# A511-1103/building-detection

Measured on AMD Instinct MI355X. Metric: 512x512 tiles/sec fwd+bwd DeepLabv3+ (v3plus.py) (full train step: fwd+loss+bwd+Adam), higher is better.
Workload: dtype f32; 1 GPU; DeepLabv3+ (v3plus.py) 512x512 bs=16/GPU fp32, train step, single GPU; global_batch=16, train_step=eager launches, side_stream_filter_gradients=True

## Files before the change

building_detection_amd/_lib.py:

```python
from __future__ import annotations

import ctypes as C
import os
import threading

_HERE = os.path.dirname(os.path.abspath(__file__))
LIB_PATH = os.path.join(_HERE, "libsegengine.so")

SG_F32, SG_BF16, SG_I64 = 0, 1, 2
SG_HEAD_F32 = 0x100
SG_COMM_ID_BYTES = 128
SG_EPI_BIAS, SG_EPI_RELU = 1, 2
SG_PRO_UP2, SG_EPI_DOWN2 = 16, 32
SG_X_UP2 = 0x200
SG_ACT_RELU, SG_ACT_SIGMOID = 0, 1
SG_LOSS_CE2, SG_LOSS_FOCAL, SG_LOSS_EDGE_FOCAL = 0, 1, 2
SG_MAX_CLASSES = 32
SG_AUGMENT_MAX_ITEMS = 64
SG_AUG_FLIP_UD, SG_AUG_FLIP_LR, SG_AUG_SWAP_RB, SG_AUG_THRESHOLD = 1, 2, 4, 8
SG_SCENE_MAX_ITEMS = 64
SG_SYM_FLIP_UD, SG_SYM_FLIP_LR, SG_SYM_TRANSPOSE = 1, 2, 4
SG_OPT_ADAM, SG_OPT_SGD = 0, 1
SG_OPT_AMSGRAD, SG_OPT_NESTEROV, SG_OPT_EMA = 1, 2, 4
SG_OPT_CLIP_NONE, SG_OPT_CLIP_VALUE, SG_OPT_CLIP_NORM, SG_OPT_CLIP_GLOBAL = 0, 1, 2, 3
# ... 148 lines not shown
    elif k == SG_CK_X6:
        n += f".BN{la.bn}.v{la.var}" + (".mf16" if la.mf16 else "") + (".npl1" if pl.npl == 1 else "")
    elif k == SG_CK_B16:
        n += f".BN{la.bn}.KS{la.ks}.PD{la.pd}"
    elif k == SG_CK_X6W:
        n += f".S{pl.x6w_S}"
    elif k == SG_CK_B16W:
        n += f".S{pl.b16w_S}"
    elif k == SG_CK_PATCH:
        n += f".C{la.pc}" + ("m" if la.pmulti else "") + f".BN{la.bn}"
    elif k == SG_CK_WIDE:
        n += (".b16" if b16 else ".x6") + f".W{la.bn}"
    n += "".join("." + o for o in operands)
    if la.skip_taps:
        n += ".skip"
    if pl.perm2 and k in (SG_CK_X6, SG_CK_B16):
        n += ".perm2"
    if la.group_m > 1:
        n += f".gm{la.group_m}"
    if la.cb:
        n += f".cb{la.cb}"
    if pl.Ckp != pl.Ck and pl.family == SG_CF_SLAB and pl.fast:
        n += ".vpad"
    if pl.nsub > 1:
        n += f".sub{pl.nb}+{pl.tail_n}"
    return n


class SegPlan(C.Structure):

    _fields_ = [(n, C.c_int) for n in ("V", "TX", "TY", "gx", "S")] + [("part_bytes", C.c_size_t)]


_vp, _i, _i64, _f, _sz = C.c_void_p, C.c_int, C.c_int64, C.c_float, C.c_size_t
_op = C.POINTER(ConvOpts)
_dp = C.POINTER(ConvDesc)
_pp = C.POINTER(C.c_void_p)
_fp = C.POINTER(C.c_float)

_SIGNATURES = {
    "sg_abi_version": (_i, []),
    "sg_last_error": (C.c_char_p, []),
    "sg_set_conv_x6": (_i, [_i]),
    "sg_create": (_i, [_i, _pp]),
    "sg_destroy": (_i, [_vp]),
    "sg_num_cus": (_i, [_vp]),
    "sg_conv2d_fwd": (_i, [_vp, _vp, _i, _dp, _vp, _vp, _vp, _vp, _i, _op]),
    "sg_conv2d_fwd_ws_bytes": (_sz, [_dp]),
    "sg_conv2d_fwd_stats_bytes": (_sz, [_dp]),
    "sg_get_conv_x6": (_i, []),
    "sg_conv2d_planes_job": (_i, [_vp, _i, _dp, _i, C.POINTER(PlanesJob), C.POINTER(C.c_size_t)]),
    "sg_prepare_planes": (_i, [_vp, _vp, _vp, _vp, _vp, _i, _i]),
    "sg_bn_tiles_ws_bytes": (_sz, [_vp, _i, _i]),
    "sg_bn_train_fwd_tiles": (_i, [_vp, _vp, _i, _i64, _i, _vp, _i, _vp, _vp, _vp, _vp, C.c_float, C.c_float, _i, _vp, _sz]),
    "sg_bn_apply": (_i, [_vp, _vp, _i, _i64, _i, _vp, _vp, _vp, _vp, _vp, _vp, _i]),
    "sg_conv2d_dgrad_ws_bytes": (_sz, [_dp]),
    "sg_conv2d_dgrad": (_i, [_vp, _vp, _i, _dp, _vp, _vp, _vp, _vp, _i, _op]),
    "sg_conv2d_wgrad_ws_bytes": (_sz, [_vp, _dp]),
    "sg_conv2d_wgrad": (_i, [_vp, _vp, _i, _dp, _vp, _vp, _vp, _vp, _op]),
    "sg_conv2d_caps": (_i, [_vp, _i, _dp, _i, C.POINTER(ConvCaps)]),
    "sg_conv2d_plan": (_i, [_vp, _i, _dp, _i, _i, _i, C.POINTER(ConvPlan)]),
    "sg_split_planes": (_i, [_vp, _vp, _vp, _i64, _i, _i, _vp]),
    "sg_conv2d_wgrad_planes_ws_bytes": (_sz, [_vp, _dp]),
    "sg_conv2d_wgrad_planes": (_i, [_vp, _vp, _dp, _vp, _vp, _vp, _vp, _sz]),
    "sg_conv2d_wgrad_plan": (_i, [_vp, _i, _dp, _i, _i, C.POINTER(WgradPlan)]),
    "sg_bias_grad_ws_bytes": (_sz, [_vp, _i64, _i]),
    "sg_bias_grad": (_i, [_vp, _vp, _i, _i64, _i, _i, _vp, _vp, _vp, _sz]),
    "sg_dwconv2d_fwd": (_i, [_vp, _vp, _i, _dp, _vp, _vp, _vp, _i, C.POINTER(BnIn)]),
    "sg_dwconv2d_dgrad": (_i, [_vp, _vp, _i, _dp, _vp, _vp, _vp, _vp, _i, _vp, C.POINTER(DwBnSums)]),
    "sg_dwconv2d_dgrad_bnsums_ws_bytes": (_sz, [_vp, _dp]),
    "sg_dwconv2d_wgrad_ws_bytes": (_sz, [_vp, _dp]),
    "sg_dwconv2d_wgrad": (_i, [_vp, _vp, _i, _dp, _vp, _vp, _vp, _i, C.POINTER(BnIn), _vp, _sz]),
    "sg_dwconv2d_plan": (_i, [_vp, _i, _dp, _i, _i, _i, C.POINTER(DwPlan)]),
    "sg_dense_fwd": (_i, [_vp, _vp, _i, _i, _i, _i, _vp, _vp, _vp, _vp, _i]),
    "sg_bn_ws_bytes": (_sz, [_vp, _i64, _i]),
    "sg_bn_train_fwd": (_i, [_vp, _vp, _i, _i64, _i, _vp, _vp, _vp, _vp, _vp, _vp, _vp, _vp, _f, _f, _i, _i, _vp, _sz]),
    "sg_bn_train_bwd": (_i, [_vp, _vp, _i, _i64, _i, _vp, _vp, _vp, _vp, _vp, _vp, _vp, _vp, _vp, _vp, _i, _vp, _sz]),
    "sg_bn_train_bwd_apply": (_i, [_vp, _vp, _i, _i64, _i] + [_vp] * 9 + [_i]),
    "sg_bn_train_bwd_thin_ok": (_i, [_vp, _i, _i64, _i, _i, _i]),
    "sg_bn_train_bwd_thin": (_i, [_vp, _vp, _i, _i64, _i, _i, _i] + [_vp] * 10 + [_i, _vp, _sz]),
    "sg_bn_infer": (_i, [_vp, _vp, _i, _i64, _i, _vp, _vp, _vp, _vp, _vp, _vp, _f, _i]),
    "sg_add2_bn": (_i, [_vp, _vp, _i, _i64, _i] + [_vp] * 11 + [_i, _i, _f, _i, _i]),
    "sg_bn_plan": (_i, [_vp, _i, _i64, _i, _i, _i, C.POINTER(BnPlan)]),
    "sg_seg_plan": (_i, [_vp, _i, _i, _i64, _i, _i, _i, C.POINTER(SegPlan)]),
    "sg_act_fwd": (_i, [_vp, _vp, _i, _i, _i64, _vp, _vp]),
    "sg_act_bwd": (_i, [_vp, _vp, _i, _i, _i64, _vp, _vp, _vp, _i]),
    "sg_add_n": (_i, [_vp, _vp, _i, _i, _pp, _i64, _vp, _i]),
    "sg_copy_channels": (_i, [_vp, _vp, _i, _i64, _i, _vp, _i, _i, _vp, _i, _i, _i]),
    "sg_softmax2_fwd": (_i, [_vp, _vp, _i, _i64, _vp, _vp]),
    "sg_softmax2_bwd": (_i, [_vp, _vp, _i, _i64, _vp, _vp, _vp]),
    "sg_softmax_fwd": (_i, [_vp, _vp, _i, _i64, _i, _vp, _vp]),
    "sg_softmax_bwd": (_i, [_vp, _vp, _i, _i64, _i, _vp, _vp, _vp]),
    "sg_softmax_branch_fwd": (_i, [_vp, _vp, _i, _i, _i, _i, _vp, _vp]),
    "sg_softmax_branch_bwd": (_i, [_vp, _vp, _i, _i, _i, _i, _vp, _vp, _vp]),
    "sg_bcast_mul_fwd": (_i, [_vp, _vp, _i, _i, _i64, _i, _i, _vp, _vp, _vp, _i]),
    "sg_bcast_mul_bwd_ws_bytes": (_sz, [_vp, _i, _i64, _i, _i]),
    "sg_bcast_mul_bwd": (_i, [_vp, _vp, _i, _i, _i64, _i, _i, _vp, _vp, _vp, _vp, _vp, _i, _vp, _sz]),
    "sg_scse_fwd": (_i, [_vp, _vp, _i, _i, _i64, _i, _vp, _vp, _vp, _vp]),
    "sg_scse_bwd_ws_bytes": (_sz, [_vp, _i, _i64, _i]),
    "sg_scse_bwd": (_i, [_vp, _vp, _i, _i, _i64, _i, _vp, _vp, _vp, _vp, _vp, _vp, _vp, _vp, _sz]),
    "sg_scse_bwd_sums": (_i, [_vp, _vp, _i, _i, _i64, _i, _vp, _vp, _vp, _vp, _vp, _vp, _vp, _sz]),
    "sg_scse_bwd_final": (_i, [_vp, _vp, _i, _i, _i64, _i, _vp, _vp, _vp, _vp, _vp, _vp, _vp, _i]),
    "sg_bam_fwd": (_i, [_vp, _vp, _i, _i, _i64, _i, _vp, _vp, _vp, _vp]),
    "sg_bam_bwd_ws_bytes": (_sz, [_vp, _i, _i64, _i]),
    "sg_bam_bwd": (_i, [_vp, _vp, _i, _i, _i64, _i, _vp, _vp, _vp, _vp, _vp, _vp, _vp, _vp, _sz]),
    "sg_maxpool_fwd": (_i, [_vp, _vp, _i, _i, _i, _i, _i, _i, _i, _i, _i, _i, _i, _vp, _vp]),
    "sg_maxpool_bwd": (_i, [_vp, _vp, _i, _i, _i, _i, _i, _i, _i, _i, _i, _i, _i, _vp, _vp, _vp, _vp]),
    "sg_maxpool_fwd_idx": (_i, [_vp, _vp, _i, _i, _i, _i, _i, _i, _i, _i, _i, _i, _i, _vp, _vp, _vp]),
    "sg_maxpool_bwd_idx": (_i, [_vp, _vp, _i, _i, _i, _i, _i, _i, _i, _i, _i, _i, _i, _vp, _vp, _vp]),
    "sg_avgpool_ws_bytes": (_sz, [_vp, _i, _i, _i, _i, _i, _i]),
    "sg_avgpool_fwd": (_i, [_vp, _vp, _i, _i, _i, _i, _i, _i, _i, _vp, _vp, _vp, _sz]),
    "sg_avgpool_bwd": (_i, [_vp, _vp, _i, _i, _i, _i, _i, _i, _i, _vp, _vp, _i]),
    "sg_upsample_nearest_fwd": (_i, [_vp, _vp, _i, _i, _i, _i, _i, _i, _i, _vp, _vp, _i]),
    "sg_upsample_nearest_bwd": (_i, [_vp, _vp, _i, _i, _i, _i, _i, _i, _i, _vp, _i, _vp, _i]),
    "sg_upsample_bilinear_fwd": (_i, [_vp, _vp, _i, _i, _i, _i, _i, _i, _i, _vp, _vp, _i]),
    "sg_upsample_bilinear_bwd": (_i, [_vp, _vp, _i, _i, _i, _i, _i, _i, _i, _vp, _i, _vp, _i]),
    "sg_loss_ws_bytes": (_sz, [_vp, _i64]),
    "sg_loss_fwd": (_i, [_vp, _vp, _i, _i64, _i, _vp, _vp, _vp, _vp, _sz]),
    "sg_loss_bwd": (_i, [_vp, _vp, _i, _i64, _i, _vp, _vp, _vp, _f]),
    "sg_confusion_counts": (_i, [_vp, _vp, _i64, _i, _vp, _vp, _vp]),
    "sg_lossn_ws_bytes": (_sz, [_vp, _i64]),
    "sg_lossn_fwd": (_i, [_vp, _vp, _i, _i64, _i, _i, _fp, _vp, _vp, _vp, _vp, _sz]),
    "sg_lossn_bwd": (_i, [_vp, _vp, _i, _i64, _i, _i, _fp, _vp, _vp, _vp, _f]),
    "sg_confusion_matrix": (_i, [_vp, _vp, _i64, _i, _i, _vp, _vp, _vp]),
    "sg_loss_region_ws_bytes": (_sz, [_vp, C.POINTER(RegionDesc)]),
    "sg_loss_region_fwd": (_i, [_vp, _vp, C.POINTER(RegionDesc), _vp, _vp, _vp, _vp, _vp, _sz]),
    "sg_loss_region_bwd": (_i, [_vp, _vp, C.POINTER(RegionDesc), _vp, _vp, _vp, _vp, _f]),
    "sg_loss_mined_ws_bytes": (_sz, [_vp, C.POINTER(MineDesc)]),
    "sg_loss_mined_fwd": (_i, [_vp, _vp, C.POINTER(MineDesc), _vp, _vp, _vp, _vp, _vp, _sz]),
    "sg_loss_mined_bwd": (_i, [_vp, _vp, C.POINTER(MineDesc), _vp, _vp, _vp, _vp, _f]),
    "sg_adam_step": (_i, [_vp, _vp, _i64, _vp, _vp, _vp, _vp, _f, _f, _f, _f, _f]),
    "sg_adam_step_lr": (_i, [_vp, _vp, _i64, _vp, _vp, _vp, _vp, _vp, _f, _f, _f, _f]),
    "sg_optim_norms_ws_bytes": (_sz, [_i]),
    "sg_optim_grad_norms": (_i, [_vp, _vp, C.POINTER(OptimTable), _vp, _f, _vp, _vp, _sz]),
    "sg_optim_step": (_i, [_vp, _vp, C.POINTER(OptimDesc), C.POINTER(OptimTable), _vp, _vp, _vp, _vp, _vp, _vp, _vp, _f, _f, _vp]),
    "sg_edge_labels": (_i, [_vp, _vp, _i, _i, _i, _i, _vp, _vp]),
    "sg_resize_linear_u8": (_i, [_vp, _vp, _i, _i, _i, _i, _vp, _i, _i, _vp]),
    "sg_augment_u8": (_i, [_vp, _vp, _i, _i, _i, _i, _vp, _i, _vp, _i, _i, _i, _vp]),
    "sg_argmax_accumulate_i8": (_i, [_vp, _vp, _vp, _i, _i, _vp, _i, _i, _i, _i]),
    "sg_argmax_max_u8": (_i, [_vp, _vp, _vp, _i, _i, _i, _vp, _i, _i, _i, _i]),
    "sg_scene_tiles_u8": (_i, [_vp, _vp, _i, _i, _vp, _i, _vp, _i, _vp]),
    "sg_prob_accumulate": (_i, [_vp, _vp, _i, _i, _vp, _i, _vp, _vp, _f, _vp, _vp, _i, _i]),
    "sg_prob_finalize": (_i, [_vp, _vp, _i, _vp, _vp, _i, _i, _vp, _i, _vp]),
    "sg_vote_ge": (_i, [_vp, _vp, _i, _pp, _i64, _i, _vp]),
    "sg_mask_objects_ws_bytes": (_sz, [_i, _i]),
    "sg_mask_objects": (_i, [_vp, _vp, _i, _i, _vp, _i, _vp, _sz, _vp, _vp, _i, _vp, _vp]),
    "sg_mask_split_words": (_i64, [_i, _i, _i, _i, _i, _i]),
    "sg_mask_split": (_i, [_vp, _vp, _i, _i, _vp, _vp, _vp, _vp, _i, _i, _vp, _vp]),
    "sg_objects_label_ws_bytes": (_sz, [_i, _i]),
    "sg_objects_label": (_i, [_vp, _vp, _i, _i, _vp, _i, _vp, _sz, _vp, _vp, _i, _vp]),
    "sg_objects_overlap_ws_bytes": (_sz, [_i64]),
    "sg_objects_overlap": (_i, [_vp, _vp, _i, _i, _vp, _vp, _i64, _vp, _sz, _vp, _vp]),
    "sg_object_distances_ws_bytes": (_sz, [_i, _i, _i]),
    "sg_object_distances": (_i, [_vp, _vp, _i, _i, _i, _vp, _vp, _sz, _vp, _vp]),
    "sg_separation_weights": (_i, [_vp, _vp, _i, _i, _i, _vp, _vp, _f, _f, _vp]),
    "sg_u8_to_f32": (_i, [_vp, _vp, _i64, _vp, _vp, _f, _f]),
    "sg_cast": (_i, [_vp, _vp, _i, _i, _i64, _vp, _vp]),
    "sg_fill_f32": (_i, [_vp, _vp, _vp, _i64, _f]),
    "sg_trace_mark": (_i, [_vp, _vp, _i, _i]),
    "sg_scale_f32": (_i, [_vp, _vp, _vp, _i64, _f]),
    "sg_comm_probe": (_i, [_vp]),
    "sg_comm_unique_id": (_i, [_vp]),
    "sg_comm_init": (_i, [_vp, _i, _i, _i, _pp]),
    "sg_comm_allreduce_sum": (_i, [_vp, _vp, _i, _vp, _i64]),
    "sg_comm_rank": (_i, [_vp]),
    "sg_comm_nranks": (_i, [_vp]),
# ... 58 lines not shown
```

building_detection_amd/csrc/norm.hip:

```cpp
#include "sg_reduce.h"

namespace {

__device__ __forceinline__ float bn_affine(float x, float mean, float invstd, float gamma, float beta) {
  return fmaf((x - mean) * invstd, gamma, beta);
}
template <int MODE, int V>
__device__ __forceinline__ void bn_mask(float (&g)[V], const float (&x)[V], const float (&y)[V], const float (&mean)[V],
                                        const float (&invstd)[V], const float (&gamma)[V], const float (&beta)[V]) {
  if constexpr (MODE == 2) {
#pragma unroll
    for (int i = 0; i < V; ++i) g[i] = bn_affine(x[i], mean[i], invstd[i], gamma[i], beta[i]) > 0.f ? g[i] : 0.f;
  } else if constexpr (MODE == 1) {
#pragma unroll
    for (int i = 0; i < V; ++i) g[i] = y[i] > 0.f ? g[i] : 0.f;
  }
}
__device__ __forceinline__ float bn_dx(float x, float g, float mean, float invstd, float gamma, float dgamma, float dbeta, float inv_n) {
  const float xh = (x - mean) * invstd;
  return gamma * invstd * (g - dbeta * inv_n - xh * dgamma * inv_n);
}

template <typename T>
struct BnStatsOp {
  static constexpr int NOUT = 2;
  const T* __restrict__ x;
  int C;
  int64_t rows;
  float* moving_mean;
  float* moving_var;
  float* save_mean;
  float* save_invstd;
  float momentum, eps;
  int unbiased;

  template <int V>
  __device__ __forceinline__ void accum(int, int64_t r, int c, float (&acc)[2][V]) const {
    float k[V], v[V];
    ldv<V>(x + c, k);
    ldv<V>(x + r * C + c, v);
#pragma unroll
    for (int i = 0; i < V; ++i) {
      const float d = v[i] - k[i];
      acc[0][i] += d;
      acc[1][i] = fmaf(d, d, acc[1][i]);
    }
  }
  __device__ __forceinline__ void finalize(int, int c, const double (&s)[2]) const {
    const double n = (double)rows;
    const double m1 = s[0] / n;
    const double mean = (double)ld1<T>(x + c) + m1;
    double var = s[1] / n - m1 * m1;
    if (var < 0.0) var = 0.0;
    save_mean[c] = (float)mean;
    save_invstd[c] = (float)(1.0 / sqrt(var + (double)eps));
    const double var_u = (unbiased && rows > 1) ? var * (n / (n - 1.0)) : var;
    moving_mean[c] = (float)((double)moving_mean[c] * momentum + mean * (1.0 - (double)momentum));
    moving_var[c] = (float)((double)moving_var[c] * momentum + var_u * (1.0 - (double)momentum));
  }
};

template <int V>
struct BnCtx {
  float mv[V], iv[V], gm[V], bt[V];
};

template <typename T, int MODE>
struct BnBwdOp {
  static constexpr int NOUT = 2;
  const T* __restrict__ x;
  const T* __restrict__ y;
  const T* __restrict__ dy;
  const float* __restrict__ mean;
  const float* __restrict__ invstd;
  const float* __restrict__ gamma;
  const float* __restrict__ beta;
  float* dgamma;
  float* dbeta;
  int C;

  template <int V>
  __device__ __forceinline__ BnCtx<V> begin(int, int c) const {
    BnCtx<V> k;
    ldv<V>(mean + c, k.mv);
    ldv<V>(invstd + c, k.iv);
    if constexpr (MODE == 2) {
      ldv<V>(gamma + c, k.gm);
      ldv<V>(beta + c, k.bt);
    }
    return k;
  }
  template <int V>
  __device__ __forceinline__ void accum(int, int64_t r, int c, float (&acc)[2][V], const BnCtx<V>& k) const {
    float xv[V], gv[V], yv[V];
    ldv<V>(x + r * C + c, xv);
    ldv<V>(dy + r * C + c, gv);
    if constexpr (MODE == 1) ldv<V>(y + r * C + c, yv);
    bn_mask<MODE>(gv, xv, yv, k.mv, k.iv, k.gm, k.bt);
#pragma unroll
    for (int i = 0; i < V; ++i) {
      acc[0][i] += gv[i];
      acc[1][i] = fmaf(gv[i], (xv[i] - k.mv[i]) * k.iv[i], acc[1][i]);
    }
  }
  __device__ __forceinline__ void finalize(int, int c, const double (&s)[2]) const {
    dbeta[c] = (float)s[0];
    dgamma[c] = (float)s[1];
  }
};

template <int V, int CO>
__device__ __forceinline__ void thin_w(const float* __restrict__ w, int c, float (&wv)[V][CO]) {
#pragma unroll
  for (int k = 0; k < V; ++k)
#pragma unroll
    for (int o = 0; o < CO; ++o) wv[k][o] = w[(c + k) * CO + o];
}
template <int V, int CO>
__device__ __forceinline__ void thin_dy(const float* __restrict__ g, const float (&wv)[V][CO], float (&dy)[V]) {
  float gv[CO];
#pragma unroll
  for (int o = 0; o < CO; ++o) gv[o] = g[o];
#pragma unroll
  for (int k = 0; k < V; ++k) {
    float a = 0.f;
#pragma unroll
    for (int o = 0; o < CO; ++o) a = fmaf(gv[o], wv[k][o], a);
    dy[k] = a;
  }
}

template <int V, int CO>
struct BnThinCtx {
  BnCtx<V> k;
  float wv[V][CO];
};

template <int MODE, int CO>
struct BnBwdThinOp {
  static constexpr int NOUT = 2;
  const float* __restrict__ x;
  const float* __restrict__ g;
  const float* __restrict__ w;
  const float* __restrict__ mean;
  const float* __restrict__ invstd;
  const float* __restrict__ gamma;
  const float* __restrict__ beta;
  float* dgamma;
  float* dbeta;
  int C, y_ld;

  template <int V>
  __device__ __forceinline__ BnThinCtx<V, CO> begin(int, int c) const {
    BnThinCtx<V, CO> q;
    ldv<V>(mean + c, q.k.mv);
    ldv<V>(invstd + c, q.k.iv);
    if constexpr (MODE == 2) {
      ldv<V>(gamma + c, q.k.gm);
      ldv<V>(beta + c, q.k.bt);
    }
    thin_w<V, CO>(w, c, q.wv);
    return q;
  }
  template <int V>
  __device__ __forceinline__ void accum(int, int64_t r, int c, float (&acc)[2][V], const BnThinCtx<V, CO>& q) const {
    float xv[V], gv[V], yv[V];
    ldv<V>(x + r * C + c, xv);
    thin_dy<V, CO>(g + r * y_ld, q.wv, gv);
    bn_mask<MODE>(gv, xv, yv, q.k.mv, q.k.iv, q.k.gm, q.k.bt);
#pragma unroll
    for (int i = 0; i < V; ++i) {
      acc[0][i] += gv[i];
      acc[1][i] = fmaf(gv[i], (xv[i] - q.k.mv[i]) * q.k.iv[i], acc[1][i]);
    }
  }
  __device__ __forceinline__ void finalize(int, int c, const double (&s)[2]) const {
    dbeta[c] = (float)s[0];
    dgamma[c] = (float)s[1];
  }
};

template <int V, typename T>
__global__ void bn_apply_kernel(const T* __restrict__ x, const float* __restrict__ mean,
                                const float* __restrict__ invstd, const float* __restrict__ gamma,
                                const float* __restrict__ beta, T* __restrict__ y, int64_t rows, int C, int relu,
                                float eps, int infer, FastDiv fd_cv) {
  const uint32_t cv = C / V;
  const uint32_t total = (uint32_t)(rows * cv);
  const uint32_t stride = gridDim.x * blockDim.x;
  for (uint32_t i = blockIdx.x * blockDim.x + threadIdx.x; i < total; i += stride) {
    const int64_t r = fd_div(i, fd_cv);
    const int c = (int)(i - (uint32_t)r * cv) * V;
    float xv[V], mv[V], iv[V], gv[V], bv[V], o[V];
    ldv<V>(x + r * C + c, xv);
    ldv<V>(mean + c, mv);
    ldv<V>(invstd + c, iv);
    ldv<V>(gamma + c, gv);
    ldv<V>(beta + c, bv);
#pragma unroll
    for (int k = 0; k < V; ++k) {
      const float is = infer ? rsqrtf(iv[k] + eps) : iv[k];
      float t = bn_affine(xv[k], mv[k], is, gv[k], bv[k]);
      if (relu) t = fmaxf(t, 0.f);
      o[k] = t;
    }
    stv<V>(y + r * C + c, o);
  }
}

template <int V, typename T, int MODE>
__global__ void bn_bwd_apply_kernel(const T* __restrict__ x, const T* __restrict__ y,
                                    const T* __restrict__ dy, const float* __restrict__ mean,
                                    const float* __restrict__ invstd, const float* __restrict__ gamma,
                                    const float* __restrict__ beta, const float* __restrict__ dgamma,
                                    const float* __restrict__ dbeta, T* __restrict__ dx, int64_t rows, int C,
                                    FastDiv fd_cv) {
  const uint32_t cv = C / V;
  const uint32_t total = (uint32_t)(rows * cv);
  const uint32_t stride = gridDim.x * blockDim.x;
  const float inv_n = 1.0f / (float)rows;
  for (uint32_t i = blockIdx.x * blockDim.x + threadIdx.x; i < total; i += stride) {
    const int64_t r = fd_div(i, fd_cv);
    const int c = (int)(i - (uint32_t)r * cv) * V;
    float xv[V], gv[V], mv[V], iv[V], gam[V], dg[V], db[V], o[V];
    ldv<V>(x + r * C + c, xv);
    ldv<V>(dy + r * C + c, gv);
    ldv<V>(mean + c, mv);
    ldv<V>(invstd + c, iv);
    ldv<V>(gamma + c, gam);
    ldv<V>(dgamma + c, dg);
    ldv<V>(dbeta + c, db);
    if constexpr (MODE == 2) {
      float bt[V];
      ldv<V>(beta + c, bt);
#pragma unroll
      for (int k = 0; k < V; ++k) gv[k] = bn_affine(xv[k], mv[k], iv[k], gam[k], bt[k]) > 0.f ? gv[k] : 0.f;
    } else if constexpr (MODE == 1) {
      float yv[V];
      ldv<V>(y + r * C + c, yv);
#pragma unroll
      for (int k = 0; k < V; ++k) gv[k] = yv[k] > 0.f ? gv[k] : 0.f;
    }
#pragma unroll
    for (int k = 0; k < V; ++k) {
      const float xh = (xv[k] - mv[k]) * iv[k];
      o[k] = gam[k] * iv[k] * (gv[k] - db[k] * inv_n - xh * dg[k] * inv_n);
    }
    stv<V>(dx + r * C + c, o);
  }
}

template <int V, typename T>
__global__ __launch_bounds__(256) void bn_apply_cols_kernel(const T* __restrict__ x, const float* __restrict__ mean,
                                                            const float* __restrict__ invstd, const float* __restrict__ gamma,
                                                            const float* __restrict__ beta, T* __restrict__ y, int64_t rows,
                                                            int C, int relu, float eps, int infer, int prow, FastDiv fd_cv) {
  const uint32_t i0 = blockIdx.x * 256u + threadIdx.x, cv = (uint32_t)(C / V);
  const uint32_t r0 = fd_div(i0, fd_cv);
  const int c = (int)(i0 - r0 * cv) * V;
  float mv[V], is[V], gv[V], bv[V];
  ldv<V>(mean + c, mv);
  ldv<V>(invstd + c, is);
  ldv<V>(gamma + c, gv);
  ldv<V>(beta + c, bv);
  if (infer) {
#pragma unroll
    for (int k = 0; k < V; ++k) is[k] = rsqrtf(is[k] + eps);
  }
  auto one = [&](const float (&xv)[V], int64_t r) {
    float o[V];
#pragma unroll
    for (int k = 0; k < V; ++k) {
      float t = bn_affine(xv[k], mv[k], is[k], gv[k], bv[k]);
      if (relu) t = fmaxf(t, 0.f);
      o[k] = t;
    }
    stv<V>(y + r * C + c, o);
  };
  const int64_t stride = prow, gstep = (int64_t)gridDim.y * 4 * prow;
  for (int64_t r = (int64_t)blockIdx.y * 4 * prow + r0; r < rows; r += gstep) {
    if (r + 3 * stride < rows) {
      float x0[V], x1[V], x2[V], x3[V];
      ldv<V>(x + r * C + c, x0);
      ldv<V>(x + (r + stride) * C + c, x1);
      ldv<V>(x + (r + 2 * stride) * C + c, x2);
      ldv<V>(x + (r + 3 * stride) * C + c, x3);
      one(x0, r); one(x1, r + stride); one(x2, r + 2 * stride); one(x3, r + 3 * stride);
    } else {
      for (int64_t q = r; q < rows; q += stride) {
        float x0[V];
        ldv<V>(x + q * C + c, x0);
        one(x0, q);
      }
    }
  }
}
constexpr int BN_APPLY_PERIODS = 4;

template <int V, typename T, int MODE>
__global__ __launch_bounds__(256) void bn_bwd_apply_cols_kernel(const T* __restrict__ x, const T* __restrict__ y,
                                                                const T* __restrict__ dy, const float* __restrict__ mean,
                                                                const float* __restrict__ invstd, const float* __restrict__ gamma,
                                                                const float* __restrict__ beta, const float* __restrict__ dgamma,
                                                                const float* __restrict__ dbeta, T* __restrict__ dx, int64_t rows,
                                                                int C, int prow, FastDiv fd_cv) {
  const uint32_t i0 = blockIdx.x * 256u + threadIdx.x, cv = (uint32_t)(C / V);
  const uint32_t r0 = fd_div(i0, fd_cv);
  const int c = (int)(i0 - r0 * cv) * V;
  float mv[V], iv[V], gam[V], dg[V], db[V], bt[V];
  ldv<V>(mean + c, mv);
  ldv<V>(invstd + c, iv);
  ldv<V>(gamma + c, gam);
  ldv<V>(dgamma + c, dg);
  ldv<V>(dbeta + c, db);
  if constexpr (MODE == 2) ldv<V>(beta + c, bt);
  const float inv_n = 1.0f / (float)rows;
  auto one = [&](const float (&xv)[V], float (&gv)[V], const float (&yv)[V], int64_t r) {
    float o[V];
    bn_mask<MODE>(gv, xv, yv, mv, iv, gam, bt);
#pragma unroll
    for (int k = 0; k < V; ++k) o[k] = bn_dx(xv[k], gv[k], mv[k], iv[k], gam[k], dg[k], db[k], inv_n);
    stv<V>(dx + r * C + c, o);
  };
  const int64_t stride = (int64_t)gridDim.y * prow, gstep = 2 * stride;
  for (int64_t r = (int64_t)blockIdx.y * prow + r0; r < rows; r += gstep) {
    if (r + stride < rows) {
      float x0[V], x1[V], g0[V], g1[V], y0[V], y1[V];
      ldv<V>(x + r * C + c, x0);
      ldv<V>(x + (r + stride) * C + c, x1);
      ldv<V>(dy + r * C + c, g0);
      ldv<V>(dy + (r + stride) * C + c, g1);
      if constexpr (MODE == 1) {
        ldv<V>(y + r * C + c, y0);
        ldv<V>(y + (r + stride) * C + c, y1);
      }
      one(x0, g0, y0, r);
      one(x1, g1, y1, r + stride);
    } else {
      float x0[V], g0[V], y0[V];
      ldv<V>(x + r * C + c, x0);
      ldv<V>(dy + r * C + c, g0);
      if constexpr (MODE == 1) ldv<V>(y + r * C + c, y0);
      one(x0, g0, y0, r);
    }
  }
}
constexpr int BN_BWD_PERIODS = 1;

template <int V, int MODE, int CO>
__global__ void bn_bwd_apply_thin_kernel(const BnBwdThinOp<MODE, CO> q, float* __restrict__ dx, int64_t rows, FastDiv fd_cv) {
  const int C = q.C;
  const uint32_t cv = C / V;
  const uint32_t total = (uint32_t)(rows * cv);
  const uint32_t stride = gridDim.x * blockDim.x;
  const float inv_n = 1.0f / (float)rows;
  for (uint32_t i = blockIdx.x * blockDim.x + threadIdx.x; i < total; i += stride) {
    const int64_t r = fd_div(i, fd_cv);
    const int c = (int)(i - (uint32_t)r * cv) * V;
    float xv[V], gv[V], mv[V], iv[V], gam[V], dg[V], db[V], o[V], wv[V][CO];
    ldv<V>(q.x + r * C + c, xv);
    thin_w<V, CO>(q.w, c, wv);
    thin_dy<V, CO>(q.g + r * q.y_ld, wv, gv);
    ldv<V>(q.mean + c, mv);
    ldv<V>(q.invstd + c, iv);
    ldv<V>(q.gamma + c, gam);
    ldv<V>(q.dgamma + c, dg);
    ldv<V>(q.dbeta + c, db);
    if constexpr (MODE == 2) {
      float bt[V];
      ldv<V>(q.beta + c, bt);
#pragma unroll
      for (int k = 0; k < V; ++k) gv[k] = bn_affine(xv[k], mv[k], iv[k], gam[k], bt[k]) > 0.f ? gv[k] : 0.f;
    }
#pragma unroll
    for (int k = 0; k < V; ++k) {
      const float xh = (xv[k] - mv[k]) * iv[k];
      o[k] = gam[k] * iv[k] * (gv[k] - db[k] * inv_n - xh * dg[k] * inv_n);
    }
    stv<V>(dx + r * C + c, o);
  }
}

template <int V, int MODE, int CO>
__global__ __launch_bounds__(256) void bn_bwd_apply_cols_thin_kernel(const BnBwdThinOp<MODE, CO> q, float* __restrict__ dx,
                                                                     int64_t rows, int prow, FastDiv fd_cv) {
  const int C = q.C;
  const uint32_t i0 = blockIdx.x * 256u + threadIdx.x, cv = (uint32_t)(C / V);
  const uint32_t r0 = fd_div(i0, fd_cv);
  const int c = (int)(i0 - r0 * cv) * V;
  float mv[V], iv[V], gam[V], dg[V], db[V], bt[V], wv[V][CO];
  ldv<V>(q.mean + c, mv);
  ldv<V>(q.invstd + c, iv);
  ldv<V>(q.gamma + c, gam);
  ldv<V>(q.dgamma + c, dg);
  ldv<V>(q.dbeta + c, db);
  if constexpr (MODE == 2) ldv<V>(q.beta + c, bt);
  thin_w<V, CO>(q.w, c, wv);
  const float inv_n = 1.0f / (float)rows;
  auto one = [&](const float (&xv)[V], float (&gv)[V], int64_t r) {
    float o[V];
    bn_mask<MODE>(gv, xv, xv, mv, iv, gam, bt);
#pragma unroll
    for (int k = 0; k < V; ++k) o[k] = bn_dx(xv[k], gv[k], mv[k], iv[k], gam[k], dg[k], db[k], inv_n);
    stv<V>(dx + r * C + c, o);
  };
  const int64_t stride = (int64_t)gridDim.y * prow, gstep = 2 * stride;
  for (int64_t r = (int64_t)blockIdx.y * prow + r0; r < rows; r += gstep) {
    if (r + stride < rows) {
      float x0[V], x1[V], g0[V], g1[V];
      ldv<V>(q.x + r * C + c, x0);
      ldv<V>(q.x + (r + stride) * C + c, x1);
      thin_dy<V, CO>(q.g + r * q.y_ld, wv, g0);
      thin_dy<V, CO>(q.g + (r + stride) * q.y_ld, wv, g1);
      one(x0, g0, r);
      one(x1, g1, r + stride);
    } else {
      float x0[V], g0[V];
      ldv<V>(q.x + r * C + c, x0);
      thin_dy<V, CO>(q.g + r * q.y_ld, wv, g0);
      one(x0, g0, r);
    }
  }
}

// ... 26 lines not shown
        for (int k = 0; k < V; ++k) is[o][k] = rsqrtf(is[o][k] + eps);
      }
    } else {
#pragma unroll
      for (int k = 0; k < V; ++k) { mv[o][k] = 0.f; is[o][k] = 1.f; gv[o][k] = 1.f; bv[o][k] = 0.f; }
    }
  }
  auto one = [&](const float (&xa)[V], const float (&xb)[V], int64_t r) {
    float o[V];
#pragma unroll
    for (int k = 0; k < V; ++k) {
      float ta = on[0] ? bn_affine(xa[k], mv[0][k], is[0][k], gv[0][k], bv[0][k]) : xa[k];
      float tb = on[1] ? bn_affine(xb[k], mv[1][k], is[1][k], gv[1][k], bv[1][k]) : xb[k];
      if (q.relu_op[0]) ta = fmaxf(ta, 0.f);
      if (q.relu_op[1]) tb = fmaxf(tb, 0.f);
      float t = ta + tb;
      if (relu) t = fmaxf(t, 0.f);
      o[k] = t;
    }
    stv<V>(y + r * C + c, o);
  };
  const int64_t stride = prow, gstep = (int64_t)gridDim.y * 2 * prow;
  for (int64_t r = (int64_t)blockIdx.y * 2 * prow + r0; r < rows; r += gstep) {
    if (r + stride < rows) {
      float a0[V], a1[V], b0[V], b1[V];
      ldv<V>(a + r * C + c, a0);
      ldv<V>(a + (r + stride) * C + c, a1);
      ldv<V>(b + r * C + c, b0);
      ldv<V>(b + (r + stride) * C + c, b1);
      one(a0, b0, r);
      one(a1, b1, r + stride);
    } else {
      float a0[V], b0[V];
      ldv<V>(a + r * C + c, a0);
      ldv<V>(b + r * C + c, b0);
      one(a0, b0, r);
    }
  }
}
constexpr int BN_ADD2_PERIODS = 2;

struct BnPlan : sg_bn_plan_t { SegPlan seg; int refused; };

inline bool bn_cols_grid(int num_cus, int64_t rows, int cv, int unroll, sg_bn_plan_t& pl) {
  int g = 256, a = cv;
  while (a) { const int t_ = g % a; g = a; a = t_; }
  const int64_t b0 = cv / g;
  if (b0 > 16384) return false;
  pl.prow = 256 / g;
  int64_t k = sg_cdiv((int64_t)8 * num_cus, b0);
  const int64_t maxk = sg_cdiv(rows, (int64_t)unroll * pl.prow);
  if (k > maxk) k = maxk;
  if (k > 65535) k = 65535;
  if (k < 1) k = 1;
  pl.gx = (int)b0; pl.gy = (int)k;
  return true;
}

inline BnPlan plan_bn(int num_cus, int dtype, int64_t rows, int C, int pass, bool aligned) {
  BnPlan pl = {};
  const bool vec = aligned && C % 4 == 0, add2 = pass == SG_BN_ADD2;
  pl.V = (vec && dtype == SG_BF16 && C % 8 == 0) ? 8 : (vec ? 4 : 1);
  const int unroll = add2 ? BN_ADD2_PERIODS : ((pass == SG_BN_BWD || pass == SG_BN_BWD_APPLY) ? BN_BWD_PERIODS : BN_APPLY_PERIODS);
  pl.cols = vec && (add2 || sg_switch<SW_BN_COLS>()) && bn_cols_grid(num_cus, rows, C / pl.V, unroll, pl);
  if (!pl.cols && add2) { pl = {}; pl.refused = SG_EUNSUPPORTED; }
  else if (!pl.cols) { pl.gx = (int)ew_blocks(rows * (C / pl.V), 8192); pl.gy = 1; }
  if (pass == SG_BN_FWD || pass == SG_BN_BWD) {
    pl.seg = seg_plan<2>(num_cus, 1, rows, C, vec, dtype == SG_BF16);
    pl.seg_V = pl.seg.V; pl.seg_TX = pl.seg.TX; pl.seg_TY = pl.seg.TY; pl.seg_gx = pl.seg.gx; pl.seg_S = pl.seg.S;
    pl.fused = seg_fused_alone(pl.seg.S);
    pl.fin_lanes = pl.fused ? 0 : seg_finalize_lanes(pl.seg.S);
    pl.ws_bytes = pl.seg.part_bytes;
  }
  return pl;
}

inline int bn_check(const sg_ctx* ctx, int dtype, int64_t rows, int C, bool chunked, const char* who) {
  SG_CHECK_ARG(ctx && (dtype == SG_F32 || dtype == SG_BF16), "%s: bad ctx/dtype", who);
  SG_CHECK_ARG(rows > 0 && C > 0, "%s: bad argument", who);
  SG_CHECK_ARG(chunked || rows * C < (1ll << 31), "%s: tensor exceeds 2^31 elements", who);
  return 0;
}

inline int bn_refuse(const BnPlan& pl, const char* who, const void* ws, size_t ws_bytes) {
  if (pl.refused) {
    sg_set_error("%s: needs C %% 4 == 0, 16-byte aligned tensors and a column grid; apply the BatchNormalization and add instead", who);
    return pl.refused;
  }
  if (pl.ws_bytes && (!ws || ws_bytes < pl.ws_bytes)) {
    sg_set_error("%s: workspace %zu < %zu", who, ws_bytes, pl.ws_bytes);
    return SG_EWORKSPACE;
  }
  return 0;
}

template <class F>
inline void bn_with_form(const BnPlan& pl, F&& fn) {
  constexpr std::integral_constant<int, 8> v8{}; constexpr std::integral_constant<int, 4> v4{};
  if (pl.V == 8) pl.cols ? fn(v8, std::true_type{}) : fn(v8, std::false_type{});
  else if (pl.V == 4) pl.cols ? fn(v4, std::true_type{}) : fn(v4, std::false_type{});
  else fn(std::integral_constant<int, 1>{}, std::false_type{});
}
template <class F>
inline int bn_with_mode(int relu, const void* beta, F&& fn) {
  if (!relu) return fn(std::integral_constant<int, 0>{});
  return beta ? fn(std::integral_constant<int, 2>{}) : fn(std::integral_constant<int, 1>{});
}

template <typename T>
int launch_bn_apply(hipStream_t st, const BnPlan& pl, const T* x, const float* mean, const float* invstd, const float* gamma,
                    const float* beta, T* y, int64_t rows, int C, int relu, float eps, int infer) {
  const FastDiv fd = make_fastdiv((uint32_t)(C / pl.V));
  const dim3 grid((unsigned)pl.gx, (unsigned)pl.gy);
  bn_with_form(pl, [&](auto v, auto cols) {
    constexpr int V = decltype(v)::value;
    if constexpr (decltype(cols)::value)
      hipLaunchKernelGGL((bn_apply_cols_kernel<V, T>), grid, dim3(256), 0, st, x, mean, invstd, gamma, beta, y, rows, C, relu, eps,
                         infer, pl.prow, fd);
    else
      hipLaunchKernelGGL((bn_apply_kernel<V, T>), grid, dim3(256), 0, st, x, mean, invstd, gamma, beta, y, rows, C, relu, eps, infer, fd);
  });
  SG_LAUNCH_CHECK(pl.cols ? "bn_apply_cols_kernel" : "bn_apply_kernel");
  return 0;
}

template <typename T, int MODE>
int launch_bn_bwd_apply(hipStream_t st, const BnPlan& pl, const BnBwdOp<T, MODE>& q, T* dx, int64_t rows) {
  const FastDiv fd = make_fastdiv((uint32_t)(q.C / pl.V));
  const dim3 grid((unsigned)pl.gx, (unsigned)pl.gy);
  bn_with_form(pl, [&](auto v, auto cols) {
    constexpr int V = decltype(v)::value;
    if constexpr (decltype(cols)::value)
      hipLaunchKernelGGL((bn_bwd_apply_cols_kernel<V, T, MODE>), grid, dim3(256), 0, st, q.x, q.y, q.dy, q.mean, q.invstd, q.gamma,
                         q.beta, q.dgamma, q.dbeta, dx, rows, q.C, pl.prow, fd);
    else
      hipLaunchKernelGGL((bn_bwd_apply_kernel<V, T, MODE>), grid, dim3(256), 0, st, q.x, q.y, q.dy, q.mean, q.invstd, q.gamma, q.beta,
                         q.dgamma, q.dbeta, dx, rows, q.C, fd);
  });
  SG_LAUNCH_CHECK(pl.cols ? "bn_bwd_apply_cols_kernel" : "bn_bwd_apply_kernel");
  return 0;
}

template <int MODE, int CO>
int launch_bn_bwd_apply_thin(hipStream_t st, const BnPlan& pl, const BnBwdThinOp<MODE, CO>& q, float* dx, int64_t rows) {
  const FastDiv fd = make_fastdiv((uint32_t)(q.C / pl.V));
  const dim3 grid((unsigned)pl.gx, (unsigned)pl.gy);
  bn_with_form(pl, [&](auto v, auto cols) {
    constexpr int V = decltype(v)::value;
    if constexpr (V == 8) return;
    else if constexpr (decltype(cols)::value)
      hipLaunchKernelGGL((bn_bwd_apply_cols_thin_kernel<V, MODE, CO>), grid, dim3(256), 0, st, q, dx, rows, pl.prow, fd);
    else
      hipLaunchKernelGGL((bn_bwd_apply_thin_kernel<V, MODE, CO>), grid, dim3(256), 0, st, q, dx, rows, fd);
  });
  SG_LAUNCH_CHECK(pl.cols ? "bn_bwd_apply_cols_thin_kernel" : "bn_bwd_apply_thin_kernel");
  return 0;
}

inline int64_t add2_chunk_rows(int64_t rows, int C) { return rows * C < (1ll << 31) ? rows : (((1ll << 31) - 1) / C) & ~1ll; }

int bn_apply_entry(const char* who, sg_ctx* ctx, void* stream, int dtype, int64_t rows, int C, const void* x, const void* gamma,
                   const void* beta, const void* mean, const void* invstd, void* y, int relu, float eps, int infer) {
  if (int e = bn_check(ctx, dtype, rows, C, false, who)) return e;
  SG_CHECK_ARG(x && gamma && beta && mean && invstd && y, "%s: bad argument", who);
  const BnPlan pl = plan_bn(ctx->num_cus, dtype, rows, C, SG_BN_APPLY, sg_all_aligned16({x, y}));
  SG_DTYPE_SWITCH(dtype, who, {
    return launch_bn_apply<T>((hipStream_t)stream, pl, (const T*)x, (const float*)mean, (const float*)invstd, (const float*)gamma,
                              (const float*)beta, (T*)y, rows, C, relu, eps, infer);
  });
  return 0;
}

}

extern "C" {

int sg_bn_plan(const sg_ctx* ctx, int dtype, int64_t rows, int C, int pass, int aligned, sg_bn_plan_t* out) {
  SG_CHECK_ARG(out, "sg_bn_plan: null out");
  *out = sg_bn_plan_t{};
  SG_CHECK_ARG(pass >= SG_BN_FWD && pass <= SG_BN_ADD2, "sg_bn_plan: bad pass");
  if (int e = bn_check(ctx, dtype, rows, C, pass == SG_BN_ADD2, "sg_bn_plan")) return e;
  if (pass == SG_BN_ADD2) rows = add2_chunk_rows(rows, C);
  SG_CHECK_ARG(rows > 0, "sg_bn_plan: a single row exceeds 2^31 elements");
  const BnPlan pl = plan_bn(ctx->num_cus, dtype, rows, C, pass, aligned != 0);
  if (int e = bn_refuse(pl, "sg_bn_plan", out, pl.ws_bytes)) return e;
  *out = pl;
  return 0;
}

size_t sg_bn_ws_bytes(const sg_ctx* ctx, int64_t rows, int C) {
  if (!ctx) return 0;
  size_t m = 0;
  for (int dtype : {SG_F32, SG_BF16})
    for (bool aligned : {false, true}) m = std::max(m, plan_bn(ctx->num_cus, dtype, rows, C, SG_BN_FWD, aligned).ws_bytes);
  return m + 256;
}

int sg_bn_train_fwd(sg_ctx* ctx, void* stream, int dtype, int64_t rows, int C, const void* x, const void* gamma, const void* beta,
                    void* moving_mean, void* moving_var, void* y, void* save_mean, void* save_invstd, float momentum, float eps,
                    int relu, int unbiased_update, void* ws, size_t ws_bytes) {
  if (int e = bn_check(ctx, dtype, rows, C, false, "sg_bn_train_fwd")) return e;
  SG_CHECK_ARG(x && gamma && beta && moving_mean && moving_var && y && save_mean && save_invstd, "sg_bn_train_fwd: bad argument");
  const BnPlan pl = plan_bn(ctx->num_cus, dtype, rows, C, SG_BN_FWD, sg_all_aligned16({x, y}));
  if (int e = bn_refuse(pl, "sg_bn_train_fwd", ws, ws_bytes)) return e;
  SG_DTYPE_SWITCH(dtype, "sg_bn_train_fwd", {
    const BnStatsOp<T> op = {(const T*)x, C, rows, (float*)moving_mean, (float*)moving_var, (float*)save_mean, (float*)save_invstd,
                             momentum, eps, unbiased_update};
    if (int e = seg_reduce_launch(op, pl.seg, 1, rows, C, (float*)ws, (hipStream_t)stream, "bn_stats")) return e;
    return launch_bn_apply<T>((hipStream_t)stream, pl, op.x, op.save_mean, op.save_invstd, (const float*)gamma, (const float*)beta, (T*)y, rows, C, relu,
                              eps, 0);
  });
  return 0;
}

int sg_bn_train_bwd(sg_ctx* ctx, void* stream, int dtype, int64_t rows, int C, const void* x, const void* y, const void* dy,
                    const void* gamma, const void* beta, const void* save_mean, const void* save_invstd, void* dx, void* dgamma,
                    void* dbeta, int relu, void* ws, size_t ws_bytes) {
  if (int e = bn_check(ctx, dtype, rows, C, false, "sg_bn_train_bwd")) return e;
  SG_CHECK_ARG(x && dy && gamma && save_mean && save_invstd && dx && dgamma && dbeta, "sg_bn_train_bwd: bad argument");
  SG_CHECK_ARG(!relu || y || beta, "sg_bn_train_bwd: relu set but neither y nor beta given");
  const BnPlan pl = plan_bn(ctx->num_cus, dtype, rows, C, SG_BN_BWD, sg_all_aligned16({x, dy, dx, relu ? y : nullptr}));
  if (int e = bn_refuse(pl, "sg_bn_train_bwd", ws, ws_bytes)) return e;
  SG_DTYPE_SWITCH(dtype, "sg_bn_train_bwd", {
    return bn_with_mode(relu, beta, [&](auto m) -> int {
      const BnBwdOp<T, decltype(m)::value> op = {(const T*)x, (const T*)y, (const T*)dy, (const float*)save_mean, (const float*)save_invstd,
                                                 (const float*)gamma, (const float*)beta, (float*)dgamma, (float*)dbeta, C};
      if (int e = seg_reduce_launch(op, pl.seg, 1, rows, C, (float*)ws, (hipStream_t)stream, "bn_bwd_reduce")) return e;
      return launch_bn_bwd_apply((hipStream_t)stream, pl, op, (T*)dx, rows);
    });
  });
  return 0;
}

int sg_bn_train_bwd_apply(sg_ctx* ctx, void* stream, int dtype, int64_t rows, int C, const void* x, const void* dy, const void* gamma,
                          const void* beta, const void* save_mean, const void* save_invstd, const void* dgamma, const void* dbeta,
                          void* dx, int relu) {
  if (int e = bn_check(ctx, dtype, rows, C, false, "sg_bn_train_bwd_apply")) return e;
  SG_CHECK_ARG(x && dy && gamma && save_mean && save_invstd && dx && dgamma && dbeta, "sg_bn_train_bwd_apply: bad argument");
  SG_CHECK_ARG(!relu || beta, "sg_bn_train_bwd_apply: relu needs beta (the mask is recomputed from x)");
  const BnPlan pl = plan_bn(ctx->num_cus, dtype, rows, C, SG_BN_BWD_APPLY, sg_all_aligned16({x, dy, dx}));
  SG_DTYPE_SWITCH(dtype, "sg_bn_train_bwd_apply", {
    return bn_with_mode(relu, beta, [&](auto m) -> int {
      const BnBwdOp<T, decltype(m)::value> op = {(const T*)x, nullptr, (const T*)dy, (const float*)save_mean, (const float*)save_invstd,
                                                 (const float*)gamma, (const float*)beta, (float*)dgamma, (float*)dbeta, C};
      return launch_bn_bwd_apply((hipStream_t)stream, pl, op, (T*)dx, rows);
    });
  });
  return 0;
}

int sg_bn_train_bwd_thin_ok(const sg_ctx* ctx, int dtype, int64_t rows, int C, int CO, int y_ld) {
  return ctx && dtype == SG_F32 && rows > 0 && C > 0 && rows * C < (1ll << 31) && CO >= 1 && CO <= 4 && y_ld >= CO &&
         rows * y_ld < (1ll << 31);
}

int sg_bn_train_bwd_thin(sg_ctx* ctx, void* stream, int dtype, int64_t rows, int C, int CO, int y_ld, const void* x, const void* g,
                         const void* w, const void* gamma, const void* beta, const void* save_mean, const void* save_invstd, void* dx,
                         void* dgamma, void* dbeta, int relu, void* ws, size_t ws_bytes) {
  if (int e = bn_check(ctx, dtype, rows, C, false, "sg_bn_train_bwd_thin")) return e;
  SG_CHECK_ARG(x && g && w && gamma && save_mean && save_invstd && dx && dgamma && dbeta, "sg_bn_train_bwd_thin: bad argument");
  SG_CHECK_ARG(!relu || beta, "sg_bn_train_bwd_thin: relu needs beta (the mask is recomputed from x)");
  if (!sg_bn_train_bwd_thin_ok(ctx, dtype, rows, C, CO, y_ld)) {
    sg_set_error("sg_bn_train_bwd_thin: needs fp32 storage and 1 <= CO <= 4, CO <= y_ld; run the thin dgrad and sg_bn_train_bwd instead");
    return SG_EUNSUPPORTED;
  }
  const BnPlan pl = plan_bn(ctx->num_cus, dtype, rows, C, SG_BN_BWD, sg_all_aligned16({x, dx}));
  if (int e = bn_refuse(pl, "sg_bn_train_bwd_thin", ws, ws_bytes)) return e;
  auto run = [&](auto m, auto co) -> int {
    const BnBwdThinOp<decltype(m)::value, decltype(co)::value> op = {
        (const float*)x, (const float*)g, (const float*)w, (const float*)save_mean, (const float*)save_invstd, (const float*)gamma,
        (const float*)beta, (float*)dgamma, (float*)dbeta, C, y_ld};
    if (int e = seg_reduce_launch(op, pl.seg, 1, rows, C, (float*)ws, (hipStream_t)stream, "bn_bwd_thin_reduce")) return e;
    return launch_bn_bwd_apply_thin((hipStream_t)stream, pl, op, (float*)dx, rows);
  };
  auto with_co = [&](auto m) -> int {
    switch (CO) {
      case 1: return run(m, std::integral_constant<int, 1>{});
      case 2: return run(m, std::integral_constant<int, 2>{});
      case 3: return run(m, std::integral_constant<int, 3>{});
      default: return run(m, std::integral_constant<int, 4>{});
    }
  };
  return relu ? with_co(std::integral_constant<int, 2>{}) : with_co(std::integral_constant<int, 0>{});
}

int sg_bn_apply(sg_ctx* ctx, void* stream, int dtype, int64_t rows, int C, const void* x, const void* gamma,
                const void* beta, const void* mean, const void* invstd, void* y, int relu) {
  return bn_apply_entry("sg_bn_apply", ctx, stream, dtype, rows, C, x, gamma, beta, mean, invstd, y, relu, 0.f, 0);
}

int sg_bn_infer(sg_ctx* ctx, void* stream, int dtype, int64_t rows, int C, const void* x, const void* gamma,
                const void* beta, const void* moving_mean, const void* moving_var, void* y, float eps, int relu) {
  return bn_apply_entry("sg_bn_infer", ctx, stream, dtype, rows, C, x, gamma, beta, moving_mean, moving_var, y, relu, eps, 1);
}

int sg_add2_bn(sg_ctx* ctx, void* stream, int dtype, int64_t rows, int C, const void* a, const void* b, const void* a_mean,
               const void* a_invstd, const void* a_gamma, const void* a_beta, const void* b_mean, const void* b_invstd,
               const void* b_gamma, const void* b_beta, void* y, int relu, int infer, float eps, int a_relu, int b_relu) {
  if (int e = bn_check(ctx, dtype, rows, C, true, "sg_add2_bn")) return e;
  SG_CHECK_ARG(a && b && y, "sg_add2_bn: bad argument");
  SG_CHECK_ARG((a_mean != nullptr) == (a_invstd != nullptr && a_gamma != nullptr && a_beta != nullptr) &&
                   (b_mean != nullptr) == (b_invstd != nullptr && b_gamma != nullptr && b_beta != nullptr),
               "sg_add2_bn: an operand's four BatchNormalization parameters come together or not at all");
  const bool aligned = sg_all_aligned16({a, b, y});
  const int64_t chunk_rows = add2_chunk_rows(rows, C);
  SG_CHECK_ARG(chunk_rows > 0, "sg_add2_bn: a single row exceeds 2^31 elements");
  const Add2BnArgs q = {{(const float*)a_mean, (const float*)b_mean}, {(const float*)a_invstd, (const float*)b_invstd},
                        {(const float*)a_gamma, (const float*)b_gamma}, {(const float*)a_beta, (const float*)b_beta},
                        {(a_mean && a_relu) ? 1 : 0, (b_mean && b_relu) ? 1 : 0}};
  SG_DTYPE_SWITCH(dtype, "sg_add2_bn", {
    for (int64_t r0 = 0; r0 < rows; r0 += chunk_rows) {
      const int64_t nr = rows - r0 < chunk_rows ? rows - r0 : chunk_rows;
      const BnPlan pl = plan_bn(ctx->num_cus, dtype, nr, C, SG_BN_ADD2, aligned);
      if (int e = bn_refuse(pl, "sg_add2_bn", nullptr, 0)) return e;
      bn_with_form(pl, [&](auto v, auto cols) {
        constexpr int V = decltype(v)::value;
        if constexpr (decltype(cols)::value)
          hipLaunchKernelGGL((add2_bn_kernel<V, T>), dim3((unsigned)pl.gx, (unsigned)pl.gy), dim3(256), 0, (hipStream_t)stream,
                             (const T*)a + r0 * C, (const T*)b + r0 * C, q, (T*)y + r0 * C, nr, C, relu, eps, infer, pl.prow,
                             make_fastdiv((uint32_t)(C / V)));
      });
    }
  });
  SG_LAUNCH_CHECK("add2_bn_kernel");
  return 0;
}

}
```

building_detection_amd/fusion.py:

```python
from . import layers as L
from . import switches


def sole_consumer(t, outs):
    while (len(t.consumers) == 1 and isinstance(t.consumers[0], L._ActNode) and t.consumers[0].fused_away
           and id(t.consumers[0].output) not in outs):
        t = t.consumers[0].output
    return t.consumers[0] if len(t.consumers) == 1 and id(t) not in outs else None


def root_of(t, path=None):
    while isinstance(t.node, L._ActNode) and t.node.fused_away and len(t.consumers) == 1:
        if path is not None:
            path.append(t.node)
        t = t.node.inputs[0]
    return t


def _bn4(nodes, outs):
    return [n for n in nodes if isinstance(n, L._BNNode) and len(n.output.shape) == 4 and id(n.output) not in outs]


def bias_and_stats(nodes, outs):
    for n in nodes:
# ... 60 lines not shown
        sc = sole_consumer(n.output, outs)
        _, h, w, c = n.output.shape
        if (n.defer_add is None and isinstance(sc, L._SepConvNode) and sc.stride == 1 and sc.bnsum_src is None
                and w % 4 == 0 and c % 4 == 0):
            n.sums_from, sc.bnsum_src = sc, n


def bn_sums_via_add(nodes, outs):
    if not switches.get("SG_BN_SUMS"):
        return
    for sc in nodes:
        if not isinstance(sc, L._SepConvNode) or sc.bnsum_src is not None or sc.stride != 1:
            continue
        path = []
        root = root_of(sc.inputs[0], path)
        first = path[-1] if path else sc
        a = root.node
        if not isinstance(a, L._AddNode) or a.relu or id(root) in outs or len(root.shape) != 4:
            continue
        if any(cn is not first and cn.index < sc.index for cn in root.consumers):
            continue
        cands = [b for b in a.bn_src if b is not None and b.sums_from is None and b.defer_add is a]
        _, h, w, c = root.shape
        if cands and w % 4 == 0 and c % 4 == 0:
            cands[0].sums_from, sc.bnsum_src = sc, cands[0]


def bn_gather(nodes, outs):
    if not switches.get("SG_BN_DEFER"):
        return
    for n in _bn4(nodes, outs):
        sc = sole_consumer(n.output, outs)
        _, h, w, c = n.output.shape
        if (isinstance(sc, L._SepConvNode) and sc.stride == 1 and not sc.pre_relu and sc.bn_src is None
                and w % 4 == 0 and c % 4 == 0):
            n.defer_to, sc.bn_src = sc, n


def bn_conv(nodes, outs):
    for n in _bn4(nodes, outs):
        c = sole_consumer(n.output, outs)
        if (n.defer_to is not None or n.defer_add is not None or not isinstance(c, L._ConvNode) or c.bn_src is not None
                or c.up_src is not None or c.stride != 1 or c.dilation != 1):
            continue
        cin = n.output.shape[-1]
        thin = c.k == 1 and c.filters <= 4 and cin % 4 == 0 and cin >= 16
        patch = c.k == 3 and c.padding == "same" and cin in (32, 64)
        if thin or patch:
            n.defer_conv, c.bn_src = c, n


def thin_grad(nodes, outs):
    for n in _bn4(nodes, outs):
        c = sole_consumer(n.output, outs)
        cin = n.output.shape[-1]
        if (isinstance(c, L._ConvNode) and c.k == 1 and c.stride == 1 and c.filters <= 4 and c.up_src is None
                and cin % 4 == 0 and cin >= 16):
            c.thin_bn = n


def scse_lowrank(nodes, outs):
    for n in nodes:
        if not isinstance(n, L._ScseCombineNode):
            continue
        x, s = n.inputs[0], n.inputs[1]
        sse, cons = s.node, x.consumers
        gaps = [q for q in cons if isinstance(q, L._AvgPoolNode) and q.global_pool]
        if (isinstance(sse, L._ConvNode) and len(cons) == 3 and len(gaps) == 1 and sse in cons and n in cons and id(x) not in outs
                and x.node is not None and sse.inputs[0] is x and sse.k == 1 and sse.stride == 1 and sse.filters == 1
                and sse.activation is None and sse.bn_src is None and sse.up_src is None and len(s.consumers) == 1
                and x.shape[-1] % 4 == 0 and x.shape[-1] >= 16):
            n.lowrank = (sse, gaps[0])


def bn_backward_in_pw(nodes, outs):
    for n in nodes:
        if isinstance(n, L._BNNode) and n.sums_from is not None and len(n.output.shape) == 4:
            prod = n.inputs[0].node
            if (isinstance(prod, L._SepConvNode) and prod.activation in (None, "linear") and len(n.inputs[0].consumers) == 1
                    and id(n.inputs[0]) not in outs):
                n.bnb_to = prod


RULES = (bias_and_stats, up2_conv, absorb_relu, bn_add, bn_sums, bn_sums_via_add, bn_gather, bn_conv, thin_grad, scse_lowrank,
         bn_backward_in_pw)


def run(nodes, outputs):
    outs = {id(t) for t in outputs}
    for rule in RULES:
        rule(nodes, outs)
```

building_detection_amd/layers.py:

```python
from __future__ import annotations


from typing import List, Optional, Sequence

import numpy as np

from .graph import KTensor, Node
from .ops import conv_out_geometry, same_pad
from . import _lib
from . import fusion
from . import switches


def _pair(v):
    if isinstance(v, (tuple, list)):
        assert len(v) == 2 and v[0] == v[1], f"only square kernels/strides occur on this path: {v}"
        return int(v[0])
    return int(v)


def _act_name(a):
    if a is None or a == "linear":
        return None
    if callable(a):
# ... 382 lines not shown
        super().__init__(name)
        self.units, self.activation = int(units), _act_name(activation)

    def __call__(self, x):
        self._once()
        return _DenseNode(self._name, self.units, self.activation).build(x)


class DeferredGrad:

    def materialise(self, eng):
        raise NotImplementedError

    def taken_by(self, node) -> bool:
        return False


class BnBackwardDeferred(DeferredGrad):

    def __init__(self, x, dy, gamma, beta, mean, invstd, dgamma, dbeta, relu):
        self.x, self.dy, self.gamma, self.beta, self.mean, self.invstd = x, dy, gamma, beta, mean, invstd
        self.dgamma, self.dbeta, self.relu = dgamma, dbeta, relu
        self.dtype, self.shape = dy.dtype, dy.shape

    def materialise(self, eng):
        return eng.bn_train_bwd_apply(self.x, self.dy, self.gamma, self.beta, self.mean, self.invstd, self.dgamma, self.dbeta,
                                      relu=self.relu)

    def taken_by(self, node):
        return isinstance(node, _SepConvNode)


class ThinGradDeferred(DeferredGrad):

    def __init__(self, g, w, desc, dtype):
        self.g, self.w, self.desc, self.dtype = g, w, desc, dtype
        self.shape = (desc.N, desc.H, desc.W, desc.Cin)

    def materialise(self, eng):
        return eng.conv2d_dgrad(self.g, self.w, self.desc, out_dtype=self.dtype)

    def taken_by(self, node):
        return isinstance(node, _BNNode) or (isinstance(node, _ActNode) and node.fused_away)


class ScseGradDeferred(DeferredGrad):

    def __init__(self, x, s, cl, dy):
        self.x, self.s, self.cl, self.dy = x, s, cl, dy
        self.dtype, self.shape = dy.dtype, dy.shape
        self.parts = []

    def add(self, eng, *part):
        self.parts.append(part)
        if len(self.parts) < 2:
            return self
        gap = next(p for p in self.parts if p[0] == "gap")
        sse = next(p for p in self.parts if p[0] == "sse")
        return eng.scse_bwd_final(self.dy, self.s, self.cl, sse[1], sse[2], gap[1], gap_first=self.parts[0][0] == "gap")

    def materialise(self, eng):
        dx, _, _ = eng.scse_bwd(self.x, self.s, self.cl, self.dy)
        n, h, w, c = self.shape
        for p in self.parts:
            if p[0] == "gap":
                dx = eng.avgpool_bwd(p[1], (n, h, w, c), h, w, out=dx, accumulate=True)
            else:
                dx = eng.conv2d_dgrad(p[1], p[2], p[3], out_dtype=self.dtype, res=dx)
        return dx


class _BNNode(Node):
    op = "batch_normalization"

    def __init__(self, name, momentum, epsilon):
        super().__init__(name)
        self.momentum, self.epsilon = momentum, epsilon
        self.relu = False
        self.defer_to = None
        self.defer_add = None
        self.sums_from = None
        self.defer_conv = None
        self.bnb_to = None

    def build(self, x):
        c = x.shape[-1]
        self.gamma = self.add_param("gamma", (c,), "ones", kind="gamma")
        self.beta = self.add_param("beta", (c,), "zeros", kind="beta")
        self.mm = self.add_param("moving_mean", (c,), "zeros", trainable=False, kind="moving_mean")
        self.mv = self.add_param("moving_variance", (c,), "ones", trainable=False, kind="moving_var")
        return self.connect([x], x.shape)

    def forward(self, rt, xs, training):
        (x,) = xs
        e = rt.eng
        if training:
            st = rt.bn_stats.pop(id(x), None)
            if st is not None:
                defer = self.defer_to is not None or self.defer_add is not None or (self.defer_conv is not None and rt.bn_conv_on(self))
                y, mean, invstd = e.bn_train_fwd_from_tiles(x, st[0], st[1], rt.param(self.gamma), rt.param(self.beta),
                                                            rt.param(self.mm), rt.param(self.mv), relu=self.relu,
                                                            momentum=self.momentum, eps=self.epsilon, apply=not defer)
                if defer:
                    rt.save(self, mean=mean, invstd=invstd, deferred=True)
                    return x
            else:
                y, mean, invstd = e.bn_train_fwd(x, rt.param(self.gamma), rt.param(self.beta), rt.param(self.mm),
                                                 rt.param(self.mv), relu=self.relu, momentum=self.momentum, eps=self.epsilon)
            rt.save(self, mean=mean, invstd=invstd, deferred=False)
            return y
        if self.defer_add is not None and x.shape[-1] % 4 == 0:
            rt.save(self, deferred=True)
            return x
        if self.defer_conv is not None and rt.bn_conv_on(self):
            rt.save(self, deferred=True)
            return x
        rt.save(self, deferred=False)
        return e.bn_infer(x, rt.param(self.gamma), rt.param(self.beta), rt.param(self.mm), rt.param(self.mv),
                          relu=self.relu, eps=self.epsilon)

    def backward(self, rt, xs, y, dy):
        (x,) = xs
        s = rt.saved(self)
        if isinstance(dy, ThinGradDeferred):
            if not s.get("sums_done") and rt.eng.bn_train_bwd_thin_ok(x, dy.g, dy.w):
                dx, _, _ = rt.eng.bn_train_bwd_thin(x, dy.g, dy.w, rt.param(self.gamma), s["mean"], s["invstd"], relu=self.relu,
                                                    dgamma=rt.grad(self.gamma), dbeta=rt.grad(self.beta), beta=rt.param(self.beta))
                return [dx]
            dy = dy.materialise(rt.eng)
        if s.get("sums_done") and self.bnb_to is not None and rt.bnb_on(self, x):
            return [BnBackwardDeferred(x, dy, rt.param(self.gamma), rt.param(self.beta), s["mean"], s["invstd"], rt.grad(self.gamma),
                                       rt.grad(self.beta), self.relu)]
        if s.get("sums_done"):
            return [rt.eng.bn_train_bwd_apply(x, dy, rt.param(self.gamma), rt.param(self.beta), s["mean"], s["invstd"],
                                              rt.grad(self.gamma), rt.grad(self.beta), relu=self.relu)]
        dx, _, _ = rt.eng.bn_train_bwd(x, y, dy, rt.param(self.gamma), s["mean"], s["invstd"], relu=self.relu,
                                       dgamma=rt.grad(self.gamma), dbeta=rt.grad(self.beta), beta=rt.param(self.beta))
        return [dx]


class BatchNormalization(Layer):
    def __init__(self, axis=-1, momentum=0.99, epsilon=1e-3, name=None, **kw):
        super().__init__(name)
        assert axis in (-1, 3, 1), "BatchNormalization on this path normalises the last axis"
        self.momentum, self.epsilon = momentum, epsilon

    def __call__(self, x):
        self._once()
        return _BNNode(self._name, self.momentum, self.epsilon).build(x)


class _ActNode(Node):
    op = "activation"

    def __init__(self, name, act, axis=-1):
        super().__init__(name)
        self.act, self.axis = act, axis
        self.fused_away = False

    def build(self, x):
        if self.act == "softmax":
            ax = self.axis if self.axis >= 0 else len(x.shape) + self.axis
            self.sm_axis = ax
            if ax == len(x.shape) - 1:
                if not 2 <= x.shape[-1] <= _lib.SG_MAX_CLASSES:
                    raise ValueError(f"last-axis softmax on this path has 2 ... {_lib.SG_MAX_CLASSES} classes, not {x.shape[-1]}")
            else:
                assert len(x.shape) == 4 and ax == 2 and x.shape[1] == 1, "branch softmax expects [N,1,B,C]"
        return self.connect([x], x.shape)

    def forward(self, rt, xs, training):
        (x,) = xs
        if self.fused_away:
            return x
        e = rt.eng
        if self.act == "relu":
            return e.act_fwd(x, _lib.SG_ACT_RELU)
        if self.act == "sigmoid":
            return e.act_fwd(x, _lib.SG_ACT_SIGMOID)
        if self.sm_axis == len(x.shape) - 1:
            return e.softmax2_fwd(x) if x.shape[-1] == 2 else e.softmax_fwd(x)
        n, _, b, c = x.shape
        return e.softmax_branch_fwd(x.view(n, b, c)).view(x.shape)

    def backward(self, rt, xs, y, dy):
        if self.fused_away:
            return [rt.shared(dy)]
        e = rt.eng
        if self.act == "relu":
            return [e.act_bwd(y, dy, _lib.SG_ACT_RELU)]
        if self.act == "sigmoid":
            return [e.act_bwd(y, dy, _lib.SG_ACT_SIGMOID)]
        if self.sm_axis == len(y.shape) - 1:
            return [e.softmax2_bwd(y, dy) if y.shape[-1] == 2 else e.softmax_bwd(y, dy)]
        n, _, b, c = y.shape
        return [e.softmax_branch_bwd(y.view(n, b, c), dy.view(n, b, c)).view(y.shape)]


class Activation(Layer):
    def __init__(self, activation, name=None, **kw):
        super().__init__(name)
        self.act = _act_name(activation)

    def __call__(self, x):
        self._once()
        return _ActNode(self._name, self.act).build(x)


class ReLU(Activation):
    def __init__(self, name=None, **kw):
        super().__init__("relu", name)


class Softmax(Layer):
    def __init__(self, axis=-1, name=None, **kw):
        super().__init__(name)
        self.axis = axis

    def __call__(self, x):
        self._once()
        return _ActNode(self._name, "softmax", self.axis).build(x)


class _MaxPoolNode(Node):
    op = "max_pooling2d"

    def __init__(self, name, pool, stride, padding):
        super().__init__(name)
        self.pool, self.stride, self.padding = pool, stride, padding

    def build(self, x):
        _, h, w, c = x.shape
        if self.padding == "same":
            ho, wo = same_pad(h, self.pool, self.stride)[0], same_pad(w, self.pool, self.stride)[0]
        else:
            ho, wo = (h - self.pool) // self.stride + 1, (w - self.pool) // self.stride + 1
        return self.connect([x], (None, ho, wo, c))

    def forward(self, rt, xs, training):
        if training and self.pool <= 15:
            y, geom, idx = rt.eng.maxpool_fwd(xs[0], self.pool, self.stride, self.padding, want_idx=True)
            rt.save(self, geom=geom, idx=idx)
            return y
        y, geom = rt.eng.maxpool_fwd(xs[0], self.pool, self.stride, self.padding)
        rt.save(self, geom=geom)
        return y

    def backward(self, rt, xs, y, dy):
        sv = rt.saved(self)
        if sv.get("idx") is not None:
            return [rt.eng.maxpool_bwd_idx(dy, sv["idx"], tuple(xs[0].shape), sv["geom"])]
        return [rt.eng.maxpool_bwd(xs[0], y, dy, sv["geom"])]


class MaxPooling2D(Layer):
    def __init__(self, pool_size=2, strides=None, padding="valid", name=None, **kw):
        super().__init__(name)
        self.pool = _pair(pool_size)
        self.stride = self.pool if strides is None else _pair(strides)
        self.padding = padding

    def __call__(self, x):
        self._once()
        return _MaxPoolNode(self._name, self.pool, self.stride, self.padding).build(x)


MaxPool2D = MaxPooling2D


class _AvgPoolNode(Node):
    op = "average_pooling2d"

    def __init__(self, name, pool, global_pool=False):
        super().__init__(name)
        self.pool, self.global_pool = pool, global_pool

    def build(self, x):
        _, h, w, c = x.shape
        if self.global_pool:
            return self.connect([x], (None, c))
        return self.connect([x], (None, h // self.pool, w // self.pool, c))

    def _k(self, x):
        return (x.shape[1], x.shape[2]) if self.global_pool else (self.pool, self.pool)

    def forward(self, rt, xs, training):
        (x,) = xs
        kh, kw = self._k(x)
        y = rt.eng.avgpool_fwd(x, kh, kw)
        return y.view(x.shape[0], x.shape[3]) if self.global_pool else y

    def backward(self, rt, xs, y, dy):
        (x,) = xs
        kh, kw = self._k(x)
        acc = rt.take_pending(self.inputs[0], owned_only=True)
        if isinstance(acc, ScseGradDeferred):
            if self.global_pool and acc.dtype == dy.dtype:
                return [acc.add(rt.eng, "gap", dy)]
            acc = acc.materialise(rt.eng)
        if acc is not None and acc.dtype == dy.dtype:
            return [rt.eng.avgpool_bwd(dy, tuple(x.shape), kh, kw, out=acc, accumulate=True)]
        if acc is not None:
            rt.put_back(self.inputs[0], acc)
        return [rt.eng.avgpool_bwd(dy, tuple(x.shape), kh, kw)]


class AveragePooling2D(Layer):
    def __init__(self, pool_size=2, strides=None, padding="valid", name=None, **kw):
        super().__init__(name)
        self.pool = _pair(pool_size)
        assert strides is None or _pair(strides) == self.pool

    def __call__(self, x):
        self._once()
        return _AvgPoolNode(self._name, self.pool).build(x)


class GlobalAveragePooling2D(Layer):
    def __call__(self, x):
        self._once()
        return _AvgPoolNode(self._name, 0, True).build(x)


GlobalAvgPool2D = GlobalAveragePooling2D


class _UpNode(Node):
    op = "up_sampling2d"

    def __init__(self, name, size, interpolation="nearest"):
        super().__init__(name)
        self.size = size
        self.interpolation = interpolation
        self.fused_into = None

    def build(self, x):
        _, h, w, c = x.shape
        return self.connect([x], (None, h * self.size, w * self.size, c))

    def forward(self, rt, xs, training):
        if self.interpolation == "bilinear":
            return rt.eng.upsample_bilinear_fwd(xs[0], self.size)
        if self.fused_into is not None and rt.up2_on(self):
            return xs[0]
        return rt.eng.upsample_fwd(xs[0], self.size)

    def backward(self, rt, xs, y, dy):
        if self.interpolation == "bilinear":
            return [rt.eng.upsample_bilinear_bwd(dy, tuple(xs[0].shape), self.size)]
        if self.fused_into is not None and rt.up2_on(self):
            return [rt.shared(dy)]
        return [rt.eng.upsample_bwd(dy, tuple(xs[0].shape), self.size)]


class UpSampling2D(Layer):
    def __init__(self, size=2, interpolation="nearest", name=None, **kw):
        super().__init__(name)
        if interpolation not in ("nearest", "bilinear"):
            raise ValueError(f"UpSampling2D: interpolation {interpolation!r} is not supported (use 'nearest' or 'bilinear')")
        self.size = _pair(size)
        self.interpolation = interpolation

    def __call__(self, x):
        self._once()
        return _UpNode(self._name, self.size, self.interpolation).build(x)


class _ReshapeNode(Node):
    op = "reshape"

    def __init__(self, name, target):
        super().__init__(name)
        self.target = tuple(target)

    def build(self, x):
        n_in = int(np.prod(x.shape[1:]))
        tgt = list(self.target)
        if -1 in tgt:
            known = int(np.prod([t for t in tgt if t != -1]))
            tgt[tgt.index(-1)] = n_in // known
        assert int(np.prod(tgt)) == n_in, (x.shape, self.target)
        return self.connect([x], (None,) + tuple(tgt))

    def forward(self, rt, xs, training):
        return xs[0].view(xs[0].shape[0], *self.output.shape[1:])

    def backward(self, rt, xs, y, dy):
        return [rt.shared(dy.view(xs[0].shape))]


class Reshape(Layer):
    def __init__(self, target_shape, name=None, **kw):
        super().__init__(name)
        self.target = tuple(target_shape)

    def __call__(self, x):
        self._once()
        return _ReshapeNode(self._name, self.target).build(x)


class _ConcatNode(Node):
    op = "concatenate"

    def build(self, xs):
        base = xs[0].shape[:-1]
        for t in xs:
            assert t.shape[:-1] == base, f"concat shapes differ: {[t.shape for t in xs]}"
        return self.connect(xs, base + (sum(t.shape[-1] for t in xs),))

    def forward(self, rt, xs, training):
        return rt.eng.concat(xs)

    def backward(self, rt, xs, y, dy):
        outs, off = [], 0
        for t, sym in zip(xs, self.inputs):
            c = t.shape[-1]
            if rt.needs_grad(sym):
                g = rt.eng.empty(*t.shape, dtype=dy.dtype)
                rt.eng.copy_channels(dy, off, g, 0, c)
                outs.append(g)
            else:
                outs.append(None)
            off += c
        return outs


def concatenate(xs, axis=-1, name=None):
    assert axis in (-1, len(xs[0].shape) - 1), "channel concat only"
    return _ConcatNode(name).build(list(xs))


class Concatenate(Layer):
    def __init__(self, axis=-1, name=None, **kw):
        super().__init__(name)
        self.axis = axis

    def __call__(self, xs):
        self._once()
        return concatenate(xs, self.axis, self._name)


class _AddNode(Node):
    op = "add"

    def __init__(self, name=None):
        super().__init__(name)
        self.relu = False
        self.bn_src = [None, None]

    def build(self, xs):
        for t in xs:
            assert t.shape == xs[0].shape, f"add shapes differ: {[t.shape for t in xs]}"
        return self.connect(xs, xs[0].shape)

    def forward(self, rt, xs, training):
        if len(xs) == 2 and (self.bn_src[0] is not None or self.bn_src[1] is not None):
            bn = [None, None]
            for i, src in enumerate(self.bn_src):
                if src is None:
                    continue
                sv = rt._saved.get(id(src)) or {}
                if sv.get("deferred"):
                    bn[i] = ((sv["mean"], sv["invstd"]) if training else (rt.param(src.mm), rt.param(src.mv))) + \
                            (rt.param(src.gamma), rt.param(src.beta))
            if bn[0] is not None or bn[1] is not None:
                eps = next(s.epsilon for s in self.bn_src if s is not None)
                ra, rb = (s is not None and s.relu for s in self.bn_src)
                return rt.eng.add2_bn(xs[0], xs[1], bn[0], bn[1], relu=self.relu, infer=not training, eps=eps,
                                      relu_a=ra and bn[0] is not None, relu_b=rb and bn[1] is not None)
        return rt.eng.add_n(xs, relu=self.relu)

    def backward(self, rt, xs, y, dy):
        g = rt.eng.act_bwd(y, dy, _lib.SG_ACT_RELU) if self.relu else dy
        return [rt.shared(g) for _ in xs]


def add(xs, name=None):
    return _AddNode(name).build(list(xs))


class Add(Layer):
    def __call__(self, xs):
        self._once()
        return add(xs, self._name)


class _BcastMulNode(Node):
    op = "multiply"

    def build(self, x, g):
        if len(g.shape) == 2 or g.shape[1:3] == (1, 1):
            assert g.shape[-1] == x.shape[-1]
            self.mode = 0
        else:
            assert g.shape[-1] == 1 and g.shape[1:3] == x.shape[1:3], (x.shape, g.shape)
            self.mode = 1
        return self.connect([x, g], x.shape)

    def forward(self, rt, xs, training):
        x, g = xs
# ... 135 lines not shown
```

building_detection_amd/ops.py:

```python
from __future__ import annotations

import collections
import contextlib
import ctypes as C
import threading
from typing import Optional, Sequence, Tuple

import torch

from . import _lib
from . import switches
from ._lib import ConvDesc, SG_F32, SG_BF16, SG_HEAD_F32, check


def same_pad(in_size: int, k: int, stride: int, dilation: int = 1) -> Tuple[int, int, int]:
    out = -(-in_size // stride)
    total = max((out - 1) * stride + (k - 1) * dilation + 1 - in_size, 0)
    before = total // 2
    return out, before, total - before


def conv_out_geometry(h: int, w: int, kh: int, kw: int, stride: int, dilation: int, padding: str):
    if padding == "same":
        ho, pt, _ = same_pad(h, kh, stride, dilation)
        wo, pl, _ = same_pad(w, kw, stride, dilation)
    elif padding == "valid":
        ho = (h - (kh - 1) * dilation - 1) // stride + 1
        wo = (w - (kw - 1) * dilation - 1) // stride + 1
        pt = pl = 0
    else:
        raise ValueError(f"padding={padding!r}")
    return ho, wo, pt, pl


def _ptr(t: Optional[torch.Tensor]):
    return None if t is None else C.c_void_p(t.data_ptr())


def _chk(t: torch.Tensor, name: str):
    if not t.is_cuda:
        raise _lib.SgError(f"{name}: expected a CUDA (HIP) tensor - this engine has no CPU path")
    if t.dtype not in (torch.float32, torch.bfloat16):
        raise _lib.SgError(f"{name}: expected float32 or bfloat16 storage, got {t.dtype}")
    if not t.is_contiguous():
        raise _lib.SgError(f"{name}: tensor must be contiguous")


def _chk32(t: torch.Tensor, name: str):
    _chk(t, name)
    if t.dtype != torch.float32:
        raise _lib.SgError(f"{name}: this tensor is fp32 in every storage mode (weights, statistics, head), got {t.dtype}")


def _dt(t: torch.Tensor) -> int:
    return SG_BF16 if t.dtype == torch.bfloat16 else SG_F32


_TRACE_MARK = switches.get("SG_TRACE_MARK")
_MARK_TAGS = {"dilated_conv": 0, "gemm_conv": 1}


_raw_stream = getattr(torch._C, "_cuda_getCurrentRawStream", None) or (lambda i: torch.cuda.current_stream(i).cuda_stream)


class _NoTimer:

    __slots__ = ()

    def __enter__(self):
        return self

    def __exit__(self, *exc):
        return False


_NO_TIMER = _NoTimer()


class _Timed:

    __slots__ = ("eng", "tag", "a")

    def __init__(self, eng, tag):
        self.eng, self.tag, self.a = eng, tag, None

    def __enter__(self):
        if getattr(self.eng, "_prof", None) is not None and self.tag:
            self.eng.join_side()
            if _TRACE_MARK and self.tag in _MARK_TAGS:
                self.eng.lib.sg_trace_mark(self.eng.h, self.eng.stream, _MARK_TAGS[self.tag], 0)
            self.a = torch.cuda.Event(enable_timing=True)
            self.a.record(torch.cuda.current_stream(self.eng.device))
        return self

    def __exit__(self, *exc):
        if self.a is not None:
            b = torch.cuda.Event(enable_timing=True)
            b.record(torch.cuda.current_stream(self.eng.device))
            self.eng._prof.setdefault(self.tag, []).append((self.a, b))
            if _TRACE_MARK and self.tag in _MARK_TAGS:
                self.eng.lib.sg_trace_mark(self.eng.h, self.eng.stream, _MARK_TAGS[self.tag], 1)
        return False


class OptimTable:

    def __init__(self, eng, chunks, segs, n):
        import numpy as np
        self.chunks = np.ascontiguousarray(chunks)
        self.segs = np.ascontiguousarray(segs)
        assert self.chunks.dtype.itemsize == C.sizeof(_lib.OptimChunk) and self.segs.dtype.itemsize == C.sizeof(_lib.OptimSeg)
        self.nchunks, self.nseg, self.n = len(self.chunks), len(self.segs), int(n)
        dev = lambda a: torch.from_numpy(a.view(np.uint8).reshape(-1).copy()).to(eng.device)
        self.chunks_dev, self.segs_dev = dev(self.chunks), dev(self.segs)
        self.ws = torch.zeros(max(self.nchunks, 2), dtype=torch.float64, device=eng.device)
        self.norms = torch.zeros(1 + self.nseg, dtype=torch.float64, device=eng.device)
        self.c = _lib.OptimTable(self.chunks.ctypes.data, self.segs.ctypes.data, self.chunks_dev.data_ptr(),
                                 self.segs_dev.data_ptr(), self.nchunks, self.nseg, self.n)


class Engine:

    def __init__(self, device: int = 0):
        if not torch.cuda.is_available():
            raise _lib.SgError("no HIP device visible; building_detection_amd requires an MI355X (gfx950) GPU")
        self.lib = _lib.load()
        torch.cuda.set_device(device)
        self.ctx = _lib.Context(device)
# ... 295 lines not shown
            bq = self._bn_in(bn_in)
            o.bn_in = C.pointer(bq)
        with self.timed(self._gemm_tag()):
            check(self.lib.sg_conv2d_wgrad(self.h, self.stream, dt, C.byref(d), _ptr(x), _ptr(dy), _ptr(dw),
                                           _ptr(db) if want_bias else None, C.byref(o)), "sg_conv2d_wgrad")
        return dw, (db if want_bias else None)

    def split_planes(self, x, out=None):
        _chk32(x, "x")
        c = x.shape[-1]
        rows = x.numel() // c
        pl = out if out is not None else torch.empty((3, rows, c), dtype=torch.int16, device=x.device)
        check(self.lib.sg_split_planes(self.h, self.stream, _ptr(x), rows, c, c, _ptr(pl)), "sg_split_planes")
        return pl

    def conv2d_wgrad_planes_ok(self, d: ConvDesc) -> bool:
        return bool(self.conv2d_caps(d).wgrad_planes)

    def conv2d_wgrad_planes(self, x_planes, dy_planes, d: ConvDesc, dw=None):
        if dw is None:
            dw = self.empty(d.KH, d.KW, d.Cin, d.Cout)
        wsp, wsn = self.ws(self.lib.sg_conv2d_wgrad_planes_ws_bytes(self.h, C.byref(d)))
        with self.timed(self._gemm_tag()):
            check(self.lib.sg_conv2d_wgrad_planes(self.h, self.stream, C.byref(d), _ptr(x_planes), _ptr(dy_planes), _ptr(dw), wsp, wsn),
                  "sg_conv2d_wgrad_planes")
        return dw

    def bias_grad(self, dy, db):
        c = dy.shape[-1]
        rows = dy.numel() // c
        wsp, wsn = self.ws(self.lib.sg_bias_grad_ws_bytes(self.h, rows, c))
        check(self.lib.sg_bias_grad(self.h, self.stream, _dt(dy), rows, c, c, _ptr(dy), _ptr(db), wsp, wsn), "sg_bias_grad")
        return db

    @staticmethod
    def _dw_bn(bn):
        if bn is None:
            return None
        gamma, beta, mean, invstd, relu = bn
        return C.byref(_lib.BnIn(_ptr(mean), _ptr(invstd), _ptr(gamma), _ptr(beta), int(relu), 0, 0.0))

    def dwconv_fwd(self, x, w, stride=1, pre_relu=False, out=None, desc=None, bn=None):
        _chk(x, "x"); _chk(w, "w")
        kh, kw, c = w.shape[0], w.shape[1], w.shape[2]
        d = desc or self.conv_desc(x.shape, c, kh, kw, stride, 1, "same")
        y = out if out is not None else self.empty(d.N, d.Ho, d.Wo, c, dtype=x.dtype)
        check(self.lib.sg_dwconv2d_fwd(self.h, self.stream, _dt(x), C.byref(d), _ptr(x), _ptr(w), _ptr(y),
                                       int(pre_relu) if bn is None else 0, self._dw_bn(bn)), "sg_dwconv2d_fwd")
        return y

    def dwconv_dgrad(self, dy, w, d: ConvDesc, x=None, pre_relu=False, out=None, res=None, sums=None):
        dx = out if out is not None else self.empty(d.N, d.H, d.W, d.Cin, dtype=dy.dtype)
        check(self.lib.sg_dwconv2d_dgrad(self.h, self.stream, _dt(dy), C.byref(d), _ptr(dy), _ptr(w), _ptr(x), _ptr(dx),
                                         int(pre_relu), _ptr(res), C.byref(sums) if sums is not None else None), "sg_dwconv2d_dgrad")
        return dx

    def dwconv_dgrad_bnsums(self, dy, w, d: ConvDesc, bn_x, bn_mean, bn_invstd, bn_gamma, bn_beta, bn_relu, dgamma, dbeta,
                            x=None, pre_relu=False, res=None, out=None):
        wsp, wsn = self.ws(self.lib.sg_dwconv2d_dgrad_bnsums_ws_bytes(self.h, C.byref(d)))
        q = _lib.DwBnSums(_ptr(bn_x), _ptr(bn_mean), _ptr(bn_invstd), _ptr(bn_gamma), _ptr(bn_beta), int(bn_relu), _ptr(dgamma),
                          _ptr(dbeta), wsp, wsn)
        return self.dwconv_dgrad(dy, w, d, x=x, pre_relu=pre_relu, out=out, res=res, sums=q)

    @staticmethod
    def dwconv_dgrad_acc_ok(d: ConvDesc) -> bool:
        return (d.KH == 3 and d.KW == 3 and d.stride == 1 and d.dilation == 1 and d.pad_t == 1 and d.pad_l == 1 and d.Ho == d.H
                and d.Wo == d.W and d.W % 4 == 0 and d.Cin % 4 == 0 and d.x_ld == 0 and d.y_ld == 0)

    def dwconv_wgrad(self, x, dy, d: ConvDesc, pre_relu=False, dw=None, bn=None):
        if dw is None:
            dw = self.empty(d.KH, d.KW, d.Cin, 1)
        wsp, wsn = self.ws(self.lib.sg_dwconv2d_wgrad_ws_bytes(self.h, C.byref(d)))
        check(self.lib.sg_dwconv2d_wgrad(self.h, self.stream, _dt(x), C.byref(d), _ptr(x), _ptr(dy), _ptr(dw),
                                         int(pre_relu) if bn is None else 0, self._dw_bn(bn), wsp, wsn), "sg_dwconv2d_wgrad")
        return dw

    def bn_train_fwd(self, x, gamma, beta, mm, mv, relu=False, momentum=0.99, eps=1e-3, out=None):
        _chk(x, "x")
        c = x.shape[-1]
        rows = x.numel() // c
        y = out if out is not None else torch.empty_like(x)
        mean, invstd = self.empty(c), self.empty(c)
        wsp, wsn = self.ws(self.lib.sg_bn_ws_bytes(self.h, rows, c))
        check(self.lib.sg_bn_train_fwd(self.h, self.stream, _dt(x), rows, c, _ptr(x), _ptr(gamma), _ptr(beta), _ptr(mm),
                                       _ptr(mv), _ptr(y), _ptr(mean), _ptr(invstd), momentum, eps, int(relu),
                                       int(x.dim() == 4), wsp, wsn), "sg_bn_train_fwd")
        return y, mean, invstd

    def bn_train_fwd_from_tiles(self, x, stats, tiles, gamma, beta, mm, mv, relu=False, momentum=0.99, eps=1e-3, out=None,
                                apply=True):
        c = x.shape[-1]
        rows = x.numel() // c
        y = (out if out is not None else torch.empty_like(x)) if apply else None
        mean, invstd = self.empty(c), self.empty(c)
        wsp, wsn = self.ws(self.lib.sg_bn_tiles_ws_bytes(self.h, int(tiles), c))
        check(self.lib.sg_bn_train_fwd_tiles(self.h, self.stream, _dt(x), rows, c, _ptr(stats), int(tiles), _ptr(mm), _ptr(mv),
                                             _ptr(mean), _ptr(invstd), momentum, eps, int(x.dim() == 4), wsp, wsn),
              "sg_bn_train_fwd_tiles")
        if apply:
            check(self.lib.sg_bn_apply(self.h, self.stream, _dt(x), rows, c, _ptr(x), _ptr(gamma), _ptr(beta), _ptr(mean),
                                       _ptr(invstd), _ptr(y), int(relu)), "sg_bn_apply")
        return y, mean, invstd

    def bn_train_bwd_apply(self, x, dy, gamma, beta, mean, invstd, dgamma, dbeta, relu=False, out=None):
        c = x.shape[-1]
        dx = out if out is not None else torch.empty_like(x)
        check(self.lib.sg_bn_train_bwd_apply(self.h, self.stream, _dt(x), x.numel() // c, c, _ptr(x), _ptr(dy), _ptr(gamma),
                                             _ptr(beta), _ptr(mean), _ptr(invstd), _ptr(dgamma), _ptr(dbeta), _ptr(dx), int(relu)),
              "sg_bn_train_bwd_apply")
        return dx

    def bn_train_bwd(self, x, y, dy, gamma, mean, invstd, relu=False, out=None, dgamma=None, dbeta=None, beta=None):
        c = x.shape[-1]
        rows = x.numel() // c
        dx = out if out is not None else torch.empty_like(x)
        dgamma = dgamma if dgamma is not None else self.empty(c)
        dbeta = dbeta if dbeta is not None else self.empty(c)
        wsp, wsn = self.ws(self.lib.sg_bn_ws_bytes(self.h, rows, c))
        check(self.lib.sg_bn_train_bwd(self.h, self.stream, _dt(x), rows, c, _ptr(x), _ptr(y), _ptr(dy), _ptr(gamma),
                                       _ptr(beta), _ptr(mean), _ptr(invstd), _ptr(dx), _ptr(dgamma), _ptr(dbeta), int(relu),
                                       wsp, wsn),
              "sg_bn_train_bwd")
        return dx, dgamma, dbeta

    def bn_train_bwd_thin_ok(self, x, g, w) -> bool:
        c = x.shape[-1]
        return (x.dtype == torch.float32 and g.dtype == torch.float32 and x.is_contiguous() and g.is_contiguous()
                and bool(self.lib.sg_bn_train_bwd_thin_ok(self.h, SG_F32, x.numel() // c, c, int(w.shape[-1]), int(g.shape[-1]))))

    def bn_train_bwd_thin(self, x, g, w, gamma, mean, invstd, relu=False, out=None, dgamma=None, dbeta=None, beta=None):
        _chk32(x, "x"); _chk32(g, "g"); _chk32(w, "w")
        c, co = x.shape[-1], w.shape[-1]
        rows = x.numel() // c
        assert w.shape[-2] == c and g.numel() // g.shape[-1] == rows and g.shape[-1] >= co
        dx = out if out is not None else torch.empty_like(x)
        dgamma = dgamma if dgamma is not None else self.empty(c)
        dbeta = dbeta if dbeta is not None else self.empty(c)
        wsp, wsn = self.ws(self.lib.sg_bn_ws_bytes(self.h, rows, c))
        check(self.lib.sg_bn_train_bwd_thin(self.h, self.stream, SG_F32, rows, c, int(co), int(g.shape[-1]), _ptr(x), _ptr(g), _ptr(w),
                                            _ptr(gamma), _ptr(beta), _ptr(mean), _ptr(invstd), _ptr(dx), _ptr(dgamma), _ptr(dbeta),
                                            int(relu), wsp, wsn), "sg_bn_train_bwd_thin")
        return dx, dgamma, dbeta

    def bn_infer(self, x, gamma, beta, mm, mv, relu=False, eps=1e-3, out=None):
        _chk(x, "x")
        c = x.shape[-1]
        y = out if out is not None else torch.empty_like(x)
        check(self.lib.sg_bn_infer(self.h, self.stream, _dt(x), x.numel() // c, c, _ptr(x), _ptr(gamma), _ptr(beta),
                                   _ptr(mm), _ptr(mv), _ptr(y), eps, int(relu)), "sg_bn_infer")
        return y

    def act_fwd(self, x, act, out=None):
        _chk(x, "x")
        y = out if out is not None else torch.empty_like(x)
        check(self.lib.sg_act_fwd(self.h, self.stream, _dt(x), act, x.numel(), _ptr(x), _ptr(y)), "sg_act_fwd")
        return y

    def act_bwd(self, y, dy, act, out=None, accumulate=False):
        dx = out if out is not None else torch.empty_like(y)
        check(self.lib.sg_act_bwd(self.h, self.stream, _dt(y), act, y.numel(), _ptr(y), _ptr(dy), _ptr(dx), int(accumulate)),
              "sg_act_bwd")
        return dx

    def add_n(self, xs: Sequence[torch.Tensor], relu=False, out=None):
        assert 1 <= len(xs) <= 8
        for t in xs:
            _chk(t, "add_n operand")
        arr = (C.c_void_p * len(xs))(*[t.data_ptr() for t in xs])
        y = out if out is not None else torch.empty_like(xs[0])
        check(self.lib.sg_add_n(self.h, self.stream, _dt(xs[0]), len(xs), arr, xs[0].numel(), _ptr(y), int(relu)), "sg_add_n")
        return y

    def add2_bn(self, a, b, bn_a=None, bn_b=None, relu=False, infer=False, eps=1e-3, out=None, relu_a=False, relu_b=False):
        _chk(a, "a"); _chk(b, "b")
        c = a.shape[-1]
        y = out if out is not None else torch.empty_like(a)
        pa = [_ptr(t) for t in bn_a] if bn_a is not None else [None] * 4
        pb = [_ptr(t) for t in bn_b] if bn_b is not None else [None] * 4
        check(self.lib.sg_add2_bn(self.h, self.stream, _dt(a), a.numel() // c, c, _ptr(a), _ptr(b), *pa, *pb, _ptr(y), int(relu),
                                  int(infer), float(eps), int(relu_a), int(relu_b)), "sg_add2_bn")
        return y

    def copy_channels(self, src, src_off, dst, dst_off, c, accumulate=False):
        rows = src.numel() // src.shape[-1]
        assert rows == dst.numel() // dst.shape[-1]
        assert src.dtype == dst.dtype, (src.dtype, dst.dtype)
        check(self.lib.sg_copy_channels(self.h, self.stream, _dt(src), rows, c, _ptr(src), src.shape[-1], src_off, _ptr(dst),
                                        dst.shape[-1], dst_off, int(accumulate)), "sg_copy_channels")
        return dst

    def concat(self, xs: Sequence[torch.Tensor], out=None):
        ctot = sum(t.shape[-1] for t in xs)
        y = out if out is not None else self.empty(*xs[0].shape[:-1], ctot, dtype=xs[0].dtype)
        off = 0
        for t in xs:
            self.copy_channels(t, 0, y, off, t.shape[-1])
            off += t.shape[-1]
        return y

    def softmax2_fwd(self, z, out=None):
        _chk32(z, "z")
        assert z.shape[-1] == 2
        p = out if out is not None else torch.empty_like(z)
        check(self.lib.sg_softmax2_fwd(self.h, self.stream, SG_F32, z.numel() // 2, _ptr(z), _ptr(p)), "sg_softmax2_fwd")
        return p

    def softmax2_bwd(self, p, dp, out=None):
        dz = out if out is not None else torch.empty_like(p)
        check(self.lib.sg_softmax2_bwd(self.h, self.stream, SG_F32, p.numel() // 2, _ptr(p), _ptr(dp), _ptr(dz)),
              "sg_softmax2_bwd")
        return dz

    def softmax_fwd(self, z, out=None):
        _chk32(z, "z")
        c = z.shape[-1]
        p = out if out is not None else torch.empty_like(z)
        check(self.lib.sg_softmax_fwd(self.h, self.stream, SG_F32, z.numel() // c, c, _ptr(z), _ptr(p)), "sg_softmax_fwd")
        return p

    def softmax_bwd(self, p, dp, out=None):
        _chk32(p, "p"); _chk32(dp, "dp")
        c = p.shape[-1]
        dz = out if out is not None else torch.empty_like(p)
        check(self.lib.sg_softmax_bwd(self.h, self.stream, SG_F32, p.numel() // c, c, _ptr(p), _ptr(dp), _ptr(dz)),
              "sg_softmax_bwd")
        return dz

    def softmax_branch_fwd(self, z):
        n, b, c = z.shape
        p = torch.empty_like(z)
        check(self.lib.sg_softmax_branch_fwd(self.h, self.stream, _dt(z), n, b, c, _ptr(z), _ptr(p)), "sg_softmax_branch_fwd")
        return p

    def softmax_branch_bwd(self, p, dp):
        n, b, c = p.shape
        dz = torch.empty_like(p)
        check(self.lib.sg_softmax_branch_bwd(self.h, self.stream, _dt(p), n, b, c, _ptr(p), _ptr(dp), _ptr(dz)),
              "sg_softmax_branch_bwd")
        return dz

    def bcast_mul_fwd(self, x, g, mode, out=None, accumulate=False):
        n, h, w, c = x.shape
        y = out if out is not None else torch.empty_like(x)
        check(self.lib.sg_bcast_mul_fwd(self.h, self.stream, _dt(x), n, h * w, c, mode, _ptr(x), _ptr(g), _ptr(y),
                                        int(accumulate)), "sg_bcast_mul_fwd")
        return y

    def bcast_mul_bwd(self, x, g, dy, mode, dx=None, accumulate_dx=False):
        n, h, w, c = x.shape
        if dx is None:
            dx = torch.empty_like(x)
            accumulate_dx = False
        dg = torch.empty_like(g)
        wsp, wsn = self.ws(self.lib.sg_bcast_mul_bwd_ws_bytes(self.h, n, h * w, c, mode))
        check(self.lib.sg_bcast_mul_bwd(self.h, self.stream, _dt(x), n, h * w, c, mode, _ptr(x), _ptr(g), _ptr(dy), _ptr(dx),
                                        _ptr(dg), int(accumulate_dx), wsp, wsn), "sg_bcast_mul_bwd")
        return dx, dg

    def scse_fwd(self, x, s, cl, out=None):
        n, h, w, c = x.shape
        y = out if out is not None else torch.empty_like(x)
        check(self.lib.sg_scse_fwd(self.h, self.stream, _dt(x), n, h * w, c, _ptr(x), _ptr(s), _ptr(cl), _ptr(y)), "sg_scse_fwd")
        return y

    def scse_bwd(self, x, s, cl, dy):
        n, h, w, c = x.shape
        dx, ds, dc = torch.empty_like(x), torch.empty_like(s), torch.empty_like(cl)
        wsp, wsn = self.ws(self.lib.sg_scse_bwd_ws_bytes(self.h, n, h * w, c))
        check(self.lib.sg_scse_bwd(self.h, self.stream, _dt(x), n, h * w, c, _ptr(x), _ptr(s), _ptr(cl), _ptr(dy), _ptr(dx),
                                   _ptr(ds), _ptr(dc), wsp, wsn), "sg_scse_bwd")
        return dx, ds, dc

    def scse_bwd_sums(self, x, s, cl, dy):
        n, h, w, c = x.shape
        ds, dc = torch.empty_like(s), torch.empty_like(cl)
        wsp, wsn = self.ws(self.lib.sg_scse_bwd_ws_bytes(self.h, n, h * w, c))
        check(self.lib.sg_scse_bwd_sums(self.h, self.stream, _dt(x), n, h * w, c, _ptr(x), _ptr(s), _ptr(cl), _ptr(dy), _ptr(ds),
                                        _ptr(dc), wsp, wsn), "sg_scse_bwd_sums")
        return ds, dc

    def scse_bwd_final(self, dy, s, cl, dsp, w, dg, gap_first=True):
        for t, name in ((dy, "dy"), (s, "s"), (cl, "c"), (dsp, "dsp"), (w, "w"), (dg, "dg")):
            _chk32(t, name)
        n, h, w_, c = dy.shape
        assert s.numel() == dsp.numel() == n * h * w_ and cl.numel() == dg.numel() == n * c and w.numel() == c
        dx = torch.empty_like(dy)
        check(self.lib.sg_scse_bwd_final(self.h, self.stream, SG_F32, n, h * w_, c, _ptr(dy), _ptr(s), _ptr(cl), _ptr(dsp), _ptr(w),
                                         _ptr(dg), _ptr(dx), int(bool(gap_first))), "sg_scse_bwd_final")
        return dx

    def bam_fwd(self, x, mc, ms, out=None):
        n, h, w, c = x.shape
        y = out if out is not None else torch.empty_like(x)
        check(self.lib.sg_bam_fwd(self.h, self.stream, _dt(x), n, h * w, c, _ptr(x), _ptr(mc), _ptr(ms), _ptr(y)), "sg_bam_fwd")
        return y

    def bam_bwd(self, x, mc, ms, dy):
        n, h, w, c = x.shape
        dx, dmc, dms = torch.empty_like(x), torch.empty_like(mc), torch.empty_like(ms)
        wsp, wsn = self.ws(self.lib.sg_bam_bwd_ws_bytes(self.h, n, h * w, c))
        check(self.lib.sg_bam_bwd(self.h, self.stream, _dt(x), n, h * w, c, _ptr(x), _ptr(mc), _ptr(ms), _ptr(dy), _ptr(dx),
                                  _ptr(dmc), _ptr(dms), wsp, wsn), "sg_bam_bwd")
        return dx, dmc, dms

    def maxpool_fwd(self, x, k, stride, padding="valid", out=None, want_idx=False):
        n, h, w, c = x.shape
        if padding == "same":
            ho, pt, _ = same_pad(h, k, stride)
            wo, pl, _ = same_pad(w, k, stride)
        else:
            ho, wo, pt, pl = (h - k) // stride + 1, (w - k) // stride + 1, 0, 0
        y = out if out is not None else self.empty(n, ho, wo, c, dtype=x.dtype)
        if want_idx:
            idx = torch.empty(n, ho, wo, c, dtype=torch.uint8, device=self.device)
            check(self.lib.sg_maxpool_fwd_idx(self.h, self.stream, _dt(x), n, h, w, c, k, stride, pt, pl, ho, wo, _ptr(x), _ptr(y),
                                              _ptr(idx)), "sg_maxpool_fwd_idx")
            return y, (k, stride, pt, pl, ho, wo), idx
        check(self.lib.sg_maxpool_fwd(self.h, self.stream, _dt(x), n, h, w, c, k, stride, pt, pl, ho, wo, _ptr(x), _ptr(y)),
              "sg_maxpool_fwd")
        return y, (k, stride, pt, pl, ho, wo)

    def maxpool_bwd_idx(self, dy, idx, xshape, geom, out=None):
        n, h, w, c = xshape
        k, stride, pt, pl, ho, wo = geom
        dx = out if out is not None else self.empty(n, h, w, c, dtype=dy.dtype)
        check(self.lib.sg_maxpool_bwd_idx(self.h, self.stream, _dt(dy), n, h, w, c, k, stride, pt, pl, ho, wo, _ptr(dy), _ptr(idx),
                                          _ptr(dx)), "sg_maxpool_bwd_idx")
        return dx

    def maxpool_bwd(self, x, y, dy, geom, out=None):
        n, h, w, c = x.shape
        k, stride, pt, pl, ho, wo = geom
        dx = out if out is not None else torch.empty_like(x)
        check(self.lib.sg_maxpool_bwd(self.h, self.stream, _dt(x), n, h, w, c, k, stride, pt, pl, ho, wo, _ptr(x), _ptr(y),
                                      _ptr(dy), _ptr(dx)), "sg_maxpool_bwd")
        return dx

    def avgpool_fwd(self, x, kh, kw, out=None):
        n, h, w, c = x.shape
        y = out if out is not None else self.empty(n, h // kh, w // kw, c, dtype=x.dtype)
        wsp, wsn = self.ws(self.lib.sg_avgpool_ws_bytes(self.h, n, h, w, c, kh, kw))
        check(self.lib.sg_avgpool_fwd(self.h, self.stream, _dt(x), n, h, w, c, kh, kw, _ptr(x), _ptr(y), wsp, wsn), "sg_avgpool_fwd")
        return y

    def avgpool_bwd(self, dy, xshape, kh, kw, out=None, accumulate=False):
        n, h, w, c = xshape
        dx = out if out is not None else self.empty(n, h, w, c, dtype=dy.dtype)
        check(self.lib.sg_avgpool_bwd(self.h, self.stream, _dt(dy), n, h, w, c, kh, kw, _ptr(dy), _ptr(dx), int(accumulate)),
              "sg_avgpool_bwd")
        return dx

    def upsample_fwd(self, x, sh, sw=None, out=None, out_ld=0):
        sw = sh if sw is None else sw
        n, h, w, c = x.shape
        y = out if out is not None else self.empty(n, h * sh, w * sw, c, dtype=x.dtype)
        check(self.lib.sg_upsample_nearest_fwd(self.h, self.stream, _dt(x), n, h, w, c, sh, sw, _ptr(x), _ptr(y), out_ld),
              "sg_upsample_nearest_fwd")
        return y

    def upsample_bwd(self, dy, xshape, sh, sw=None, out=None, accumulate=False, dy_ld=0):
        sw = sh if sw is None else sw
        n, h, w, c = xshape
        dx = out if out is not None else self.empty(n, h, w, c, dtype=dy.dtype)
        check(self.lib.sg_upsample_nearest_bwd(self.h, self.stream, _dt(dy), n, h, w, c, sh, sw, _ptr(dy), dy_ld, _ptr(dx),
                                               int(accumulate)), "sg_upsample_nearest_bwd")
        return dx

    def upsample_bilinear_fwd(self, x, sh, sw=None, out=None, out_ld=0):
        sw = sh if sw is None else sw
        n, h, w, c = x.shape
        y = out if out is not None else self.empty(n, h * sh, w * sw, c, dtype=x.dtype)
        check(self.lib.sg_upsample_bilinear_fwd(self.h, self.stream, _dt(x), n, h, w, c, sh, sw, _ptr(x), _ptr(y), out_ld),
              "sg_upsample_bilinear_fwd")
        return y

    def upsample_bilinear_bwd(self, dy, xshape, sh, sw=None, out=None, accumulate=False, dy_ld=0):
        sw = sh if sw is None else sw
        n, h, w, c = xshape
        dx = out if out is not None else self.empty(n, h, w, c, dtype=dy.dtype)
        check(self.lib.sg_upsample_bilinear_bwd(self.h, self.stream, _dt(dy), n, h, w, c, sh, sw, _ptr(dy), dy_ld, _ptr(dx),
                                                int(accumulate)), "sg_upsample_bilinear_bwd")
        return dx

    def loss_fwd(self, kind, p, y_true):
        _chk32(p, "p"); _chk32(y_true, "y_true")
        rows = p.numel() // 2
        out = self.empty(1)
        wsp, wsn = self.ws(self.lib.sg_loss_ws_bytes(self.h, rows))
        check(self.lib.sg_loss_fwd(self.h, self.stream, kind, rows, y_true.shape[-1], _ptr(p), _ptr(y_true), _ptr(out), wsp, wsn),
              "sg_loss_fwd")
        return out

    def loss_bwd(self, kind, p, y_true, scale=1.0, out=None):
        dp = out if out is not None else torch.empty_like(p)
        check(self.lib.sg_loss_bwd(self.h, self.stream, kind, p.numel() // 2, y_true.shape[-1], _ptr(p), _ptr(y_true), _ptr(dp),
                                   float(scale)), "sg_loss_bwd")
        return dp

    def confusion_counts(self, p, y_true, out=None):
        if out is None:
            out = torch.zeros(4, dtype=torch.int64, device=self.device)
        check(self.lib.sg_confusion_counts(self.h, self.stream, p.numel() // 2, y_true.shape[-1], _ptr(p), _ptr(y_true),
                                           C.c_void_p(out.data_ptr())), "sg_confusion_counts")
        return out

    @staticmethod
    def _alpha(alpha, c):
        if alpha is None:
            return None
        if len(alpha) != c:
            raise ValueError(f"{len(alpha)} class weights for {c} classes")
        return (C.c_float * c)(*[float(a) for a in alpha])

    def lossn_fwd(self, kind, p, y_true, alpha=None):
        _chk32(p, "p"); _chk32(y_true, "y_true")
        c = p.shape[-1]
        rows = p.numel() // c
        out = self.empty(1)
        wsp, wsn = self.ws(self.lib.sg_lossn_ws_bytes(self.h, rows))
        check(self.lib.sg_lossn_fwd(self.h, self.stream, kind, rows, c, y_true.shape[-1], self._alpha(alpha, c), _ptr(p),
                                    _ptr(y_true), _ptr(out), wsp, wsn), "sg_lossn_fwd")
        return out

    def lossn_bwd(self, kind, p, y_true, alpha=None, scale=1.0, out=None):
        _chk32(p, "p"); _chk32(y_true, "y_true")
        c = p.shape[-1]
        dp = out if out is not None else torch.empty_like(p)
        check(self.lib.sg_lossn_bwd(self.h, self.stream, kind, p.numel() // c, c, y_true.shape[-1], self._alpha(alpha, c),
                                    _ptr(p), _ptr(y_true), _ptr(dp), float(scale)), "sg_lossn_bwd")
        return dp

    @staticmethod
    def region_desc(region, p, y_true):
        c, y_cols = int(p.shape[-1]), int(y_true.shape[-1])
        rows = p.numel() // c
        if y_true.numel() != rows * y_cols or y_cols not in (c, 2 * c):
            raise ValueError(f"y_true {tuple(y_true.shape)} does not go with p {tuple(p.shape)}: C or 2C columns per pixel")
        if region["point_kind"] == _lib.SG_LOSS_EDGE_FOCAL and y_cols != 2 * c:
            raise ValueError(f"edge_focal_loss needs y_true[..., {2 * c}] (one-hot, then one edge weight per class), got {y_cols} columns")
        if len(region["class_w"]) != c or (region["point_alpha"] is not None and len(region["point_alpha"]) != c):
            raise ValueError(f"the loss carries class weights for another class count than {c}")
        images = int(p.shape[0]) if region["per_image"] and p.dim() > 1 else 1
        d = _lib.RegionDesc(C=c, y_cols=y_cols, images=images, point_kind=int(region["point_kind"]), rows_per_image=rows // images,
                            a=region["a"], b=region["b"], smooth=region["smooth"], gamma=region["gamma"],
                            point_weight=region["point_weight"], region_weight=region["region_weight"])
        for i in range(c):
            d.class_w[i] = region["class_w"][i]
            d.point_alpha[i] = 1.0 if region["point_alpha"] is None else region["point_alpha"][i]
        return d

    def loss_region_fwd(self, region, p, y_true):
        _chk32(p, "p"); _chk32(y_true, "y_true")
        d = self.region_desc(region, p, y_true)
        out, coef = self.empty(3), self.empty(d.images, 2 * d.C)
        wsp, wsn = self.ws(self.lib.sg_loss_region_ws_bytes(self.h, C.byref(d)))
        check(self.lib.sg_loss_region_fwd(self.h, self.stream, C.byref(d), _ptr(p), _ptr(y_true), _ptr(out), _ptr(coef), wsp, wsn),
              "sg_loss_region_fwd")
        return out, coef

    def loss_region_bwd(self, region, p, y_true, coef, scale=1.0, out=None):
        _chk32(p, "p"); _chk32(y_true, "y_true"); _chk32(coef, "coef")
        d = self.region_desc(region, p, y_true)
# ... 254 lines not shown
```

building_detection_amd/runtime.py:

```python
from __future__ import annotations

import math
import os
import time
from typing import Callable, Dict, List, Optional, Sequence

import numpy as np

from . import _lib
from . import fusion
from . import switches
from .graph import KTensor, Node, ParamSpec, collect_nodes, init_array
from . import layers as L
from . import losses as LS

ALIGN = 4


class _Shared:
    __slots__ = ("t",)

    def __init__(self, t):
        self.t = t

# ... 646 lines not shown
        out = []
        while self.next < len(self.buckets) and self.buckets[self.next][2] >= node_index:
            s, e, _ = self.buckets[self.next]
            out.append((s, e))
            self.next += 1
        return out

    def done(self):
        return self.next == len(self.buckets)


def run_segments(segments, arena, transport, lanes=None):
    import contextlib
    marks = []
    for k, seg in enumerate(segments):
        launch, ready = seg[0], seg[1]
        side_launch = seg[2] if len(seg) > 2 else None
        if lanes is not None and k >= 2:
            lanes.wait_on_main(marks[k - 2])
            marks[k - 2] = None
        launch()
        ctx = contextlib.nullcontext()
        mark = None
        if side_launch is not None:
            if lanes is not None:
                lanes.fork()
                with lanes.on_side():
                    side_launch()
                mark = lanes.mark_side()
                ctx = lanes.on_side()
            else:
                side_launch()
        marks.append(mark)
        if transport is not None and ready:
            if lanes is not None and side_launch is None:
                lanes.fork()
                ctx = lanes.on_side()
            with ctx:
                for s, e in ready:
                    transport.allreduce_async(arena[s:e])
    if lanes is not None:
        for ev in marks:
            lanes.wait_on_main(ev)
    if transport is not None:
        transport.join()


_GATES = {"bnb_to": ("SG_BN_PW", "conv2d_dgrad_bnb_ok"), "defer_conv": ("SG_BN_CONV", "conv2d_bn_in_ok"),
          "fused_into": ("SG_UP2_FUSE", "conv2d_up2_ok")}


class _Runtime:

    def __init__(self, model: Model):
        import torch
        from .ops import get_engine
        self.torch = torch
        self.model = model
        dev = int(os.environ.get("LOCAL_RANK", "0")) if torch.cuda.is_available() and torch.cuda.device_count() > 1 else 0
        self.eng = get_engine(dev)
        e = self.eng
        self._gates: Dict[tuple, bool] = {}
        self._x6 = e.lib.sg_get_conv_x6
        self._act_planes: Dict[int, tuple] = {}
        self._act_planes_use: Dict[int, bool] = {}
        self.w_train = e.zeros(max(model._n_train, ALIGN))
        self.g_train = e.zeros(max(model._n_train, ALIGN))
        self.adam_m = e.zeros(max(model._n_train, ALIGN))
        self.adam_v = e.zeros(max(model._n_train, ALIGN))
        self.w_frozen = e.zeros(max(model._n_frozen, ALIGN))
        rng = np.random.default_rng(model.seed)
        host_t = np.zeros(max(model._n_train, ALIGN), np.float32)
        host_n = np.zeros(max(model._n_frozen, ALIGN), np.float32)
        for p in model.params:
            a = init_array(p, rng).reshape(-1)
            (host_t if p.trainable else host_n)[p.offset:p.offset + p.size] = a
        self.w_train.copy_(torch.from_numpy(host_t))
        self.w_frozen.copy_(torch.from_numpy(host_n))
        self._pviews: Dict[int, object] = {}
        self._gviews: Dict[int, object] = {}
        self.values: Dict[int, object] = {}
        self._saved: Dict[int, dict] = {}
        self.bn_stats: Dict[int, tuple] = {}
        self.on_node_done = None
        self._pending = None
        self.node_done_fires = None
        self._planes_key = None
        self._planes_ptr: Dict[tuple, int] = {}
        self._planes_kind: Dict[tuple, int] = {}
        self._planes_arena = None
        self._planes_jobs = None
        self._planes_launch = (0, 0)
        self._planes_dirty = True
        self._w_version = 0
        self._use_planes = switches.get("SG_PREPARED_PLANES")

    def param(self, p: ParamSpec):
        v = self._pviews.get(id(p))
        if v is None:
            arena = self.w_train if p.trainable else self.w_frozen
            v = arena[p.offset:p.offset + p.size].view(p.shape)
            self._pviews[id(p)] = v
        return v

    def grad(self, p: ParamSpec):
        v = self._gviews.get(id(p))
        if v is None:
            v = self.g_train[p.offset:p.offset + p.size].view(p.shape)
            self._gviews[id(p)] = v
        return v

    def to_device(self, a):
        torch = self.torch
        if isinstance(a, torch.Tensor):
            return a if a.is_cuda and a.dtype == torch.float32 else a.to(self.eng.device, torch.float32)
        return torch.from_numpy(np.ascontiguousarray(a, dtype=np.float32)).to(self.eng.device)

    def weights_changed(self):
        self._planes_dirty = True
        self._w_version += 1

    def prepare_into(self, arena, jobs, launch):
        import ctypes as C
        if launch[0]:
            _lib.check(self.eng.lib.sg_prepare_planes(self.eng.h, self.eng.stream, C.c_void_p(self.w_train.data_ptr()),
                                                      C.c_void_p(arena.data_ptr()), C.c_void_p(jobs.data_ptr()), launch[0],
                                                      launch[1]), "sg_prepare_planes")

    def _gate(self, node, mark, x=None) -> bool:
        key = (mark, id(node), 0 if x is None else x.shape[0], self._x6())
        got = self._gates.get(key)
        if got is None:
            c, (switch, ask) = getattr(node, mark), _GATES[mark]
            got = False
            if (c is not None and switches.get(switch) and self.model.compute_dtype == "float32"
                    and (x is None or x.dtype == self.torch.float32)):
                if x is None:
                    _, h, w, cin = c.inputs[0].shape
                    d = self.eng.conv_desc((1, h, w, cin), c.filters, c.k, c.k, c.stride, c.dilation, c.padding)
                else:
                    n, h, w, cout = x.shape
                    d = self.eng.conv_desc((n, h, w, c.inputs[0].shape[-1]), cout, 1, 1, 1, 1, "same")
                got = bool(getattr(self.eng, ask)(d))
            self._gates[key] = got
        return got

    def bnb_on(self, bn_node, x) -> bool:
        return self._gate(bn_node, "bnb_to", x)

    def bn_conv_on(self, bn_node) -> bool:
        return self._gate(bn_node, "defer_conv")

    def planes_in_on(self) -> bool:
        return (self.model.compute_dtype == "float32" and switches.get("SG_ACT_PLANES")
                and int(self.eng.lib.sg_get_conv_x6()) == 1)

    def act_planes(self, node, x, d, make=True):
        if not self.planes_in_on():
            return None
        key = id(node.inputs[0])
        got = self._act_planes.get(key)
        if got is not None and got[0] is x:
            return got[1]
        if not make:
            return None
        use = self._act_planes_use.get(id(node))
        if use is None:
            use = bool(self.eng.conv2d_planes_in(d, False))
            self._act_planes_use[id(node)] = use
        if not use:
            return None
        pl = self.eng.split_planes(x)
        self._act_planes[key] = (x, pl)
        return pl

    def up2_on(self, up_node) -> bool:
        return self._gate(up_node, "fused_into")

    def plane_kind(self, node, tag) -> int:
        return self._planes_kind.get((id(node), tag), 0) if self._planes_ptr else 0

    def planes(self, node, tag):
        return self._planes_ptr.get((id(node), tag))

    def ensure_planes(self, batch: int, training: bool):
        if not self._use_planes:
            return
        import ctypes as C
        e, m, torch = self.eng, self.model, self.torch
        bwd = training or m.optimizer is not None
        key = (int(batch), m.compute_dtype, e.lib.sg_get_conv_x6(), bwd)
        if key != self._planes_key:
            dt = _lib.SG_BF16 if m.compute_dtype == "bfloat16" else _lib.SG_F32
            jobs, ptr_of, kinds, off, blocks = [], {}, {}, 0, 0
            for n in m.nodes:
                sites = getattr(n, "plane_sites", None)
                if sites is None:
                    continue
                for tag, wspec, d, dgrad, phase, head in sites(self, int(batch)):
                    if (phase == "bwd" and not bwd) or not wspec.trainable:
                        continue
                    job, nbytes = _lib.PlanesJob(), C.c_size_t(0)
                    _lib.check(e.lib.sg_conv2d_planes_job(e.h, dt | (_lib.SG_HEAD_F32 if (head and dt == _lib.SG_BF16) else 0),
                                                          C.byref(d), dgrad, C.byref(job), C.byref(nbytes)), "sg_conv2d_planes_job")
                    if job.kind == 0:
                        continue
                    job.w_off, job.out_off, job.block0 = wspec.offset, off, blocks
                    ptr_of[(id(n), tag)] = off
                    kinds[(id(n), tag)] = int(job.kind)
                    off += (nbytes.value + 255) // 256 * 256
                    blocks += job.nblocks
                    jobs.append(job)
            self._planes_key = key
            self._planes_kind = kinds
            self._planes_ptr = {}
            self._planes_arena = self._planes_jobs = None
            self._planes_launch = (len(jobs), blocks)
            if jobs:
                self._planes_arena = torch.empty(off, dtype=torch.uint8, device=e.device)
                arr = (_lib.PlanesJob * len(jobs))(*jobs)
                host = torch.frombuffer(bytearray(bytes(arr)), dtype=torch.uint8)
                self._planes_jobs = host.to(e.device)
                base = self._planes_arena.data_ptr()
                self._planes_ptr = {k: base + o for k, o in ptr_of.items()}
            self._planes_dirty = True
        if self._planes_dirty and self._planes_launch[0]:
            _lib.check(e.lib.sg_prepare_planes(e.h, e.stream, C.c_void_p(self.w_train.data_ptr()),
                                               C.c_void_p(self._planes_arena.data_ptr()), C.c_void_p(self._planes_jobs.data_ptr()),
                                               self._planes_launch[0], self._planes_launch[1]), "sg_prepare_planes")
        self._planes_dirty = False

    def save(self, node, **kw):
        self._saved.setdefault(id(node), {}).update(kw)

    def saved(self, node):
        return self._saved[id(node)]

    def needs_grad(self, sym: KTensor) -> bool:
        return sym.node is not None

    def take_pending(self, sym: KTensor, owned_only: bool = False):
        if self._pending is None or not switches.get("SG_GRAD_ACC"):
            return None
        cur = self._pending.get(id(sym))
        if cur is None or (owned_only and not cur[1]):
            return None
        del self._pending[id(sym)]
        return cur[0]

    def put_back(self, sym: KTensor, t):
        self._pending[id(sym)] = [t, True]

    def shared(self, t):
        return _Shared(t)

    def release(self):
        self.values.clear()
        self._saved.clear()
        self.bn_stats.clear()
        self._act_planes.clear()

    def forward(self, x, training: bool):
        m = self.model
        exp = m.inputs[0].shape[1:]
        if tuple(x.shape[1:]) != tuple(exp):
            raise ValueError(f"input shape {tuple(x.shape)} does not match the model's {(None,) + tuple(exp)}")
        x = x.contiguous()
        self.ensure_planes(x.shape[0], training)
        if m.compute_dtype == "bfloat16":
            x = self.eng.cast(x, self.torch.bfloat16)
        self.values = {id(m.inputs[0]): x}
        self._act_planes.clear()
        if training:
            for n in m.nodes:
                xs = [self.values[id(t)] for t in n.inputs]
                self.values[id(n.output)] = n.forward(self, xs, training)
            return self._as_f32(self.values[id(m.outputs[0])])
        last_use = m._last_use()
        for i, n in enumerate(m.nodes):
            xs = [self.values[id(t)] for t in n.inputs]
            self.values[id(n.output)] = n.forward(self, xs, False)
            for t in n.inputs:
                if last_use.get(id(t)) == i:
                    self.values.pop(id(t), None)
            del xs
        return self._as_f32(self.values[id(m.outputs[0])])

    def _as_f32(self, y):
        return y if y.dtype == self.torch.float32 else self.eng.cast(y, self.torch.float32)

    def backward(self, dout):
        m = self.model
        yout = self.values.get(id(m.outputs[0]))
        if yout is not None and yout.dtype != dout.dtype:
            dout = self.eng.cast(dout, yout.dtype)
        grads: Dict[int, list] = {id(m.outputs[0]): [dout, True]}
        e = self.eng
        hook = self.on_node_done
        for n in reversed(m.nodes):
            slot = grads.pop(id(n.output), None)
            if slot is None:
                if hook is not None:
                    if self.node_done_fires is None or self.node_done_fires(n.index):
                        e.join_side()
                    hook(n.index)
                continue
            dy = slot[0]
            if isinstance(dy, L.DeferredGrad) and not dy.taken_by(n):
                dy = dy.materialise(e)
            xs = [self.values[id(t)] for t in n.inputs]
            y = self.values[id(n.output)]
            self._pending = grads
            dxs = n.backward(self, xs, y, dy)
            self._pending = None
            for sym, g in zip(n.inputs, dxs):
                if g is None or sym.node is None:
                    continue
                fresh = True
                if isinstance(g, _Shared):
                    g, fresh = g.t, False
                elif g is dy:
                    fresh = False
                cur = grads.get(id(sym))
                if cur is not None:
                    if isinstance(g, L.DeferredGrad):
                        g, fresh = g.materialise(e), True
                    if isinstance(cur[0], L.DeferredGrad):
                        cur[0], cur[1] = cur[0].materialise(e), True
                if cur is None:
                    grads[id(sym)] = [g, fresh]

                elif cur[1]:
                    e.add_n([cur[0], g], out=cur[0])
                elif fresh:
                    e.add_n([cur[0], g], out=g)
                    grads[id(sym)] = [g, True]
                else:
                    grads[id(sym)] = [e.add_n([cur[0], g]), True]
            self._saved.pop(id(n), None)
            if hook is not None:
                if self.node_done_fires is None or self.node_done_fires(n.index):
                    e.join_side()
                hook(n.index)
        self._act_planes.clear()
        e.join_side()
```

building_detection_amd/switches.py:

```python
import os

SWITCHES = {
    "SG_BN_ADD": ("eq1", "1", "BatchNormalization layers in front of a residual Add ride in the add kernel; off: their own launch"),
    "SG_BN_SUMS": ("eq1", "1", "BatchNormalization backward sums come from the depthwise dgrad's epilogue; off: their own reduction"),
    "SG_BN_DEFER": ("eq1", "1", "BatchNormalization(+ReLU) in front of a SeparableConv2D is applied in the depthwise gather"),
    "SG_BN_PW": ("eq1", "0", "the BatchNormalization backward apply rides in the A path of the pointwise dgrad (bit-identical, a loss in the step)"),
    "SG_BN_CONV": ("ne0", "1", "BatchNormalization layers in front of thin 1x1 / patch-kernel convolutions ride in their loader; 0: own launch"),
    "SG_THIN_GRAD_BN": ("ne0", "1", "a thin 1x1 convolution's input gradient is evaluated inside the BatchNormalization backward in front of it; 0: written out"),
    "SG_SCSE_LOWRANK": ("ne0", "1", "an scSE block's input gradient is written once, by a final kernel that adds the two gates' rank-one terms; 0: three passes"),
    "SG_ACT_PLANES": ("ne0", "1", "activation planes made once per tensor and step, kept for the planes-in filter gradient; 0: split in every launch"),
    "SG_UP2_FUSE": ("ne0", "1", "UpSampling2D(2) -> Conv2D 3x3 as one sub-pixel launch; 0: a pair of launches"),
    "SG_GRAD_ACC": ("eq1", "1", "the gradient of a two-consumer block input is summed in the dgrad epilogue; off: by a separate add"),
    "SG_PREPARED_PLANES": ("ne0", "1", "weight planes prepared once per optimiser step; 0: rebuilt inside every convolution call"),
    "SG_JIT_LANES": ("ne0", "1", "the captured training step keeps filter gradients on a side lane; 0: inline in one linear graph"),
    "SG_JIT_LANE_BLOCKS": ("int", "24", "filter-gradient blocks per segment of the captured step's side lane"),
    "SG_SIDE_WGRAD": ("int", "1", "filter gradients on the side stream: 1 all, 2 the GEMM ones only, 3 the depthwise ones only, 0 none"),
    "SG_SIDE_KEEP_GIB": ("float", "4", "GiB of side-stream operands held before the main stream joins the side stream and drops them"),
    "SG_TRACE_MARK": ("eq1", "0", "bracket the roofline kernel set with marker kernels for a kernel trace (read once, at import)"),
    "SG_CONV_NOTHIN": ("flag", "", "thin 1x1 streaming kernels off (the library reads the same variable)"),
    "SG_COMM_INIT_TIMEOUT": ("float", "180", "seconds sg_comm_init may take per rank before every rank gives up together"),
}

_RULES = {
    "eq1": lambda v: v == "1",
    "ne0": lambda v: v != "0",
    "int": int,
    "float": float,
}


def get(name: str):
    kind, default, _ = SWITCHES[name]
    if kind == "flag":
        return name in os.environ
    return _RULES[kind](os.environ.get(name, default))
```

include/segengine.h:

```cpp
#ifndef SEGENGINE_H_
#define SEGENGINE_H_

#include <stddef.h>
#include <stdint.h>

#ifdef __cplusplus
extern "C" {
#endif

#define SG_ABI_VERSION 1

#define SG_EINVAL   (-1)
#define SG_EWORKSPACE (-2)
#define SG_EUNSUPPORTED (-3)
#define SG_ECOMM    (-4)

#define SG_F32  0
#define SG_BF16 1
#define SG_I64  2
#define SG_HEAD_F32 0x100
#define SG_X_UP2 0x200

#define SG_EPI_BIAS 1
#define SG_EPI_RELU 2
// ... 127 lines not shown
size_t sg_bias_grad_ws_bytes(const sg_ctx* ctx, int64_t rows, int C);
int sg_bias_grad(sg_ctx* ctx, void* stream, int dtype, int64_t rows, int C, int ld, const void* dy,
                 void* dbias, void* ws, size_t ws_bytes);

typedef struct sg_dw_bnsums {
  const void *x, *mean, *invstd, *gamma, *beta;
  int relu;
  void *dgamma, *dbeta;
  void* ws;
  size_t ws_bytes;
} sg_dw_bnsums;
int sg_dwconv2d_fwd(sg_ctx* ctx, void* stream, int dtype, const sg_conv_desc* d, const void* x,
                    const void* w, void* y, int pre_relu, const sg_bn_in* bn);
size_t sg_dwconv2d_dgrad_bnsums_ws_bytes(const sg_ctx* ctx, const sg_conv_desc* d);
int sg_dwconv2d_dgrad(sg_ctx* ctx, void* stream, int dtype, const sg_conv_desc* d, const void* dy,
                      const void* w, const void* x_for_mask, void* dx, int pre_relu, const void* res,
                      const sg_dw_bnsums* sums);
size_t sg_dwconv2d_wgrad_ws_bytes(const sg_ctx* ctx, const sg_conv_desc* d);
int sg_dwconv2d_wgrad(sg_ctx* ctx, void* stream, int dtype, const sg_conv_desc* d, const void* x,
                      const void* dy, void* dw, int pre_relu, const sg_bn_in* bn, void* ws, size_t ws_bytes);

#define SG_DW_FWD 0
#define SG_DW_DGRAD 1
#define SG_DW_WGRAD 2
#define SG_DWK_GENERIC 0
#define SG_DWK_RUN 1
#define SG_DWK_STRIP 2
typedef struct sg_dw_plan {
  int family, V, RR, lc, HS, nhs, count, gx, gy, S, seg_V, seg_TX, seg_gx, seg_S, bn, res, sums;
  size_t ws_bytes;
} sg_dw_plan;
int sg_dwconv2d_plan(const sg_ctx* ctx, int dtype, const sg_conv_desc* d, int direction, int aligned, int sums, sg_dw_plan* out);

int sg_dense_fwd(sg_ctx* ctx, void* stream, int dtype, int rows, int in, int out, const void* x,
                 const void* w, const void* bias, void* y, int flags);

#define SG_WS_PREPARED ((size_t)-1)
typedef struct sg_planes_job {
  int64_t w_off, out_off;
  int32_t kind;
  int32_t K, N, Kpad, Npad, Ck, Ckp, s_tap, s_k, s_n, npl;
  int32_t block0, nblocks;
  int32_t kd;
} sg_planes_job;
int sg_get_conv_x6(void);
int sg_conv2d_planes_job(const sg_ctx* ctx, int dtype, const sg_conv_desc* d, int dgrad, sg_planes_job* out, size_t* bytes);
int sg_prepare_planes(sg_ctx* ctx, void* stream, const void* w_arena, void* planes_arena, const sg_planes_job* jobs_dev,
                      int njobs, int total_blocks);

size_t sg_bn_ws_bytes(const sg_ctx* ctx, int64_t rows, int C);
int sg_bn_train_fwd(sg_ctx* ctx, void* stream, int dtype, int64_t rows, int C, const void* x,
                    const void* gamma, const void* beta, void* moving_mean, void* moving_var, void* y,
                    void* save_mean, void* save_invstd, float momentum, float eps, int relu,
                    int unbiased_update, void* ws, size_t ws_bytes);
int sg_add2_bn(sg_ctx* ctx, void* stream, int dtype, int64_t rows, int C, const void* a, const void* b,
               const void* a_mean, const void* a_invstd, const void* a_gamma, const void* a_beta, const void* b_mean,
               const void* b_invstd, const void* b_gamma, const void* b_beta, void* y, int relu, int infer, float eps,
               int a_relu, int b_relu);
int sg_bn_train_bwd(sg_ctx* ctx, void* stream, int dtype, int64_t rows, int C, const void* x,
                    const void* y, const void* dy, const void* gamma, const void* beta, const void* save_mean,
                    const void* save_invstd, void* dx, void* dgamma, void* dbeta, int relu, void* ws,
                    size_t ws_bytes);
int sg_bn_train_bwd_apply(sg_ctx* ctx, void* stream, int dtype, int64_t rows, int C, const void* x, const void* dy,
                          const void* gamma, const void* beta, const void* save_mean, const void* save_invstd,
                          const void* dgamma, const void* dbeta, void* dx, int relu);
int sg_bn_train_bwd_thin_ok(const sg_ctx* ctx, int dtype, int64_t rows, int C, int CO, int y_ld);
int sg_bn_train_bwd_thin(sg_ctx* ctx, void* stream, int dtype, int64_t rows, int C, int CO, int y_ld, const void* x,
                         const void* g, const void* w, const void* gamma, const void* beta, const void* save_mean,
                         const void* save_invstd, void* dx, void* dgamma, void* dbeta, int relu, void* ws, size_t ws_bytes);
int sg_bn_infer(sg_ctx* ctx, void* stream, int dtype, int64_t rows, int C, const void* x,
                const void* gamma, const void* beta, const void* moving_mean, const void* moving_var,
                void* y, float eps, int relu);

#define SG_BN_FWD 0
#define SG_BN_APPLY 1
#define SG_BN_BWD 2
#define SG_BN_BWD_APPLY 3
#define SG_BN_ADD2 4
typedef struct sg_bn_plan_t {
  int V, cols, prow, gx, gy, seg_V, seg_TX, seg_TY, seg_gx, seg_S, fused, fin_lanes;
  size_t ws_bytes;
} sg_bn_plan_t;
int sg_bn_plan(const sg_ctx* ctx, int dtype, int64_t rows, int C, int pass, int aligned, sg_bn_plan_t* out);

typedef struct sg_seg_plan_t {
  int V, TX, TY, gx, S;
  size_t part_bytes;
} sg_seg_plan_t;
int sg_seg_plan(const sg_ctx* ctx, int nout, int nseg, int64_t rows, int C, int vec, int wide8, sg_seg_plan_t* out);

#define SG_ACT_RELU 0
#define SG_ACT_SIGMOID 1
int sg_act_fwd(sg_ctx* ctx, void* stream, int dtype, int act, int64_t n, const void* x, void* y);
int sg_act_bwd(sg_ctx* ctx, void* stream, int dtype, int act, int64_t n, const void* y, const void* dy,
               void* dx, int accumulate);
int sg_add_n(sg_ctx* ctx, void* stream, int dtype, int k, const void* const* xs, int64_t n, void* y,
             int relu);
int sg_copy_channels(sg_ctx* ctx, void* stream, int dtype, int64_t rows, int C, const void* src,
                     int src_ld, int src_off, void* dst, int dst_ld, int dst_off, int accumulate);
int sg_softmax2_fwd(sg_ctx* ctx, void* stream, int dtype, int64_t rows, const void* z, void* p);
int sg_softmax2_bwd(sg_ctx* ctx, void* stream, int dtype, int64_t rows, const void* p, const void* dp,
                    void* dz);
int sg_softmax_fwd(sg_ctx* ctx, void* stream, int dtype, int64_t rows, int C, const void* z, void* p);
int sg_softmax_bwd(sg_ctx* ctx, void* stream, int dtype, int64_t rows, int C, const void* p, const void* dp,
                   void* dz);
int sg_softmax_branch_fwd(sg_ctx* ctx, void* stream, int dtype, int N, int B, int C, const void* z,
                          void* p);
int sg_softmax_branch_bwd(sg_ctx* ctx, void* stream, int dtype, int N, int B, int C, const void* p,
                          const void* dp, void* dz);

int sg_bcast_mul_fwd(sg_ctx* ctx, void* stream, int dtype, int N, int64_t HW, int C, int mode,
                     const void* x, const void* g, void* y, int accumulate);
size_t sg_bcast_mul_bwd_ws_bytes(const sg_ctx* ctx, int N, int64_t HW, int C, int mode);
int sg_bcast_mul_bwd(sg_ctx* ctx, void* stream, int dtype, int N, int64_t HW, int C, int mode,
                     const void* x, const void* g, const void* dy, void* dx, void* dg, int accumulate_dx,
                     void* ws, size_t ws_bytes);
int sg_scse_fwd(sg_ctx* ctx, void* stream, int dtype, int N, int64_t HW, int C, const void* x,
                const void* s, const void* c, void* y);
size_t sg_scse_bwd_ws_bytes(const sg_ctx* ctx, int N, int64_t HW, int C);
int sg_scse_bwd(sg_ctx* ctx, void* stream, int dtype, int N, int64_t HW, int C, const void* x,
                const void* s, const void* c, const void* dy, void* dx, void* ds, void* dc, void* ws,
                size_t ws_bytes);
int sg_scse_bwd_sums(sg_ctx* ctx, void* stream, int dtype, int N, int64_t HW, int C, const void* x, const void* s,
                     const void* c, const void* dy, void* ds, void* dc, void* ws, size_t ws_bytes);
int sg_scse_bwd_final(sg_ctx* ctx, void* stream, int dtype, int N, int64_t HW, int C, const void* dy, const void* s,
                      const void* c, const void* dsp, const void* w, const void* dg, void* dx, int gap_first);
int sg_bam_fwd(sg_ctx* ctx, void* stream, int dtype, int N, int64_t HW, int C, const void* x,
               const void* mc, const void* ms, void* y);
size_t sg_bam_bwd_ws_bytes(const sg_ctx* ctx, int N, int64_t HW, int C);
int sg_bam_bwd(sg_ctx* ctx, void* stream, int dtype, int N, int64_t HW, int C, const void* x,
               const void* mc, const void* ms, const void* dy, void* dx, void* dmc, void* dms, void* ws,
               size_t ws_bytes);

int sg_maxpool_fwd(sg_ctx* ctx, void* stream, int dtype, int N, int H, int W, int C, int k, int stride,
                   int pad_t, int pad_l, int Ho, int Wo, const void* x, void* y);
int sg_maxpool_bwd(sg_ctx* ctx, void* stream, int dtype, int N, int H, int W, int C, int k, int stride,
                   int pad_t, int pad_l, int Ho, int Wo, const void* x, const void* y, const void* dy,
                   void* dx);
int sg_maxpool_fwd_idx(sg_ctx* ctx, void* stream, int dtype, int N, int H, int W, int C, int k, int stride,
                       int pad_t, int pad_l, int Ho, int Wo, const void* x, void* y, void* idx);
int sg_maxpool_bwd_idx(sg_ctx* ctx, void* stream, int dtype, int N, int H, int W, int C, int k, int stride,
                       int pad_t, int pad_l, int Ho, int Wo, const void* dy, const void* idx, void* dx);
size_t sg_avgpool_ws_bytes(const sg_ctx* ctx, int N, int H, int W, int C, int kh, int kw);
int sg_avgpool_fwd(sg_ctx* ctx, void* stream, int dtype, int N, int H, int W, int C, int kh, int kw,
                   const void* x, void* y, void* ws, size_t ws_bytes);
int sg_avgpool_bwd(sg_ctx* ctx, void* stream, int dtype, int N, int H, int W, int C, int kh, int kw,
                   const void* dy, void* dx, int accumulate);
int sg_upsample_nearest_fwd(sg_ctx* ctx, void* stream, int dtype, int N, int H, int W, int C, int sh,
                            int sw, const void* x, void* y, int y_ld);
int sg_upsample_nearest_bwd(sg_ctx* ctx, void* stream, int dtype, int N, int H, int W, int C, int sh,
                            int sw, const void* dy, int dy_ld, void* dx, int accumulate);
int sg_upsample_bilinear_fwd(sg_ctx* ctx, void* stream, int dtype, int N, int H, int W, int C, int sh,
                             int sw, const void* x, void* y, int y_ld);
int sg_upsample_bilinear_bwd(sg_ctx* ctx, void* stream, int dtype, int N, int H, int W, int C, int sh,
                             int sw, const void* dy, int dy_ld, void* dx, int accumulate);

#define SG_LOSS_CE2 0
#define SG_LOSS_FOCAL 1
#define SG_LOSS_EDGE_FOCAL 2
size_t sg_loss_ws_bytes(const sg_ctx* ctx, int64_t rows);
int sg_loss_fwd(sg_ctx* ctx, void* stream, int kind, int64_t rows, int y_cols, const void* p,
                const void* y_true, void* loss_out, void* ws, size_t ws_bytes);
int sg_loss_bwd(sg_ctx* ctx, void* stream, int kind, int64_t rows, int y_cols, const void* p,
                const void* y_true, void* dp, float grad_scale);
int sg_confusion_counts(sg_ctx* ctx, void* stream, int64_t rows, int y_cols, const void* p,
                        const void* y_true, void* out_i64x4);
// ... 151 lines not shown
```

Measured before the change: 234.8 tiles/s.

## Write BN and upsample outputs directly into concat slices, read gradients strided

BatchNormalization and UpSampling2D producers now write their output straight into a channel slice of a preallocated concatenation buffer through a pixel-stride argument. In backward, the BN and upsample kernels read their slice of the concat gradient in place instead of copying it out. This removes the concat copy kernels and the gradient split copies in DeepLabv3+'s ASPP and decoder concatenations. The cost is scalar loads and stores when the stride breaks 16-byte alignment, plus densify copies for consumers that cannot take strided gradients.

```diff
diff --git a/building_detection_amd/_lib.py b/building_detection_amd/_lib.py
--- a/building_detection_amd/_lib.py
+++ b/building_detection_amd/_lib.py
@@ -254,6 +254,12 @@
     "sg_bn_infer": (_i, [_vp, _vp, _i, _i64, _i, _vp, _vp, _vp, _vp, _vp, _vp, _f, _i]),
     "sg_add2_bn": (_i, [_vp, _vp, _i, _i64, _i] + [_vp] * 11 + [_i, _i, _f, _i, _i]),
     "sg_bn_plan": (_i, [_vp, _i, _i64, _i, _i, _i, C.POINTER(BnPlan)]),
+    "sg_bn_train_fwd_ld": (_i, [_vp, _vp, _i, _i64, _i, _vp, _vp, _vp, _vp, _vp, _vp, _vp, _vp, _f, _f, _i, _i, _vp, _sz, _i]),
+    "sg_bn_apply_ld": (_i, [_vp, _vp, _i, _i64, _i, _vp, _vp, _vp, _vp, _vp, _vp, _i, _i]),
+    "sg_bn_infer_ld": (_i, [_vp, _vp, _i, _i64, _i, _vp, _vp, _vp, _vp, _vp, _vp, _f, _i, _i]),
+    "sg_bn_train_bwd_ld": (_i, [_vp, _vp, _i, _i64, _i, _vp, _vp, _vp, _vp, _vp, _vp, _vp, _vp, _vp, _vp, _i, _vp, _sz, _i]),
+    "sg_bn_train_bwd_apply_ld": (_i, [_vp, _vp, _i, _i64, _i] + [_vp] * 9 + [_i, _i]),
+    "sg_slice_ok": (_i, [_vp, _i, _i64, _i, _i, _i]),
     "sg_seg_plan": (_i, [_vp, _i, _i, _i64, _i, _i, _i, C.POINTER(SegPlan)]),
     "sg_act_fwd": (_i, [_vp, _vp, _i, _i, _i64, _vp, _vp]),
     "sg_act_bwd": (_i, [_vp, _vp, _i, _i, _i64, _vp, _vp, _vp, _i]),
diff --git a/building_detection_amd/csrc/norm.hip b/building_detection_amd/csrc/norm.hip
--- a/building_detection_amd/csrc/norm.hip
+++ b/building_detection_amd/csrc/norm.hip
@@ -19,6 +19,25 @@
 __device__ __forceinline__ float bn_dx(float x, float g, float mean, float invstd, float gamma, float dgamma, float dbeta, float inv_n) {
   const float xh = (x - mean) * invstd;
   return gamma * invstd * (g - dbeta * inv_n - xh * dgamma * inv_n);
+}
+
+template <int V, bool SV, typename T>
+__device__ __forceinline__ void ldv_slice(const T* __restrict__ p, float (&o)[V]) {
+  if constexpr (SV) {
+    ldv<V>(p, o);
+  } else {
+#pragma unroll
+    for (int i = 0; i < V; ++i) o[i] = ld1<T>(p + i);
+  }
+}
+template <int V, bool SV, typename T>
+__device__ __forceinline__ void stv_slice(T* __restrict__ p, const float (&o)[V]) {
+  if constexpr (SV) {
+    stv<V>(p, o);
+  } else {
+#pragma unroll
+    for (int i = 0; i < V; ++i) st1<T>(p + i, o[i]);
+  }
 }
 
 template <typename T>
@@ -65,7 +84,7 @@
   float mv[V], iv[V], gm[V], bt[V];
 };
 
-template <typename T, int MODE>
+template <typename T, int MODE, bool SV = true>
 struct BnBwdOp {
   static constexpr int NOUT = 2;
   const T* __restrict__ x;
@@ -78,6 +97,7 @@
   float* dgamma;
   float* dbeta;
   int C;
+  int dy_ld;
 
   template <int V>
   __device__ __forceinline__ BnCtx<V> begin(int, int c) const {
@@ -94,7 +114,7 @@
   __device__ __forceinline__ void accum(int, int64_t r, int c, float (&acc)[2][V], const BnCtx<V>& k) const {
     float xv[V], gv[V], yv[V];
     ldv<V>(x + r * C + c, xv);
-    ldv<V>(dy + r * C + c, gv);
+    ldv_slice<V, SV>(dy + r * dy_ld + c, gv);
     if constexpr (MODE == 1) ldv<V>(y + r * C + c, yv);
     bn_mask<MODE>(gv, xv, yv, k.mv, k.iv, k.gm, k.bt);
 #pragma unroll
@@ -180,11 +200,11 @@
   }
 };
 
-template <int V, typename T>
+template <int V, typename T, bool SV = true>
 __global__ void bn_apply_kernel(const T* __restrict__ x, const float* __restrict__ mean,
                                 const float* __restrict__ invstd, const float* __restrict__ gamma,
                                 const float* __restrict__ beta, T* __restrict__ y, int64_t rows, int C, int relu,
-                                float eps, int infer, FastDiv fd_cv) {
+                                float eps, int infer, FastDiv fd_cv, int y_ld) {
   const uint32_t cv = C / V;
   const uint32_t total = (uint32_t)(rows * cv);
   const uint32_t stride = gridDim.x * blockDim.x;
@@ -204,17 +224,17 @@
       if (relu) t = fmaxf(t, 0.f);
       o[k] = t;
     }
-    stv<V>(y + r * C + c, o);
-  }
-}
-
-template <int V, typename T, int MODE>
+    stv_slice<V, SV>(y + r * y_ld + c, o);
+  }
+}
+
+template <int V, typename T, int MODE, bool SV = true>
 __global__ void bn_bwd_apply_kernel(const T* __restrict__ x, const T* __restrict__ y,
                                     const T* __restrict__ dy, const float* __restrict__ mean,
                                     const float* __restrict__ invstd, const float* __restrict__ gamma,
                                     const float* __restrict__ beta, const float* __restrict__ dgamma,
                                     const float* __restrict__ dbeta, T* __restrict__ dx, int64_t rows, int C,
-                                    FastDiv fd_cv) {
+                                    FastDiv fd_cv, int dy_ld) {
   const uint32_t cv = C / V;
   const uint32_t total = (uint32_t)(rows * cv);
   const uint32_t stride = gridDim.x * blockDim.x;
@@ -224,7 +244,7 @@
     const int c = (int)(i - (uint32_t)r * cv) * V;
     float xv[V], gv[V], mv[V], iv[V], gam[V], dg[V], db[V], o[V];
     ldv<V>(x + r * C + c, xv);
-    ldv<V>(dy + r * C + c, gv);
+    ldv_slice<V, SV>(dy + r * dy_ld + c, gv);
     ldv<V>(mean + c, mv);
     ldv<V>(invstd + c, iv);
     ldv<V>(gamma + c, gam);
@@ -250,11 +270,12 @@
   }
 }
 
-template <int V, typename T>
+template <int V, typename T, bool SV = true>
 __global__ __launch_bounds__(256) void bn_apply_cols_kernel(const T* __restrict__ x, const float* __restrict__ mean,
                                                             const float* __restrict__ invstd, const float* __restrict__ gamma,
                                                             const float* __restrict__ beta, T* __restrict__ y, int64_t rows,
-                                                            int C, int relu, float eps, int infer, int prow, FastDiv fd_cv) {
+                                                            int C, int relu, float eps, int infer, int prow, FastDiv fd_cv,
+                                                            int y_ld) {
   const uint32_t i0 = blockIdx.x * 256u + threadIdx.x, cv = (uint32_t)(C / V);
   const uint32_t r0 = fd_div(i0, fd_cv);
   const int c = (int)(i0 - r0 * cv) * V;
@@ -275,7 +296,7 @@
       if (relu) t = fmaxf(t, 0.f);
       o[k] = t;
     }
-    stv<V>(y + r * C + c, o);
+    stv_slice<V, SV>(y + r * y_ld + c, o);
   };
   const int64_t stride = prow, gstep = (int64_t)gridDim.y * 4 * prow;
   for (int64_t r = (int64_t)blockIdx.y * 4 * prow + r0; r < rows; r += gstep) {
@@ -297,13 +318,13 @@
 }
 constexpr int BN_APPLY_PERIODS = 4;
 
-template <int V, typename T, int MODE>
+template <int V, typename T, int MODE, bool SV = true>
 __global__ __launch_bounds__(256) void bn_bwd_apply_cols_kernel(const T* __restrict__ x, const T* __restrict__ y,
                                                                 const T* __restrict__ dy, const float* __restrict__ mean,
                                                                 const float* __restrict__ invstd, const float* __restrict__ gamma,
                                                                 const float* __restrict__ beta, const float* __restrict__ dgamma,
                                                                 const float* __restrict__ dbeta, T* __restrict__ dx, int64_t rows,
-                                                                int C, int prow, FastDiv fd_cv) {
+                                                                int C, int prow, FastDiv fd_cv, int dy_ld) {
   const uint32_t i0 = blockIdx.x * 256u + threadIdx.x, cv = (uint32_t)(C / V);
   const uint32_t r0 = fd_div(i0, fd_cv);
   const int c = (int)(i0 - r0 * cv) * V;
@@ -328,8 +349,8 @@
       float x0[V], x1[V], g0[V], g1[V], y0[V], y1[V];
       ldv<V>(x + r * C + c, x0);
       ldv<V>(x + (r + stride) * C + c, x1);
-      ldv<V>(dy + r * C + c, g0);
-      ldv<V>(dy + (r + stride) * C + c, g1);
+      ldv_slice<V, SV>(dy + r * dy_ld + c, g0);
+      ldv_slice<V, SV>(dy + (r + stride) * dy_ld + c, g1);
       if constexpr (MODE == 1) {
         ldv<V>(y + r * C + c, y0);
         ldv<V>(y + (r + stride) * C + c, y1);
@@ -339,7 +360,7 @@
     } else {
       float x0[V], g0[V], y0[V];
       ldv<V>(x + r * C + c, x0);
-      ldv<V>(dy + r * C + c, g0);
+      ldv_slice<V, SV>(dy + r * dy_ld + c, g0);
       if constexpr (MODE == 1) ldv<V>(y + r * C + c, y0);
       one(x0, g0, y0, r);
     }
@@ -532,6 +553,24 @@
   return 0;
 }
 
+inline int bn_check_ld(int64_t rows, int C, int ld, const char* who) {
+  SG_CHECK_ARG(ld == 0 || ld >= C, "%s: pixel stride %d < C = %d", who, ld, C);
+  SG_CHECK_ARG(rows * (int64_t)(ld ? ld : C) < (1ll << 31), "%s: strided tensor exceeds 2^31 elements", who);
+  return 0;
+}
+
+struct BnSlice { bool aligned; int ld, vec; };
+inline BnSlice bn_slice(int dtype, const void* s, int C, int ld) {
+  const bool sa = sg_all_aligned16({s});
+  if (!ld || ld == C) return {sa, C, 1};
+  return {true, ld, (sa && ((int64_t)ld * (dtype == SG_BF16 ? 2 : 4)) % 16 == 0) ? 1 : 0};
+}
+
+template <class F>
+inline int bn_with_slice(const BnSlice& s, F&& fn) {
+  return s.vec ? fn(std::true_type{}) : fn(std::false_type{});
+}
+
 inline int bn_refuse(const BnPlan& pl, const char* who, const void* ws, size_t ws_bytes) {
   if (pl.refused) {
     sg_set_error("%s: needs C %% 4 == 0, 16-byte aligned tensors and a column grid; apply the BatchNormalization and add instead", who);
@@ -559,33 +598,38 @@
 
 template <typename T>
 int launch_bn_apply(hipStream_t st, const BnPlan& pl, const T* x, const float* mean, const float* invstd, const float* gamma,
-                    const float* beta, T* y, int64_t rows, int C, int relu, float eps, int infer) {
+                    const float* beta, T* y, int64_t rows, int C, int relu, float eps, int infer, const BnSlice& ys) {
   const FastDiv fd = make_fastdiv((uint32_t)(C / pl.V));
   const dim3 grid((unsigned)pl.gx, (unsigned)pl.gy);
   bn_with_form(pl, [&](auto v, auto cols) {
     constexpr int V = decltype(v)::value;
-    if constexpr (decltype(cols)::value)
-      hipLaunchKernelGGL((bn_apply_cols_kernel<V, T>), grid, dim3(256), 0, st, x, mean, invstd, gamma, beta, y, rows, C, relu, eps,
-                         infer, pl.prow, fd);
-    else
-      hipLaunchKernelGGL((bn_apply_kernel<V, T>), grid, dim3(256), 0, st, x, mean, invstd, gamma, beta, y, rows, C, relu, eps, infer, fd);
+    bn_with_slice(ys, [&](auto sv) {
+      constexpr bool SV = decltype(sv)::value;
+      if constexpr (decltype(cols)::value)
+        hipLaunchKernelGGL((bn_apply_cols_kernel<V, T, SV>), grid, dim3(256), 0, st, x, mean, invstd, gamma, beta, y, rows, C, relu, eps,
+                           infer, pl.prow, fd, ys.ld);
+      else
+        hipLaunchKernelGGL((bn_apply_kernel<V, T, SV>), grid, dim3(256), 0, st, x, mean, invstd, gamma, beta, y, rows, C, relu, eps, infer,
+                           fd, ys.ld);
+      return 0;
+    });
   });
   SG_LAUNCH_CHECK(pl.cols ? "bn_apply_cols_kernel" : "bn_apply_kernel");
   return 0;
 }
 
-template <typename T, int MODE>
-int launch_bn_bwd_apply(hipStream_t st, const BnPlan& pl, const BnBwdOp<T, MODE>& q, T* dx, int64_t rows) {
+template <typename T, int MODE, bool SV>
+int launch_bn_bwd_apply(hipStream_t st, const BnPlan& pl, const BnBwdOp<T, MODE, SV>& q, T* dx, int64_t rows) {
   const FastDiv fd = make_fastdiv((uint32_t)(q.C / pl.V));
   const dim3 grid((unsigned)pl.gx, (unsigned)pl.gy);
   bn_with_form(pl, [&](auto v, auto cols) {
     constexpr int V = decltype(v)::value;
     if constexpr (decltype(cols)::value)
-      hipLaunchKernelGGL((bn_bwd_apply_cols_kernel<V, T, MODE>), grid, dim3(256), 0, st, q.x, q.y, q.dy, q.mean, q.invstd, q.gamma,
-                         q.beta, q.dgamma, q.dbeta, dx, rows, q.C, pl.prow, fd);
+      hipLaunchKernelGGL((bn_bwd_apply_cols_kernel<V, T, MODE, SV>), grid, dim3(256), 0, st, q.x, q.y, q.dy, q.mean, q.invstd, q.gamma,
+                         q.beta, q.dgamma, q.dbeta, dx, rows, q.C, pl.prow, fd, q.dy_ld);
     else
-      hipLaunchKernelGGL((bn_bwd_apply_kernel<V, T, MODE>), grid, dim3(256), 0, st, q.x, q.y, q.dy, q.mean, q.invstd, q.gamma, q.beta,
-                         q.dgamma, q.dbeta, dx, rows, q.C, fd);
+      hipLaunchKernelGGL((bn_bwd_apply_kernel<V, T, MODE, SV>), grid, dim3(256), 0, st, q.x, q.y, q.dy, q.mean, q.invstd, q.gamma, q.beta,
+                         q.dgamma, q.dbeta, dx, rows, q.C, fd, q.dy_ld);
   });
   SG_LAUNCH_CHECK(pl.cols ? "bn_bwd_apply_cols_kernel" : "bn_bwd_apply_kernel");
   return 0;
@@ -610,13 +654,16 @@
 inline int64_t add2_chunk_rows(int64_t rows, int C) { return rows * C < (1ll << 31) ? rows : (((1ll << 31) - 1) / C) & ~1ll; }
 
 int bn_apply_entry(const char* who, sg_ctx* ctx, void* stream, int dtype, int64_t rows, int C, const void* x, const void* gamma,
-                   const void* beta, const void* mean, const void* invstd, void* y, int relu, float eps, int infer) {
+                   const void* beta, const void* mean, const void* invstd, void* y, int relu, float eps, int infer,
+                   int y_ld) {
   if (int e = bn_check(ctx, dtype, rows, C, false, who)) return e;
+  if (int e = bn_check_ld(rows, C, y_ld, who)) return e;
   SG_CHECK_ARG(x && gamma && beta && mean && invstd && y, "%s: bad argument", who);
-  const BnPlan pl = plan_bn(ctx->num_cus, dtype, rows, C, SG_BN_APPLY, sg_all_aligned16({x, y}));
+  const BnSlice ys = bn_slice(dtype, y, C, y_ld);
+  const BnPlan pl = plan_bn(ctx->num_cus, dtype, rows, C, SG_BN_APPLY, sg_all_aligned16({x}) && ys.aligned);
   SG_DTYPE_SWITCH(dtype, who, {
     return launch_bn_apply<T>((hipStream_t)stream, pl, (const T*)x, (const float*)mean, (const float*)invstd, (const float*)gamma,
-                              (const float*)beta, (T*)y, rows, C, relu, eps, infer);
+                              (const float*)beta, (T*)y, rows, C, relu, eps, infer, ys);
   });
   return 0;
 }
@@ -649,16 +696,25 @@
 int sg_bn_train_fwd(sg_ctx* ctx, void* stream, int dtype, int64_t rows, int C, const void* x, const void* gamma, const void* beta,
                     void* moving_mean, void* moving_var, void* y, void* save_mean, void* save_invstd, float momentum, float eps,
                     int relu, int unbiased_update, void* ws, size_t ws_bytes) {
+  return sg_bn_train_fwd_ld(ctx, stream, dtype, rows, C, x, gamma, beta, moving_mean, moving_var, y, save_mean, save_invstd, momentum, eps,
+                            relu, unbiased_update, ws, ws_bytes, 0);
+}
+
+int sg_bn_train_fwd_ld(sg_ctx* ctx, void* stream, int dtype, int64_t rows, int C, const void* x, const void* gamma, const void* beta,
+                       void* moving_mean, void* moving_var, void* y, void* save_mean, void* save_invstd, float momentum, float eps,
+                       int relu, int unbiased_update, void* ws, size_t ws_bytes, int y_ld) {
   if (int e = bn_check(ctx, dtype, rows, C, false, "sg_bn_train_fwd")) return e;
+  if (int e = bn_check_ld(rows, C, y_ld, "sg_bn_train_fwd")) return e;
   SG_CHECK_ARG(x && gamma && beta && moving_mean && moving_var && y && save_mean && save_invstd, "sg_bn_train_fwd: bad argument");
-  const BnPlan pl = plan_bn(ctx->num_cus, dtype, rows, C, SG_BN_FWD, sg_all_aligned16({x, y}));
+  const BnSlice ys = bn_slice(dtype, y, C, y_ld);
+  const BnPlan pl = plan_bn(ctx->num_cus, dtype, rows, C, SG_BN_FWD, sg_all_aligned16({x}) && ys.aligned);
   if (int e = bn_refuse(pl, "sg_bn_train_fwd", ws, ws_bytes)) return e;
   SG_DTYPE_SWITCH(dtype, "sg_bn_train_fwd", {
     const BnStatsOp<T> op = {(const T*)x, C, rows, (float*)moving_mean, (float*)moving_var, (float*)save_mean, (float*)save_invstd,
                              momentum, eps, unbiased_update};
     if (int e = seg_reduce_launch(op, pl.seg, 1, rows, C, (float*)ws, (hipStream_t)stream, "bn_stats")) return e;
     return launch_bn_apply<T>((hipStream_t)stream, pl, op.x, op.save_mean, op.save_invstd, (const float*)gamma, (const float*)beta, (T*)y, rows, C, relu,
-                              eps, 0);
+                              eps, 0, ys);
   });
   return 0;
 }
@@ -666,17 +722,29 @@
 int sg_bn_train_bwd(sg_ctx* ctx, void* stream, int dtype, int64_t rows, int C, const void* x, const void* y, const void* dy,
                     const void* gamma, const void* beta, const void* save_mean, const void* save_invstd, void* dx, void* dgamma,
                     void* dbeta, int relu, void* ws, size_t ws_bytes) {
+  return sg_bn_train_bwd_ld(ctx, stream, dtype, rows, C, x, y, dy, gamma, beta, save_mean, save_invstd, dx, dgamma, dbeta, relu, ws,
+                            ws_bytes, 0);
+}
+
+int sg_bn_train_bwd_ld(sg_ctx* ctx, void* stream, int dtype, int64_t rows, int C, const void* x, const void* y, const void* dy,
+                       const void* gamma, const void* beta, const void* save_mean, const void* save_invstd, void* dx, void* dgamma,
+                       void* dbeta, int relu, void* ws, size_t ws_bytes, int dy_ld) {
   if (int e = bn_check(ctx, dtype, rows, C, false, "sg_bn_train_bwd")) return e;
+  if (int e = bn_check_ld(rows, C, dy_ld, "sg_bn_train_bwd")) return e;
   SG_CHECK_ARG(x && dy && gamma && save_mean && save_invstd && dx && dgamma && dbeta, "sg_bn_train_bwd: bad argument");
   SG_CHECK_ARG(!relu || y || beta, "sg_bn_train_bwd: relu set but neither y nor beta given");
-  const BnPlan pl = plan_bn(ctx->num_cus, dtype, rows, C, SG_BN_BWD, sg_all_aligned16({x, dy, dx, relu ? y : nullptr}));
+  const BnSlice ds = bn_slice(dtype, dy, C, dy_ld);
+  const BnPlan pl = plan_bn(ctx->num_cus, dtype, rows, C, SG_BN_BWD, sg_all_aligned16({x, dx, relu ? y : nullptr}) && ds.aligned);
   if (int e = bn_refuse(pl, "sg_bn_train_bwd", ws, ws_bytes)) return e;
   SG_DTYPE_SWITCH(dtype, "sg_bn_train_bwd", {
     return bn_with_mode(relu, beta, [&](auto m) -> int {
-      const BnBwdOp<T, decltype(m)::value> op = {(const T*)x, (const T*)y, (const T*)dy, (const float*)save_mean, (const float*)save_invstd,
-                                                 (const float*)gamma, (const float*)beta, (float*)dgamma, (float*)dbeta, C};
-      if (int e = seg_reduce_launch(op, pl.seg, 1, rows, C, (float*)ws, (hipStream_t)stream, "bn_bwd_reduce")) return e;
-      return launch_bn_bwd_apply((hipStream_t)stream, pl, op, (T*)dx, rows);
+      return bn_with_slice(ds, [&](auto sv) -> int {
+        const BnBwdOp<T, decltype(m)::value, decltype(sv)::value> op = {
+            (const T*)x, (const T*)y, (const T*)dy, (const float*)save_mean, (const float*)save_invstd, (const float*)gamma,
+            (const float*)beta, (float*)dgamma, (float*)dbeta, C, ds.ld};
+        if (int e = seg_reduce_launch(op, pl.seg, 1, rows, C, (float*)ws, (hipStream_t)stream, "bn_bwd_reduce")) return e;
+        return launch_bn_bwd_apply((hipStream_t)stream, pl, op, (T*)dx, rows);
+      });
     });
   });
   return 0;
@@ -685,15 +753,26 @@
 int sg_bn_train_bwd_apply(sg_ctx* ctx, void* stream, int dtype, int64_t rows, int C, const void* x, const void* dy, const void* gamma,
                           const void* beta, const void* save_mean, const void* save_invstd, const void* dgamma, const void* dbeta,
                           void* dx, int relu) {
+  return sg_bn_train_bwd_apply_ld(ctx, stream, dtype, rows, C, x, dy, gamma, beta, save_mean, save_invstd, dgamma, dbeta, dx, relu, 0);
+}
+
+int sg_bn_train_bwd_apply_ld(sg_ctx* ctx, void* stream, int dtype, int64_t rows, int C, const void* x, const void* dy, const void* gamma,
+                             const void* beta, const void* save_mean, const void* save_invstd, const void* dgamma, const void* dbeta,
+                             void* dx, int relu, int dy_ld) {
   if (int e = bn_check(ctx, dtype, rows, C, false, "sg_bn_train_bwd_apply")) return e;
+  if (int e = bn_check_ld(rows, C, dy_ld, "sg_bn_train_bwd_apply")) return e;
   SG_CHECK_ARG(x && dy && gamma && save_mean && save_invstd && dx && dgamma && dbeta, "sg_bn_train_bwd_apply: bad argument");
   SG_CHECK_ARG(!relu || beta, "sg_bn_train_bwd_apply: relu needs beta (the mask is recomputed from x)");
-  const BnPlan pl = plan_bn(ctx->num_cus, dtype, rows, C, SG_BN_BWD_APPLY, sg_all_aligned16({x, dy, dx}));
+  const BnSlice ds = bn_slice(dtype, dy, C, dy_ld);
+  const BnPlan pl = plan_bn(ctx->num_cus, dtype, rows, C, SG_BN_BWD_APPLY, sg_all_aligned16({x, dx}) && ds.aligned);
   SG_DTYPE_SWITCH(dtype, "sg_bn_train_bwd_apply", {
     return bn_with_mode(relu, beta, [&](auto m) -> int {
-      const BnBwdOp<T, decltype(m)::value> op = {(const T*)x, nullptr, (const T*)dy, (const float*)save_mean, (const float*)save_invstd,
-                                                 (const float*)gamma, (const float*)beta, (float*)dgamma, (float*)dbeta, C};
-      return launch_bn_bwd_apply((hipStream_t)stream, pl, op, (T*)dx, rows);
+      return bn_with_slice(ds, [&](auto sv) -> int {
+        const BnBwdOp<T, decltype(m)::value, decltype(sv)::value> op = {
+            (const T*)x, nullptr, (const T*)dy, (const float*)save_mean, (const float*)save_invstd, (const float*)gamma,
+            (const float*)beta, (float*)dgamma, (float*)dbeta, C, ds.ld};
+        return launch_bn_bwd_apply((hipStream_t)stream, pl, op, (T*)dx, rows);
+      });
     });
   });
   return 0;
@@ -736,12 +815,28 @@
 
 int sg_bn_apply(sg_ctx* ctx, void* stream, int dtype, int64_t rows, int C, const void* x, const void* gamma,
                 const void* beta, const void* mean, const void* invstd, void* y, int relu) {
-  return bn_apply_entry("sg_bn_apply", ctx, stream, dtype, rows, C, x, gamma, beta, mean, invstd, y, relu, 0.f, 0);
+  return bn_apply_entry("sg_bn_apply", ctx, stream, dtype, rows, C, x, gamma, beta, mean, invstd, y, relu, 0.f, 0, 0);
+}
+
+int sg_bn_apply_ld(sg_ctx* ctx, void* stream, int dtype, int64_t rows, int C, const void* x, const void* gamma,
+                   const void* beta, const void* mean, const void* invstd, void* y, int relu, int y_ld) {
+  return bn_apply_entry("sg_bn_apply", ctx, stream, dtype, rows, C, x, gamma, beta, mean, invstd, y, relu, 0.f, 0, y_ld);
 }
 
 int sg_bn_infer(sg_ctx* ctx, void* stream, int dtype, int64_t rows, int C, const void* x, const void* gamma,
                 const void* beta, const void* moving_mean, const void* moving_var, void* y, float eps, int relu) {
-  return bn_apply_entry("sg_bn_infer", ctx, stream, dtype, rows, C, x, gamma, beta, moving_mean, moving_var, y, relu, eps, 1);
+  return bn_apply_entry("sg_bn_infer", ctx, stream, dtype, rows, C, x, gamma, beta, moving_mean, moving_var, y, relu, eps, 1, 0);
+}
+
+int sg_bn_infer_ld(sg_ctx* ctx, void* stream, int dtype, int64_t rows, int C, const void* x, const void* gamma,
+                   const void* beta, const void* moving_mean, const void* moving_var, void* y, float eps, int relu, int y_ld) {
+  return bn_apply_entry("sg_bn_infer", ctx, stream, dtype, rows, C, x, gamma, beta, moving_mean, moving_var, y, relu, eps, 1, y_ld);
+}
+
+int sg_slice_ok(const sg_ctx* ctx, int dtype, int64_t rows, int C, int ld, int off) {
+  if (!ctx || (dtype != SG_F32 && dtype != SG_BF16) || rows <= 0 || C <= 0 || off < 0 || ld < off + C) return 0;
+  const int eb = dtype == SG_BF16 ? 2 : 4;
+  return C % 4 == 0 && ((int64_t)off * eb) % 16 == 0 && ((int64_t)ld * eb) % 16 == 0 && rows * (int64_t)ld < (1ll << 31);
 }
 
 int sg_add2_bn(sg_ctx* ctx, void* stream, int dtype, int64_t rows, int C, const void* a, const void* b, const void* a_mean,
diff --git a/building_detection_amd/fusion.py b/building_detection_amd/fusion.py
--- a/building_detection_amd/fusion.py
+++ b/building_detection_amd/fusion.py
@@ -166,6 +166,29 @@
                 n.bnb_to = prod
 
 
+def concat_inplace(nodes, outs):
+    for n in nodes:
+        if not isinstance(n, L._ConcatNode) or len(n.output.shape) != 4:
+            continue
+        n.inplace = [None] * len(n.inputs)
+        off = 0
+        for i, t in enumerate(n.inputs):
+            c = t.shape[-1]
+            root = root_of(t)
+            p_ = root.node
+            ok = p_ is not None and sum(1 for u in n.inputs if u is t) == 1 and sole_consumer(root, outs) is n
+            if ok and isinstance(p_, L._BNNode):
+                ok = (p_.defer_to is None and p_.defer_add is None and p_.defer_conv is None and p_.sums_from is None
+                      and p_.bnb_to is None and (root is t or p_.relu))
+            elif ok and isinstance(p_, L._UpNode):
+                ok = p_.fused_into is None and root is t
+            else:
+                ok = False
+            if ok:
+                n.inplace[i], p_.concat_slot = p_, (n, i, off)
+            off += c
+
+
 RULES = (bias_and_stats, up2_conv, absorb_relu, bn_add, bn_sums, bn_sums_via_add, bn_gather, bn_conv, thin_grad, scse_lowrank,
          bn_backward_in_pw)
 
@@ -174,3 +197,4 @@
     outs = {id(t) for t in outputs}
     for rule in RULES:
         rule(nodes, outs)
+    concat_inplace(nodes, outs)
diff --git a/building_detection_amd/layers.py b/building_detection_amd/layers.py
--- a/building_detection_amd/layers.py
+++ b/building_detection_amd/layers.py
@@ -488,6 +488,7 @@
         self.sums_from = None
         self.defer_conv = None
         self.bnb_to = None
+        self.concat_slot = None
 
     def build(self, x):
         c = x.shape[-1]
@@ -506,13 +507,15 @@
                 defer = self.defer_to is not None or self.defer_add is not None or (self.defer_conv is not None and rt.bn_conv_on(self))
                 y, mean, invstd = e.bn_train_fwd_from_tiles(x, st[0], st[1], rt.param(self.gamma), rt.param(self.beta),
                                                             rt.param(self.mm), rt.param(self.mv), relu=self.relu,
-                                                            momentum=self.momentum, eps=self.epsilon, apply=not defer)
+                                                            momentum=self.momentum, eps=self.epsilon, apply=not defer,
+                                                            out=None if defer else rt.concat_out(self, x))
                 if defer:
                     rt.save(self, mean=mean, invstd=invstd, deferred=True)
                     return x
             else:
                 y, mean, invstd = e.bn_train_fwd(x, rt.param(self.gamma), rt.param(self.beta), rt.param(self.mm),
-                                                 rt.param(self.mv), relu=self.relu, momentum=self.momentum, eps=self.epsilon)
+                                                 rt.param(self.mv), relu=self.relu, momentum=self.momentum, eps=self.epsilon,
+                                                 out=rt.concat_out(self, x))
             rt.save(self, mean=mean, invstd=invstd, deferred=False)
             return y
         if self.defer_add is not None and x.shape[-1] % 4 == 0:
@@ -523,7 +526,10 @@
             return x
         rt.save(self, deferred=False)
         return e.bn_infer(x, rt.param(self.gamma), rt.param(self.beta), rt.param(self.mm), rt.param(self.mv),
-                          relu=self.relu, eps=self.epsilon)
+                          relu=self.relu, eps=self.epsilon, out=rt.concat_out(self, x))
+
+    def takes_strided_dy(self, rt):
+        return not (rt.saved(self).get("sums_done") and self.bnb_to is not None)
 
     def backward(self, rt, xs, y, dy):
         (x,) = xs
@@ -589,6 +595,9 @@
         n, _, b, c = x.shape
         return e.softmax_branch_fwd(x.view(n, b, c)).view(x.shape)
 
+    def takes_strided_dy(self, rt):
+        return self.fused_away
+
     def backward(self, rt, xs, y, dy):
         if self.fused_away:
             return [rt.shared(dy)]
@@ -739,6 +748,7 @@
         self.size = size
         self.interpolation = interpolation
         self.fused_into = None
+        self.concat_slot = None
 
     def build(self, x):
         _, h, w, c = x.shape
@@ -746,10 +756,13 @@
 
     def forward(self, rt, xs, training):
         if self.interpolation == "bilinear":
-            return rt.eng.upsample_bilinear_fwd(xs[0], self.size)
+            return rt.eng.upsample_bilinear_fwd(xs[0], self.size, out=rt.concat_out(self, xs[0]))
         if self.fused_into is not None and rt.up2_on(self):
             return xs[0]
-        return rt.eng.upsample_fwd(xs[0], self.size)
+        return rt.eng.upsample_fwd(xs[0], self.size, out=rt.concat_out(self, xs[0]))
+
+    def takes_strided_dy(self, rt):
+        return self.fused_into is None
 
     def backward(self, rt, xs, y, dy):
         if self.interpolation == "bilinear":
@@ -814,14 +827,35 @@
             assert t.shape[:-1] == base, f"concat shapes differ: {[t.shape for t in xs]}"
         return self.connect(xs, base + (sum(t.shape[-1] for t in xs),))
 
-    def forward(self, rt, xs, training):
-        return rt.eng.concat(xs)
+    inplace = None
+
+    def forward(self, rt, xs, training):
+        buf = rt.take_concat_buf(self)
+        if buf is None or any(t.dtype != buf.dtype or tuple(t.shape[:-1]) != tuple(buf.shape[:-1]) for t in xs):
+            rt.save(self, placed=None)
+            return rt.eng.concat(xs)
+        placed, off, ctot = [], 0, buf.shape[-1]
+        for t in xs:
+            c = t.shape[-1]
+            here = (not t.is_contiguous() and t.data_ptr() == buf.data_ptr() + off * buf.element_size()
+                    and t.stride(-2) == ctot and t.stride(-1) == 1)
+            if not here:
+                rt.eng.copy_channels(t, 0, buf, off, c)
+            placed.append(here)
+            off += c
+        rt.save(self, placed=placed)
+        return buf
 
     def backward(self, rt, xs, y, dy):
         outs, off = [], 0
-        for t, sym in zip(xs, self.inputs):
+        placed = rt.saved(self).get("placed") if id(self) in rt._saved else None
+        ctot = dy.shape[-1]
+        for i, (t, sym) in enumerate(zip(xs, self.inputs)):
             c = t.shape[-1]
-            if rt.needs_grad(sym):
+            if (rt.needs_grad(sym) and placed is not None and placed[i] and dy.is_contiguous()
+                    and rt.eng.slice_ok(dy.dtype, dy.numel() // ctot, c, ctot, off)):
+                outs.append(rt.shared(dy[..., off:off + c]))
+            elif rt.needs_grad(sym):
                 g = rt.eng.empty(*t.shape, dtype=dy.dtype)
                 rt.eng.copy_channels(dy, off, g, 0, c)
                 outs.append(g)
diff --git a/building_detection_amd/ops.py b/building_detection_amd/ops.py
--- a/building_detection_amd/ops.py
+++ b/building_detection_amd/ops.py
@@ -44,6 +44,19 @@
         raise _lib.SgError(f"{name}: expected float32 or bfloat16 storage, got {t.dtype}")
     if not t.is_contiguous():
         raise _lib.SgError(f"{name}: tensor must be contiguous")
+
+
+def slice_ld(t: torch.Tensor) -> int:
+    if t.is_contiguous():
+        return 0
+    ld = int(t.stride(-2)) if t.dim() >= 2 else 0
+    want, step = [1], ld
+    for n in reversed(t.shape[:-1]):
+        want.insert(0, step)
+        step *= n
+    if ld < t.shape[-1] or any(n > 1 and s != w for n, s, w in zip(t.shape, t.stride(), want)):
+        raise _lib.SgError(f"not a channel slice of a contiguous tensor: shape {tuple(t.shape)}, strides {tuple(t.stride())}")
+    return ld
 
 
 def _chk32(t: torch.Tensor, name: str):
@@ -505,9 +518,9 @@
         y = out if out is not None else torch.empty_like(x)
         mean, invstd = self.empty(c), self.empty(c)
         wsp, wsn = self.ws(self.lib.sg_bn_ws_bytes(self.h, rows, c))
-        check(self.lib.sg_bn_train_fwd(self.h, self.stream, _dt(x), rows, c, _ptr(x), _ptr(gamma), _ptr(beta), _ptr(mm),
-                                       _ptr(mv), _ptr(y), _ptr(mean), _ptr(invstd), momentum, eps, int(relu),
-                                       int(x.dim() == 4), wsp, wsn), "sg_bn_train_fwd")
+        check(self.lib.sg_bn_train_fwd_ld(self.h, self.stream, _dt(x), rows, c, _ptr(x), _ptr(gamma), _ptr(beta), _ptr(mm),
+                                          _ptr(mv), _ptr(y), _ptr(mean), _ptr(invstd), momentum, eps, int(relu),
+                                          int(x.dim() == 4), wsp, wsn, slice_ld(y)), "sg_bn_train_fwd")
         return y, mean, invstd
 
     def bn_train_fwd_from_tiles(self, x, stats, tiles, gamma, beta, mm, mv, relu=False, momentum=0.99, eps=1e-3, out=None,
@@ -521,16 +534,16 @@
                                              _ptr(mean), _ptr(invstd), momentum, eps, int(x.dim() == 4), wsp, wsn),
               "sg_bn_train_fwd_tiles")
         if apply:
-            check(self.lib.sg_bn_apply(self.h, self.stream, _dt(x), rows, c, _ptr(x), _ptr(gamma), _ptr(beta), _ptr(mean),
-                                       _ptr(invstd), _ptr(y), int(relu)), "sg_bn_apply")
+            check(self.lib.sg_bn_apply_ld(self.h, self.stream, _dt(x), rows, c, _ptr(x), _ptr(gamma), _ptr(beta), _ptr(mean),
+                                          _ptr(invstd), _ptr(y), int(relu), slice_ld(y)), "sg_bn_apply")
         return y, mean, invstd
 
     def bn_train_bwd_apply(self, x, dy, gamma, beta, mean, invstd, dgamma, dbeta, relu=False, out=None):
         c = x.shape[-1]
         dx = out if out is not None else torch.empty_like(x)
-        check(self.lib.sg_bn_train_bwd_apply(self.h, self.stream, _dt(x), x.numel() // c, c, _ptr(x), _ptr(dy), _ptr(gamma),
-                                             _ptr(beta), _ptr(mean), _ptr(invstd), _ptr(dgamma), _ptr(dbeta), _ptr(dx), int(relu)),
-              "sg_bn_train_bwd_apply")
+        check(self.lib.sg_bn_train_bwd_apply_ld(self.h, self.stream, _dt(x), x.numel() // c, c, _ptr(x), _ptr(dy), _ptr(gamma),
+                                                _ptr(beta), _ptr(mean), _ptr(invstd), _ptr(dgamma), _ptr(dbeta), _ptr(dx), int(relu),
+                                                slice_ld(dy)), "sg_bn_train_bwd_apply")
         return dx
 
     def bn_train_bwd(self, x, y, dy, gamma, mean, invstd, relu=False, out=None, dgamma=None, dbeta=None, beta=None):
@@ -540,9 +553,11 @@
         dgamma = dgamma if dgamma is not None else self.empty(c)
         dbeta = dbeta if dbeta is not None else self.empty(c)
         wsp, wsn = self.ws(self.lib.sg_bn_ws_bytes(self.h, rows, c))
-        check(self.lib.sg_bn_train_bwd(self.h, self.stream, _dt(x), rows, c, _ptr(x), _ptr(y), _ptr(dy), _ptr(gamma),
-                                       _ptr(beta), _ptr(mean), _ptr(invstd), _ptr(dx), _ptr(dgamma), _ptr(dbeta), int(relu),
-                                       wsp, wsn),
+        if relu and beta is None and y is not None and not y.is_contiguous():
+            raise _lib.SgError("bn_train_bwd: a ReLU mask read from y needs a dense y (pass beta: the mask is then recomputed from x)")
+        check(self.lib.sg_bn_train_bwd_ld(self.h, self.stream, _dt(x), rows, c, _ptr(x), _ptr(y), _ptr(dy), _ptr(gamma),
+                                          _ptr(beta), _ptr(mean), _ptr(invstd), _ptr(dx), _ptr(dgamma), _ptr(dbeta), int(relu),
+                                          wsp, wsn, slice_ld(dy)),
               "sg_bn_train_bwd")
         return dx, dgamma, dbeta
 
@@ -569,8 +584,8 @@
         _chk(x, "x")
         c = x.shape[-1]
         y = out if out is not None else torch.empty_like(x)
-        check(self.lib.sg_bn_infer(self.h, self.stream, _dt(x), x.numel() // c, c, _ptr(x), _ptr(gamma), _ptr(beta),
-                                   _ptr(mm), _ptr(mv), _ptr(y), eps, int(relu)), "sg_bn_infer")
+        check(self.lib.sg_bn_infer_ld(self.h, self.stream, _dt(x), x.numel() // c, c, _ptr(x), _ptr(gamma), _ptr(beta),
+                                      _ptr(mm), _ptr(mv), _ptr(y), eps, int(relu), slice_ld(y)), "sg_bn_infer")
         return y
 
     def act_fwd(self, x, act, out=None):
@@ -608,9 +623,19 @@
         rows = src.numel() // src.shape[-1]
         assert rows == dst.numel() // dst.shape[-1]
         assert src.dtype == dst.dtype, (src.dtype, dst.dtype)
-        check(self.lib.sg_copy_channels(self.h, self.stream, _dt(src), rows, c, _ptr(src), src.shape[-1], src_off, _ptr(dst),
-                                        dst.shape[-1], dst_off, int(accumulate)), "sg_copy_channels")
+        check(self.lib.sg_copy_channels(self.h, self.stream, _dt(src), rows, c, _ptr(src), slice_ld(src) or src.shape[-1], src_off,
+                                        _ptr(dst), slice_ld(dst) or dst.shape[-1], dst_off, int(accumulate)), "sg_copy_channels")
         return dst
+
+    def slice_ok(self, dtype, rows, c, ld, off) -> bool:
+        if dtype not in (torch.float32, torch.bfloat16):
+            return False
+        return bool(self.lib.sg_slice_ok(self.h, SG_BF16 if dtype == torch.bfloat16 else SG_F32, int(rows), int(c), int(ld), int(off)))
+
+    def dense(self, t):
+        if t.is_contiguous():
+            return t
+        return self.copy_channels(t, 0, self.empty(*t.shape, dtype=t.dtype), 0, t.shape[-1])
 
     def concat(self, xs: Sequence[torch.Tensor], out=None):
         ctot = sum(t.shape[-1] for t in xs)
@@ -777,6 +802,7 @@
         sw = sh if sw is None else sw
         n, h, w, c = x.shape
         y = out if out is not None else self.empty(n, h * sh, w * sw, c, dtype=x.dtype)
+        out_ld = out_ld or slice_ld(y)
         check(self.lib.sg_upsample_nearest_fwd(self.h, self.stream, _dt(x), n, h, w, c, sh, sw, _ptr(x), _ptr(y), out_ld),
               "sg_upsample_nearest_fwd")
         return y
@@ -785,6 +811,7 @@
         sw = sh if sw is None else sw
         n, h, w, c = xshape
         dx = out if out is not None else self.empty(n, h, w, c, dtype=dy.dtype)
+        dy_ld = dy_ld or slice_ld(dy)
         check(self.lib.sg_upsample_nearest_bwd(self.h, self.stream, _dt(dy), n, h, w, c, sh, sw, _ptr(dy), dy_ld, _ptr(dx),
                                                int(accumulate)), "sg_upsample_nearest_bwd")
         return dx
@@ -793,6 +820,7 @@
         sw = sh if sw is None else sw
         n, h, w, c = x.shape
         y = out if out is not None else self.empty(n, h * sh, w * sw, c, dtype=x.dtype)
+        out_ld = out_ld or slice_ld(y)
         check(self.lib.sg_upsample_bilinear_fwd(self.h, self.stream, _dt(x), n, h, w, c, sh, sw, _ptr(x), _ptr(y), out_ld),
               "sg_upsample_bilinear_fwd")
         return y
@@ -801,6 +829,7 @@
         sw = sh if sw is None else sw
         n, h, w, c = xshape
         dx = out if out is not None else self.empty(n, h, w, c, dtype=dy.dtype)
+        dy_ld = dy_ld or slice_ld(dy)
         check(self.lib.sg_upsample_bilinear_bwd(self.h, self.stream, _dt(dy), n, h, w, c, sh, sw, _ptr(dy), dy_ld, _ptr(dx),
                                                 int(accumulate)), "sg_upsample_bilinear_bwd")
         return dx
diff --git a/building_detection_amd/runtime.py b/building_detection_amd/runtime.py
--- a/building_detection_amd/runtime.py
+++ b/building_detection_amd/runtime.py
@@ -752,6 +752,7 @@
         self.values: Dict[int, object] = {}
         self._saved: Dict[int, dict] = {}
         self.bn_stats: Dict[int, tuple] = {}
+        self._concat_bufs: Dict[int, object] = {}
         self.on_node_done = None
         self._pending = None
         self.node_done_fires = None
@@ -843,6 +844,25 @@
         pl = self.eng.split_planes(x)
         self._act_planes[key] = (x, pl)
         return pl
+
+    def concat_out(self, node, x):
+        slot = node.concat_slot
+        if slot is None or not switches.get("SG_CONCAT_INPLACE"):
+            return None
+        cn, _, off = slot
+        lead = (x.shape[0],) + tuple(node.output.shape[1:-1])
+        c, ctot = node.output.shape[-1], cn.output.shape[-1]
+        if not self.eng.slice_ok(x.dtype, int(np.prod(lead)), c, ctot, off):
+            return None
+        buf = self._concat_bufs.get(id(cn))
+        if buf is None:
+            buf = self._concat_bufs[id(cn)] = self.eng.empty(*lead, ctot, dtype=x.dtype)
+        elif buf.dtype != x.dtype or tuple(buf.shape[:-1]) != lead:
+            return None
+        return buf[..., off:off + c]
+
+    def take_concat_buf(self, concat_node):
+        return self._concat_bufs.pop(id(concat_node), None)
 
     def up2_on(self, up_node) -> bool:
         return self._gate(up_node, "fused_into")
@@ -929,6 +949,7 @@
         self._saved.clear()
         self.bn_stats.clear()
         self._act_planes.clear()
+        self._concat_bufs.clear()
 
     def forward(self, x, training: bool):
         m = self.model
@@ -940,6 +961,7 @@
         if m.compute_dtype == "bfloat16":
             x = self.eng.cast(x, self.torch.bfloat16)
         self.values = {id(m.inputs[0]): x}
+        self._concat_bufs.clear()
         self._act_planes.clear()
         if training:
             for n in m.nodes:
@@ -978,6 +1000,10 @@
             dy = slot[0]
             if isinstance(dy, L.DeferredGrad) and not dy.taken_by(n):
                 dy = dy.materialise(e)
+            elif not isinstance(dy, L.DeferredGrad) and not dy.is_contiguous():
+                takes = getattr(n, "takes_strided_dy", None)
+                if takes is None or not takes(self):
+                    dy = e.dense(dy)
             xs = [self.values[id(t)] for t in n.inputs]
             y = self.values[id(n.output)]
             self._pending = grads
@@ -992,6 +1018,8 @@
                 elif g is dy:
                     fresh = False
                 cur = grads.get(id(sym))
+                if cur is not None and not isinstance(g, L.DeferredGrad) and not g.is_contiguous():
+                    g, fresh = e.dense(g), True
                 if cur is not None:
                     if isinstance(g, L.DeferredGrad):
                         g, fresh = g.materialise(e), True
diff --git a/building_detection_amd/switches.py b/building_detection_amd/switches.py
--- a/building_detection_amd/switches.py
+++ b/building_detection_amd/switches.py
@@ -10,6 +10,7 @@
     "SG_SCSE_LOWRANK": ("ne0", "1", "an scSE block's input gradient is written once, by a final kernel that adds the two gates' rank-one terms; 0: three passes"),
     "SG_ACT_PLANES": ("ne0", "1", "activation planes made once per tensor and step, kept for the planes-in filter gradient; 0: split in every launch"),
     "SG_UP2_FUSE": ("ne0", "1", "UpSampling2D(2) -> Conv2D 3x3 as one sub-pixel launch; 0: a pair of launches"),
+    "SG_CONCAT_INPLACE": ("eq1", "1", "BatchNormalization / UpSampling2D producers write their slice of a concatenation, its gradient is read in slices; off: copy kernels"),
     "SG_GRAD_ACC": ("eq1", "1", "the gradient of a two-consumer block input is summed in the dgrad epilogue; off: by a separate add"),
     "SG_PREPARED_PLANES": ("ne0", "1", "weight planes prepared once per optimiser step; 0: rebuilt inside every convolution call"),
     "SG_JIT_LANES": ("ne0", "1", "the captured training step keeps filter gradients on a side lane; 0: inline in one linear graph"),
diff --git a/include/segengine.h b/include/segengine.h
--- a/include/segengine.h
+++ b/include/segengine.h
@@ -233,6 +233,24 @@
   size_t ws_bytes;
 } sg_bn_plan_t;
 int sg_bn_plan(const sg_ctx* ctx, int dtype, int64_t rows, int C, int pass, int aligned, sg_bn_plan_t* out);
+
+int sg_bn_train_fwd_ld(sg_ctx* ctx, void* stream, int dtype, int64_t rows, int C, const void* x,
+                       const void* gamma, const void* beta, void* moving_mean, void* moving_var, void* y,
+                       void* save_mean, void* save_invstd, float momentum, float eps, int relu,
+                       int unbiased_update, void* ws, size_t ws_bytes, int y_ld);
+int sg_bn_apply_ld(sg_ctx* ctx, void* stream, int dtype, int64_t rows, int C, const void* x, const void* gamma,
+                   const void* beta, const void* mean, const void* invstd, void* y, int relu, int y_ld);
+int sg_bn_infer_ld(sg_ctx* ctx, void* stream, int dtype, int64_t rows, int C, const void* x,
+                   const void* gamma, const void* beta, const void* moving_mean, const void* moving_var,
+                   void* y, float eps, int relu, int y_ld);
+int sg_bn_train_bwd_ld(sg_ctx* ctx, void* stream, int dtype, int64_t rows, int C, const void* x,
+                       const void* y, const void* dy, const void* gamma, const void* beta, const void* save_mean,
+                       const void* save_invstd, void* dx, void* dgamma, void* dbeta, int relu, void* ws,
+                       size_t ws_bytes, int dy_ld);
+int sg_bn_train_bwd_apply_ld(sg_ctx* ctx, void* stream, int dtype, int64_t rows, int C, const void* x, const void* dy,
+                             const void* gamma, const void* beta, const void* save_mean, const void* save_invstd,
+                             const void* dgamma, const void* dbeta, void* dx, int relu, int dy_ld);
+int sg_slice_ok(const sg_ctx* ctx, int dtype, int64_t rows, int C, int ld, int off);
 
 typedef struct sg_seg_plan_t {
   int V, TX, TY, gx, S;
```

Measured after the change: 233.3 tiles/s. About the same (-0.6%).
